# Franc-Z/CuClarabel

Measured on AMD Instinct MI355X. Metric: KKT factorize+solve/sec (fp64) per IPM iter, 100k-var SOCP, higher is better.
Workload: dtype f64

## Files before the change

### cuclarabel_amd/csrc/chain_kernels.hip

```cpp
#include "kernels.hpp"
#include "solve_common.hpp"
#include <cstdlib>

namespace hipkkt {

constexpr int kTinyFrontMax = 8;
constexpr int kChainPF = 4;

__device__ __forceinline__ void chain_add(int* w)
{
    (void)__hip_atomic_fetch_add(w, 1, __ATOMIC_RELAXED, __HIP_MEMORY_SCOPE_AGENT);
}
__device__ __forceinline__ void chain_set(int* w, int v)
{
    __hip_atomic_store(w, v, __ATOMIC_RELAXED, __HIP_MEMORY_SCOPE_AGENT);
}
__device__ __forceinline__ void drain_stores() { asm volatile("s_waitcnt vmcnt(0)" ::: "memory"); }

template <int BS, int PF, int NR>
__device__ __forceinline__ void chain_fwd_block(const SolveArgs& A, const ChainArgs& C, const RecSeg& R, int begin, int bx, long long t0)
{
    extern __shared__ __attribute__((aligned(16))) double smem[];
    __shared__ int sh_ok;
    const int tid = threadIdx.x, lane = tid & 63;
// ... 341 lines not shown
            if (tid < f) z[lds_ix<NR>(c, cst, tid)] = (tid < nc) ? zv[c] * dinv : -zv[c];
    }
#pragma unroll
    for (int c = 0; c < NR; ++c) {
        const double* xc = A.xp + c;
        for (int i = tid + BS; i < f; i += BS)
            z[lds_ix<NR>(c, cst, i)] = (i < nc) ? LD_AGENT_F64(xc + (int64_t)(c0 + i) * NR) * A.Dinv[c0 + i]
                                      : -LD_AGENT_F64(xc + (int64_t)(rec ? rec_idx(rec, i) : T.rows[rp + i - nc]) * NR);
    }
    __syncthreads();
    CH_STAMP(1, 3);
    auto apply = [&](const ItemRegs& R, int it) {
        if constexpr (NR == 2) {
            item_apply_cols<NR>(R, z, cst, nc, f, part, ncpad, it, ncb, lane);
        } else {
            const int rs = it / ncb, cb = it - rs * ncb;
            const int j = cb * 64 + lane, r0 = 8 * rs;
#pragma unroll
            for (int c = 0; c < NR; ++c) {
                double acc = 0.0;
#pragma unroll
                for (int q = 0; q < 8; ++q) acc = fma(R.m[q], (r0 + q < f) ? z[c * cst + r0 + q] : 0.0, acc);
                if (j < nc) part[c * cst + rs * ncpad + j] = acc;
            }
        }
    };
#pragma unroll
    for (int p = 0; p < PB; ++p)
        if (wv + p * NW < nitB) apply(rbk[p], wv + p * NW);
    for (int it0 = wv + PB * NW; it0 < nitB; it0 += 2 * NW) {
        ItemRegs rr[2];
#pragma unroll
        for (int u = 0; u < 2; ++u) {
            const int it = it0 + u * NW;
            const int rs = it / ncb, cb = it - rs * ncb;
            const int j = cb * 64 + lane, r0 = 8 * rs;
            const bool live = it < nitB && !(r0 + 7 < cb * 64);
#pragma unroll
            for (int q = 0; q < 8; ++q) rr[u].m[q] = (live && j < nc && r0 + q < f) ? Wt[j + (int64_t)(r0 + q) * nc] : 0.0;
        }
#pragma unroll
        for (int u = 0; u < 2; ++u)
            if (it0 + u * NW < nitB) apply(rr[u], it0 + u * NW);
    }
    __syncthreads();
    CH_STAMP(1, 4);
    for (int j = tid; j < nc; j += BS) {
        const int pi = j == tid ? ridx : (rec ? rec_idx(rec, j) : T.perm[c0 + j]);
        const double2 vp = lds_sum_pair<NR>(part, j, nrs, ncpad);
#pragma unroll
        for (int c = 0; c < NR; ++c) {
            const double v = lds_sum_col<NR>(vp, part, cst, c, j, nrs, ncpad);
            ST_AGENT_F64(A.xp + (int64_t)(c0 + j) * NR + c, v);
            A.out[c * A.ld_out + pi] = v;
        }
    }
    drain_stores();
    __syncthreads();
    CH_STAMP(1, 5);
    if (tid == 0) chain_set(C.done + s, C.epoch);
}
#undef CH_STAMP

template <int BS, int NR>
__device__ __forceinline__ void chain_bwd_wave(const SolveArgs& A, const ChainArgs& C, const RecSeg& R, int begin, int count, int bx, long long t0)
{
    const int lane = threadIdx.x & 63;
    const int wv = __builtin_amdgcn_readfirstlane((int)(threadIdx.x >> 6));
    const int item = bx * (BS / 64) + wv;
    if (item >= count) return;
    const TreeDev& T = A.T;
    int s, c0, nc, nb, par, idx = 0;
    int64_t f_off;
    if (const char* rec = rec_of(A, R, 1, item)) {
        const SolveHdr h = *reinterpret_cast<const SolveHdr*>(rec);
        idx = rec_idx(rec, lane);
        s = h.s; c0 = h.c0; nc = h.nc; nb = h.nb; par = h.par; f_off = h.mat_off;
    } else {
        const FrontDesc fd = T.desc[begin + item];
        s = fd.s; c0 = fd.c0; nc = fd.nc; nb = fd.nb; f_off = fd.front_off;
        par = T.sn_parent[s];
        idx = (lane < nc) ? T.perm[c0 + lane] : ((lane < nc + nb) ? T.rows[fd.rp + lane - nc] : 0);
    }
    const int f = nc + nb;
    const double* __restrict__ F = A.fronts + f_off;
    const double di = (lane < nc) ? A.Dinv[c0 + lane] : 0.0;
    const int ri = idx, pi = idx;
    double lv0[8];
#pragma unroll
    for (int q = 0; q < 8; ++q) {
        const int j = nc - 1 - q;
        lv0[q] = (j >= 0 && lane > j && lane < f) ? F[lane + (int64_t)j * f] : 0.0;
    }
    if (chain_parent_pending(T, C, par)) {
        int ok = 1;
        if (lane == 0 && !wait_flag(C.done + par, C.epoch, C.abort_word, t0, A.top_limit)) ok = 0;
        ok = __builtin_amdgcn_readfirstlane(ok);
        if (!ok) return;
        asm volatile("" ::: "memory");
    }
    double y[NR];
#pragma unroll
    for (int c = 0; c < NR; ++c) y[c] = (lane < f) ? LD_AGENT_F64(A.xp + (int64_t)(lane < nc ? c0 + lane : ri) * NR + c) : 0.0;
    if (lane < nc) {
#pragma unroll
        for (int c = 0; c < NR; ++c) y[c] *= di;
    }
    for (int j1 = nc; j1 > 0; j1 -= 8) {
        double lv[8];
#pragma unroll
        for (int q = 0; q < 8; ++q) {
            const int j = j1 - 1 - q;
            lv[q] = j1 == nc ? lv0[q] : ((j >= 0 && lane > j && lane < f) ? F[lane + (int64_t)j * f] : 0.0);
        }
#pragma unroll
        for (int q = 0; q < 8; ++q) {
            const int j = j1 - 1 - q;
            if (j >= 0) {
#pragma unroll
                for (int c = 0; c < NR; ++c) {
                    const double sum = wave_reduce_sum(lv[q] * y[c]);
                    if (lane == j) y[c] -= sum;
                }
            }
        }
    }
    if (lane < nc) {
#pragma unroll
        for (int c = 0; c < NR; ++c) {
            ST_AGENT_F64(A.xp + (int64_t)(c0 + lane) * NR + c, y[c]);
            A.out[c * A.ld_out + pi] = y[c];
        }
    }
    drain_stores();
    if (lane == 0) chain_set(C.done + s, C.epoch);
}

template <int BS, int NR>
__device__ __forceinline__ void chain_bwd_tiny(const SolveArgs& A, const ChainArgs& C, const RecSeg& R, int begin, int count, int bx, long long t0)
{
    const int sub = threadIdx.x & 7;
    const int item = bx * (BS >> 3) + (int)(threadIdx.x >> 3);
    const bool live = item < count;
    if (!__any(live)) return;
    const TreeDev& T = A.T;
    int s, c0, nc, nb, par, idx = 0;
    int64_t f_off;
    if (const char* rec = rec_of(A, R, 2, live ? item : count - 1)) {
        const SolveHdr* h = reinterpret_cast<const SolveHdr*>(rec);
        s = h->s; c0 = h->c0; nc = h->nc; nb = h->nb; par = h->par; f_off = h->mat_off;
        idx = rec_idx(rec, sub);
    } else {
        const FrontDesc fd = T.desc[begin + (live ? item : count - 1)];
        s = fd.s; c0 = fd.c0; nc = fd.nc; nb = fd.nb; f_off = fd.front_off;
        par = T.sn_parent[s];
        idx = (sub < nc) ? T.perm[c0 + sub] : ((sub < nc + nb) ? T.rows[fd.rp + sub - nc] : 0);
    }
    const int f = nc + nb;
    const double* __restrict__ F = A.fronts + f_off;
    const double di = (sub < nc) ? A.Dinv[c0 + sub] : 0.0;
    const int ri = idx, pi = idx;
    double lv[kTinyFrontMax];
#pragma unroll
    for (int j = 0; j < kTinyFrontMax; ++j) lv[j] = (j < nc && sub > j && sub < f) ? F[sub + j * f] : 0.0;
    {
        bool ok = true;
        if (live && sub == 0 && chain_parent_pending(T, C, par) && !wait_flag(C.done + par, C.epoch, C.abort_word, t0, A.top_limit)) ok = false;
        if (__any(!ok)) return;
        asm volatile("" ::: "memory");
    }
    double y[NR];
#pragma unroll
    for (int c = 0; c < NR; ++c) y[c] = (sub < f) ? LD_AGENT_F64(A.xp + (int64_t)(sub < nc ? c0 + sub : ri) * NR + c) : 0.0;
    if (sub < nc) {
#pragma unroll
        for (int c = 0; c < NR; ++c) y[c] *= di;
    }
#pragma unroll
    for (int j = kTinyFrontMax - 1; j >= 0; --j) {
#pragma unroll
        for (int c = 0; c < NR; ++c) {
            const double sum = group8_sum(lv[j] * y[c]);
            if (j < nc && sub == j) y[c] -= sum;
        }
    }
    if (live && sub < nc) {
#pragma unroll
        for (int c = 0; c < NR; ++c) {
            ST_AGENT_F64(A.xp + (int64_t)(c0 + sub) * NR + c, y[c]);
            A.out[c * A.ld_out + pi] = y[c];
        }
    }
    drain_stores();
    if (live && sub == 0) chain_set(C.done + s, C.epoch);
}

template <int BS, int NR, int PF>
__global__ __launch_bounds__(BS) void k_bwd_chain(SolveArgs A, ChainArgs C)
{
    const long long t0 = wall_clock64();
    const int k = chain_find_seg(C, blockIdx.x);
    const int begin = C.seg[k].begin, nblock = C.seg[k].nblock, nwave = C.seg[k].nwave, ntiny = C.seg[k].ntiny;
    const int b = (int)blockIdx.x - C.seg[k].wg0;
    const int nwb = (nwave + BS / 64 - 1) / (BS / 64);
    if (b < nblock) { chain_bwd_block<BS, PF, NR>(A, C, C.seg[k].rec, begin, b, t0); return; }
    if (b < nblock + nwb) chain_bwd_wave<BS, NR>(A, C, C.seg[k].rec, begin + nblock, nwave, b - nblock, t0);
    else chain_bwd_tiny<BS, NR>(A, C, C.seg[k].rec, begin + nblock + nwave, ntiny, b - nblock - nwb, t0);
}

#define HIPKKT_NR_SWITCH(nr, ...)                                                                 \
    do {                                                                                         \
        if ((nr) == 1) { constexpr int NR = 1; __VA_ARGS__; }                                    \
        else if ((nr) == 2) { constexpr int NR = 2; __VA_ARGS__; }                               \
        else { constexpr int NR = 4; __VA_ARGS__; }                                              \
    } while (0)

static void init_chain_lds()
{
    static PerDeviceOnce once;
    once.run([]() {
        hipError_t e = hipSuccess;
        auto set = [&](auto k, int bytes) { if (e == hipSuccess) e = set_max_lds(k, bytes); };
#define HIPKKT_SET_CHAIN(NRV) set(k_fwd_chain<kChainBS, NRV, kChainPF>, 150 * 1024); set(k_bwd_chain<kChainBS, NRV, kChainPF>, 150 * 1024);
        HIPKKT_SET_CHAIN(1) HIPKKT_SET_CHAIN(2) HIPKKT_SET_CHAIN(4)
#undef HIPKKT_SET_CHAIN
        return e;
    });
}

void launch_fwd_chain(const SolveArgs& a, const ChainArgs& c, int nwg, size_t lds, hipStream_t st, int nr)
{
    if (nwg <= 0) return;
    init_chain_lds();
    HIPKKT_NR_SWITCH(nr, hipLaunchKernelGGL((k_fwd_chain<kChainBS, NR, kChainPF>), dim3(nwg), dim3(kChainBS), lds * NR, st, a, c));
}
void launch_bwd_chain(const SolveArgs& a, const ChainArgs& c, int nwg, size_t lds, hipStream_t st, int nr)
{
    if (nwg <= 0) return;
    init_chain_lds();
    HIPKKT_NR_SWITCH(nr, hipLaunchKernelGGL((k_bwd_chain<kChainBS, NR, kChainPF>), dim3(nwg), dim3(kChainBS), lds * NR, st, a, c));
}

}
// ... 1 lines not shown
```

### cuclarabel_amd/csrc/hipkkt.hip

```cpp
#include "../../include/hipkkt.h"

#include <hip/hip_runtime.h>

#include <algorithm>
#include <cfloat>
#include <chrono>
#include <cmath>
#include <cstdio>
#include <cstdlib>
#include <cstring>
#include <array>
#include <map>
#include <memory>
#include <mutex>
#include <stdexcept>
#include <string>
#include <vector>

#include "kernels.hpp"
#include "kkt_assembly.hpp"
#include "symbolic.hpp"
#include "knobs.hpp"

namespace hipkkt {
// ... 86 lines not shown
    LDLEngine(int N, const int64_t* colptr, const int64_t* rowval, int base, const std::vector<int>& dsigns,
              const hipkkt_settings& st)
    {
        SymbolicOptions opt;
        opt.ordering = st.ordering;
        opt.amd_dense_scale = st.amd_dense_scale > 0 ? st.amd_dense_scale : 1.5;
        if (st.nd_leaf_size > 0) opt.nd_leaf_size = st.nd_leaf_size;
        opt.user_perm = st.user_perm;
        apply_knobs(opt);
        analyse(N, colptr, rowval, base, opt, S);
        panel_cap = opt.panel_cap;
        panel_max_slices = std::max(1, opt.panel_max_slices);
        dyn_eps = st.dynamic_regularization_eps;
        dyn_delta = st.dynamic_regularization_delta;
        build_schedule();
        upload(dsigns);
        if (knobs().verbose) {
            int nblock = 0, nsl_fronts = 0, ov_slices = 0;
            for (const Launch& L : launches) if (!L.small) { nblock += L.count; nsl_fronts += L.nsliced; }
            if (overlap_wanted()) for (size_t q = ov_first; q < launches.size(); ++q) ov_slices += launches[q].slice_count;
            std::fprintf(stderr, "[hipkkt] N %d, %d supernodes in %zu levels (%zu launches), %d block-class fronts, %d of them in "
                         "%zu row slices; persistent solve set: last %zu launches, %d fronts on %d workgroups, %d (front, slice) tasks; "
                         "factorisation overlap: last %zu launches (%d row slices in them)\n",
                         S.N, S.nsuper, S.levels.size(), launches.size(), nblock, nsl_fronts, slice_list.size(), top_launches,
                         top_count, top_ntask > 0 ? top_sgrid : top_grid, top_ntask, overlap_wanted() ? launches.size() - ov_first : (size_t)0,
                         ov_slices);
            {
                int ntall_all = 0;
                for (const Launch& L : launches) ntall_all += L.ntall;
                if (ntall_all) std::fprintf(stderr, "[hipkkt] %d fronts too tall for the block sweep kernels (k_fwd_tall / k_bwd_tall)\n", ntall_all);
            }
            if (knobs().verbose >= 2)
                for (size_t q = 0; q < launches.size(); ++q) {
                    const Launch& L = launches[q];
                    int fmin = 1 << 30, ncmin = 1 << 30;
                    double flops = 0;
                    for (int t = L.begin; t < L.begin + L.count; ++t) {
                        const int sn = sched[(size_t)t], nc = S.sn_start[sn + 1] - S.sn_start[sn], f = front_size(sn);
                        fmin = std::min(fmin, f); ncmin = std::min(ncmin, nc);
                        flops += (double)nc * (f - nc) * (f - nc) + (double)nc * nc * (f - nc) + (double)nc * nc * nc / 3;
                    }
                    std::fprintf(stderr, "[hipkkt] launch %zu level %d: %d fronts (%s), f %d..%d, nc %d..%d, %d sliced into %d, %d tiles (%d columns deep on average), %.3f GF\n",
                                 q, L.level, L.count, L.small ? "one wave" : "block", fmin, L.fmax, ncmin, L.ncmax, L.nsliced, L.slice_count,
                                 L.ntiles, L.tile_nc, flops * 1e-9);
                }
            if (overlap_wanted())
                for (size_t q = ov_first; q < launches.size(); ++q)
                    std::fprintf(stderr, "[hipkkt] overlap admission: launch %zu: %d panel workgroups, %d tiles behind a gate, %d CUs\n", q,
                                 ov_group_of[q] >= 0 ? ov_groups[(size_t)ov_group_of[q]].count : launches[q].count - launches[q].nsliced + launches[q].slice_count,
                                 launches[q].ntiles, n_cus);
        }
    }

    void factor(const double* d_Kval, const double* d_eps)
    {
        const bool want_stamps = knobs().stamps;
        const bool no_graph = !knobs().graph;
        if (want_stamps || no_graph || n_factor_calls++ == 0) {
            enqueue_factor(d_Kval, d_eps, stream, nullptr, want_stamps);
            return;
        }
        auto key = std::make_pair((const void*)d_Kval, (const void*)d_eps);
        auto it = factor_graphs.find(key);
        if (it == factor_graphs.end()) {
            ensure_capture_streams();
            HIP_CHECK(hipStreamBeginCapture(cap_stream, hipStreamCaptureModeThreadLocal));
            enqueue_factor(d_Kval, d_eps, cap_stream, cap_side, false);
            hipGraph_t g;
            HIP_CHECK(hipStreamEndCapture(cap_stream, &g));
            hipGraphExec_t ex;
            HIP_CHECK(hipGraphInstantiate(&ex, g, nullptr, nullptr, 0));
            HIP_CHECK(hipGraphDestroy(g));
            it = factor_graphs.emplace(key, ex).first;
        }
        HIP_CHECK(hipGraphLaunch(it->second, stream));
    }

    void solve(const double* d_b, double* d_x, bool allow_top = false, int nr = 1, int64_t ldb = 0, int64_t ldx = 0)
    {
        const bool no_graph = !knobs().graph;
        if (nr > 1) {
            if (!supports_nr(nr)) throw ArgError("solve: this structure takes one right-hand side per sweep");
            reserve_nr(nr);
        }
        if (no_graph || nr > 1 || n_solve_calls++ == 0) {
            const bool waits = allow_top && ((!top_disabled && top_launches > 0) || (!chain_disabled && chain_from < launches.size()));
            const bool tok = waits && claim_dev(kOpS);
            TokenRelease rel{this, tok};
            enqueue_solve(d_b, d_x, stream, tok, nr, ldb, ldx, tok);
            if (tok) { rel.on = false; dev_enqueued(true); }
            return;
        }
        auto key = std::make_pair((const void*)d_b, (const void*)d_x);
        auto it = solve_graphs.find(key);
        if (it == solve_graphs.end()) {
            ensure_capture_streams();
            HIP_CHECK(hipStreamBeginCapture(cap_stream, hipStreamCaptureModeThreadLocal));
            enqueue_solve(d_b, d_x, cap_stream, false, 1, 0, 0);
            hipGraph_t g;
            HIP_CHECK(hipStreamEndCapture(cap_stream, &g));
            hipGraphExec_t ex;
            HIP_CHECK(hipGraphInstantiate(&ex, g, nullptr, nullptr, 0));
            HIP_CHECK(hipGraphDestroy(g));
            it = solve_graphs.emplace(key, ex).first;
        }
        HIP_CHECK(hipGraphLaunch(it->second, stream));
    }
    bool supports_nr(int nr) const
    {
        if (nr == 1) return true;
        if (nr != 2 && nr != 4) return false;
        if (top_ntask > 0 && (nr != 2 || top_sgrid2 <= 0)) return false;
        const size_t below = top_ntask > 0 ? launches.size() - top_launches : launches.size();
        for (size_t q = 0; q < below; ++q)
            if (!launches[q].small && (launches[q].ntall > 0 || launches[q].lds_solve * (size_t)nr > kLdsCap)) return false;
        return true;
    }

    void solve_multi(const double* d_B, int64_t ldb, double* d_X, int64_t ldx, int nrhs)
    {
        if (nrhs <= 0) return;
        if (nrhs == 1) { solve(d_B, d_X); return; }
        const int KP = multi_prepare(nrhs);
        launch_permute_in(d_B, ldb, xp_m.p, KP, d_iperm.p, S.N, nrhs, stream);
        multi_sweeps(KP);
        launch_permute_out(d_X, ldx, xp_m.p, KP, d_iperm.p, S.N, nrhs, stream);
        HIP_CHECK(hipGetLastError());
    }
    void solve_multi_rm(const double* d_B, double* d_X, int KP, const double* d_add = nullptr)
    {
        if (KP <= 0 || (KP & 15)) throw ArgError("solve_multi_rm: KP must be a positive multiple of 16");
        multi_prepare(KP);
        multi_sweeps(KP, d_B, d_X, d_add);
        HIP_CHECK(hipGetLastError());
    }

private:
    int multi_prepare(int nrhs)
    {
        const int KP = (nrhs + 15) & ~15;
        if (KP / 8 > 65535) throw ArgError("solve_multi: too many right-hand sides per call");
        {
            int64_t widest = 0;
            for (const Launch& L : launches) if (!L.small) widest = std::max<int64_t>(widest, (L.count + 7) / 8);
            if (widest * (KP / 16) > 65535) throw ArgError("solve_multi: too many right-hand sides per call for this structure (split the call)");
        }
        wait_w(stream);
        if ((size_t)KP > multi_cap) {
            xp_m.alloc((size_t)S.N * KP);
            uvec_m.alloc(std::max<size_t>(S.rows.size(), 1) * KP);
            multi_cap = (size_t)KP;
        }
        if (!d_iperm.p) d_iperm.upload(S.iperm);
        return KP;
    }
    void multi_sweeps(int KP, const double* b_rm = nullptr, double* out_rm = nullptr, const double* add_rm = nullptr)
    {
        SolveArgs a;
        a.T = tree();
// ... 102 lines not shown
            if (cap_side && !new_main) beside.push_back(cap_side);
            if (cu_mask) ov_stream = stream_beside(ov_stream, beside, masked, &ov_concurrent);
            else ov_stream = stream_beside(ov_stream, beside, plain, &ov_concurrent);
            if (!ov_stream) {
                ov_disabled = true;
                std::fprintf(stderr, "[hipkkt] no stream for the Schur tiles: factorisation overlap off\n");
            } else if (!had) {
                HIP_CHECK(hipEventCreateWithFlags(&ev_ov_fork, hipEventDisableTiming));
                HIP_CHECK(hipEventCreateWithFlags(&ev_ov_join, hipEventDisableTiming));
            }
            if (ov_stream && !ov_concurrent && knobs().verbose)
                std::fprintf(stderr, "[hipkkt] the main and the tile stream share a hardware queue: no merged panel kernel for this handle\n");
        }
        ensure_capture_streams();
        if (new_main) {
            std::vector<hipStream_t> beside{st};
            if (ov_stream) beside.push_back(ov_stream);
            cap_side = stream_beside(cap_side, beside, plain, &side_concurrent);
            if (!side_concurrent && knobs().verbose)
                std::fprintf(stderr, "[hipkkt] no stream beside the main stream for the W formation: it will run in submission order\n");
        }
        sides_for = st;
    }

    void enqueue_factor(const double* d_Kval, const double* d_eps, hipStream_t st, hipStream_t side, bool want_stamps)
    {
        wait_w(st);
        if (ov_join_pending) {
            if (side) HIP_CHECK(hipEventSynchronize(ev_ov_join));
            else HIP_CHECK(hipStreamWaitEvent(st, ev_ov_join, 0));
            ov_join_pending = false;
        }
        ZeroList zl;
        zl.add(flags.p, 3);
        const bool want_ov = overlap_wanted();
        const bool use_ov = want_ov && !side && !want_stamps && !ov_disabled && ov_first < launches.size();
        const bool no_overlap = knobs().no_overlap;
        const bool side_w = !side && !no_overlap && !want_stamps && late_launches > 0 && late_launches < launches.size();
        const bool tok_x = use_ov && claim_dev(kOpX);
        const bool tok = tok_x || (side_w && claim_dev(kOpM));
        TokenRelease ov_release{this, tok};
        if (!side && !want_stamps) choose_side_streams(st, tok_x);
        const bool ov_on = tok_x && !ov_disabled && ov_stream != nullptr;
        auto group_of = [&](size_t q) -> const MergeGroup* {
            return (ov_concurrent && q < ov_group_of.size() && ov_group_of[q] >= 0) ? &ov_groups[(size_t)ov_group_of[q]] : nullptr;
        };
        const size_t merge_from = (ov_concurrent && !ov_groups.empty()) ? ov_groups.back().first : ~(size_t)0;
        if (ov_on) {
            zl.add(d_ov_prog.p, S.nsuper);
            zl.add(d_ov_done.p, S.nsuper);
            if (!slice_list.empty()) zl.add(d_ov_sprog.p, (int)slice_list.size());
            zl.add(d_ov_started.p, (int)launches.size());
        }
        launch_zero_ints_multi(zl, st);
        FactorArgs a;
        a.T = tree();
        a.Kval = d_Kval;
        a.eps = d_eps;
        a.fronts = fronts.p;
        a.upd = upd.p;
        a.Dinv = Dinv.p;
        a.flags = flags.p;
        a.dyn_eps = dyn_eps;
        a.dyn_delta = dyn_delta;
        a.ov_prog = d_ov_prog.p; a.ov_done = d_ov_done.p; a.ov_ntiles = d_ov_ntiles.p; a.ov = 0;
        a.ov_sprog = d_ov_sprog.p; a.ov_sbase = d_ov_sbase.p;
        a.ov_started = d_ov_started.p; a.ov_slot = 0;
        const long long ov_limit = knobs().ov_test_limit;
        a.ov_limit = ov_limit;
        a.stamps = nullptr;
        a.stamp_row = 0;
        if (want_stamps) {
            if (!stamps.p) { stamps.alloc(launches.size() * 16); }
            stamps.zero(st);
            a.stamps = (long long*)stamps.p;
        }
        int li = 0;
        bool forked = false;
#ifdef HIPKKT_EXPERIMENTS
        static const bool no_gate = std::getenv("HIPKKT_EXPERIMENT_NO_GATE") != nullptr;
#else
        constexpr bool no_gate = false;
#endif
#ifdef HIPKKT_EXPERIMENTS
        static const int skip_w_after = std::getenv("HIPKKT_EXPERIMENT_SKIP_WINV") ? std::atoi(std::getenv("HIPKKT_EXPERIMENT_SKIP_WINV")) : -1;
        const bool skip_w = skip_w_after >= 0 && n_skipw_calls++ >= skip_w_after;
#else
        const bool skip_w = false;
#endif
        auto form_w = [&](const int* list, int count, int ncmax, hipStream_t on, int max_blocks) {
            const size_t i0 = (size_t)(list - d_tinv_list.p);
            const int nsmall = i0 + (size_t)count < tinv_small_prefix.size() ? tinv_small_prefix[i0 + (size_t)count] - tinv_small_prefix[i0] : 0;
            if (!skip_w) launch_tinv(a.T, fronts.p, tinv.p, list, count, ncmax, on, max_blocks, nsmall);
        };
        const size_t nl = launches.size();
        const size_t first_top = (tok && side_w) ? nl - late_launches : nl;
        bool eager_fork = false;
        int w_done = 0;
        for (size_t q = 0; q < nl; ++q) {
            const Launch& L = launches[q];
            a.stamp_row = li++;
            const bool runs = ov_on && merge_from < nl;
            const size_t tail_fork = runs ? nl : (nl >= (size_t)std::max(0, knobs().winv_tail) ? nl - (size_t)std::max(0, knobs().winv_tail) : 0);
            const MergeGroup* gq = runs ? group_of(q) : nullptr;
            const bool run_forks = knobs().winv_run_forks;
            const bool run_first = gq && gq->first == q && (run_forks || q == merge_from);
            auto fork_at = [&](size_t want) {
// ... 67 lines not shown
            w_pending = true;
        } else {
            form_w(d_tinv_list.p, (int)tinv_list.size(), tinv_ncmax, st, 0);
        }
        if (ov_on) {
            HIP_CHECK(hipEventRecord(ev_ov_join, ov_stream));
            ov_join_pending = true;
        }
        if (tok) {
            ov_release.on = false;
            dev_enqueued(true);
        }
        HIP_CHECK(hipGetLastError());
        if (want_stamps) {
            std::vector<long long> h(launches.size() * 16);
            HIP_CHECK(hipMemcpyAsync(h.data(), stamps.p, h.size() * 8, hipMemcpyDeviceToHost, st));
            HIP_CHECK(hipStreamSynchronize(st));
            static int printed = 0;
            if (printed++ == 2) {
                for (size_t r = 0; r < launches.size(); ++r) {
                    const long long* q = &h[r * 16];
                    if (launches[r].small) continue;
                    std::fprintf(stderr, "[stamps2] launch %zu: wave 0's items %.1f us (first batch's loads %.1f us), then all waves %.1f us\n", r, (q[7] - q[6]) * 0.01, (q[15] - q[6]) * 0.01, (q[3] - q[7]) * 0.01);
                    std::fprintf(stderr, "[stamps] launch %zu fronts %d f=%lld nc=%lld kids=%lld | zero %.1f K %.1f kids %.1f factor %.1f "
                                 "(diag %.1f trsm %.1f trail %.1f) store %.1f us  clk %.0f MHz\n", r, launches[r].count, q[11], q[12], q[13],
                                 (q[1] - q[0]) * 0.01, (q[2] - q[1]) * 0.01, (q[3] - q[2]) * 0.01, (q[4] - q[3]) * 0.01,
                                 q[8] * 0.01, q[9] * 0.01, q[10] * 0.01, (q[5] - q[4]) * 0.01,
                                 (double)q[14] / ((q[5] - q[0]) * 0.01));
                }
            }
        }
    }

    void reserve_nr(int nr)
    {
        if ((size_t)nr <= nr_cap) return;
        wait_w(stream);
        HIP_CHECK(hipStreamSynchronize(stream));
        for (auto& kv : solve_graphs) (void)hipGraphExecDestroy(kv.second);
        solve_graphs.clear();
        xp.alloc((size_t)S.N * nr);
        uvec.alloc(std::max<size_t>(S.rows.size(), 1) * nr);
        nr_cap = (size_t)nr;
    }
    int top_grid_for(int nr)
    {
        if (nr == 1) return top_grid;
        if (top_ntask > 0) return nr == 2 ? top_sgrid2 : 0;
        int& g = top_grid_nr[nr == 2 ? 0 : 1];
        if (g < 0) g = std::min(top_grid, top_solve_capacity_nr(top_lds * (size_t)nr, nr));
        return g;
    }

    void enqueue_solve(const double* d_b, double* d_x, hipStream_t st, bool use_top, int nr, int64_t ldb, int64_t ldx, bool allow_chain = false)
    {
        SolveArgs a;
        a.T = tree();
        a.fronts = fronts.p;
        a.tinv = tinv.p;
        a.Dinv = Dinv.p;
        a.b = d_b;
        a.out = d_x;
        a.xp = xp.p;
        a.uvec = uvec.p;
        const long long top_limit = knobs().top_test_limit;
        a.top_limit = top_limit;
        const int stamp_call = knobs().top_stamps;
        a.top_stamps = nullptr;
        bool stamp_now = false;
        a.ld_b = ldb; a.ld_out = ldx; a.ld_xp = S.N; a.ld_uvec = (int64_t)std::max<size_t>(S.rows.size(), 1);
        a.tk_pos = d_tk_pos.p; a.tk_sl = d_tk_sl.p; a.tbase = d_tbase.p; a.xf = xf.p; a.add = nullptr;
        a.chain_cnt = nullptr;
        a.recs = d_recs.p ? reinterpret_cast<const char*>(d_recs.p) : nullptr;
        a.tall_ws = tall_ws.p;
        const bool no_top = knobs().no_top;
        if (nr > 1 && top_ntask > 0 && (no_top || !use_top || top_disabled || top_sgrid2 <= 0)) {
            for (int c = 0; c < nr; ++c) enqueue_solve(d_b + (int64_t)c * ldb, d_x + (int64_t)c * ldx, st, use_top, 1, 0, 0, allow_chain);
            return;
        }
        const size_t nl = launches.size();
        const bool chain_env = knobs().chain;
        const bool chain_top = knobs().chain_top;
        const bool chain_want = chain_env && allow_chain && !chain_disabled && chain_from < nl && chain_lds * (size_t)nr <= 150 * 1024;
        const bool keep_top = chain_want && (chain_top || top_ntask > 0);
        const int tgrid = (no_top || !use_top || top_disabled || (chain_want && !keep_top)) ? 0 : top_grid_for(nr);
        size_t ntl = tgrid > 0 ? top_launches : 0;
        int ncount = top_count;
        if (ntl > 0 && w_pending && late_launches > 0 && late_launches < ntl && !(nr > 1 && top_ntask > 0)) { ntl = late_launches; ncount = late_count; }
        const size_t first_w = nl - std::min(nl, late_launches);
        const bool chain_on = chain_want && chain_from + 2 <= nl - ntl;
        const size_t nper = chain_on ? chain_from : nl - ntl;
        const bool no_merge = knobs().no_level_merge;
        auto pair_at = [&](size_t q) {
            return !no_merge && q + 1 < nper && !launches[q].small && launches[q].ntall == 0 && launches[q + 1].small &&
                   launches[q].level == launches[q + 1].level;
        };
        auto pair_rec = [](const Launch& Lb, const Launch& Ls) {
            RecSeg r = Ls.rec;
            r.off[0] = Lb.rec.off[0]; r.stride[0] = Lb.rec.stride[0]; r.fmax[0] = Lb.rec.fmax[0];
            return r;
        };
        bool chain_stamp = false;
        ChainArgs ca;
        int ca_wgs = 0;
        size_t ca_lds = 0;
        auto chain_reset = [&]() {
            ca.nseg = 0; ca.lo = 1 << 30; ca.hi = 0; ca.cnt = d_chain.p; ca.done = d_chain.p + S.nsuper; ca.nchild = d_chain_nchild.p;
            ca.abort_word = top_flags.p + 2 * top_nflag; ca.epoch = chain_epoch;
            ca.lo0 = chain_on ? launches[nper].begin : 0;
            ca.nstamp = chain_on ? launches[nl - ntl - 1].begin + launches[nl - ntl - 1].count - ca.lo0 : 0;
            ca_wgs = 0; ca_lds = 0;
        };
        auto chain_flush = [&](bool fwd) {
            if (ca.nseg > 0) {
                a.top_stamps = chain_stamp ? (long long*)top_stamps.p : nullptr;
                if (fwd) launch_fwd_chain(a, ca, ca_wgs, ca_lds, st, nr);
                else launch_bwd_chain(a, ca, ca_wgs, ca_lds, st, nr);
                a.top_stamps = nullptr;
            }
            chain_reset();
        };
        auto chain_add = [&](const Launch& L, bool fwd) {
            const bool blocks = !L.small;
            if (ca.nseg == kChainMaxSeg) chain_flush(fwd);
            ChainSeg& sg = ca.seg[ca.nseg++];
            sg.begin = L.begin;
            sg.nblock = blocks ? L.count : 0;
            sg.nwave = blocks ? 0 : L.count - L.ntiny;
            sg.ntiny = blocks ? 0 : L.ntiny;
            sg.wg0 = ca_wgs;
// ... 1414 lines not shown
            pool.push_back(s.b);
        }
        spans.clear();
    }
    ~Profiler()
    {
        for (Span& s : spans) { (void)hipEventDestroy(s.a); (void)hipEventDestroy(s.b); }
        for (hipEvent_t e : pool) (void)hipEventDestroy(e);
    }
};

}

using namespace hipkkt;

struct hipkkt_ldl_s {
    int device = 0;
    hipkkt_settings st;
    hipStream_t stream = nullptr;
    int64_t N = 0, nnzK = 0;
    int base = 0;
    std::unique_ptr<LDLEngine> eng;
    DBuf<double> Kval, vals, b, x;
    DBuf<double> mB;
    size_t mcap = 0;
    DBuf<int> idx;
    ~hipkkt_ldl_s() { if (stream) (void)hipStreamDestroy(stream); }
};

struct hipkkt_kkt_s {
    int device = 0;
    hipkkt_settings st;
    hipStream_t stream = nullptr;
    bool own_stream = true;
    KKTAssembly K;
    std::unique_ptr<LDLEngine> eng;
    DBuf<double> Kval, Pval, Aval;
    DBuf<int> mapP, mapA, mapHs, mapDiag, mapU, mapV, mapD, soc_of_entry;
    DBuf<int64_t> fptr;
    DBuf<int> fcol, fmap;
    DBuf<int64_t> fpend;
    DBuf<double> fval;
    bool fval_dirty = true;
    DBuf<int> kpos;
    DBuf<int> long_rows;
    DBuf<int64_t> long_chunk_ptr, chunk_q;
    DBuf<double> long_partial;
    int nlong = 0, nchunks = 0;
    size_t long_partial_cols = 0;
    int lanes_per_row = 8;
    DBuf<double> b, x, e, dx, rx, rz, sbuf, zbuf, ybuf;
    double *cur_x = nullptr, *cur_dx = nullptr;
    DBuf<double> partial, scal;
    std::unique_ptr<PinnedScalars> pin;
    DBuf<int> c_kind, c_off, c_numel, c_sidx, c_soff, c_elem, c_soclist;
    DBuf<int64_t> c_boff;
    DBuf<double> w, eta, soc_u, soc_v, soc_eta2, Hs;
    DBuf<int> fail;
    int nsoc = 0, npsd = 0, psd_kmax = 1;
    DBuf<int> c_explist, c_powlist, c_nsidx;
    DBuf<double> c_param, ns_grad, ns_H;
    int nexp = 0, npow = 0, ns_strategy = HIPKKT_SCALING_PRIMAL_DUAL;
    double ns_mu = 0.0;
    DBuf<int> gp_cone, gp_dim1, gp_off, gp_small, gp_big, gp_mapP, gp_mapQR, gp_mapD;
    DBuf<double> gp_alpha, gp_grad, gp_d, gp_p, gp_qr;
    int ngp_small = 0, ngp_big = 0;
    double gp_mu = 0.0;
    DBuf<int> c_psdlist, c_psddim;
    DBuf<int64_t> c_psdaoff;
    DBuf<double> psdA, psdR, psdRinv;
    bool has_psd = false, psd_too_big = false, scaling_valid = false;
    double last_eps = 0;
    int64_t last_ir = 0;
    DBuf<double> irbuf;
    double *ir_state = nullptr, *ir_readback = nullptr, *ir_sticky = nullptr, *ir_norms = nullptr, *sys_out_dev = nullptr;
    int ir_stride = 0;
    int r_spec = 1;
    bool publish_ok = true;
    long long publish_seq = 0;
    int spec_low_calls = 0;
    bool deferred = false;
    DBuf<double> lam;
    DBuf<double> sq, snegq, sb, sx2, sz2, sworkx, sworkz, sconic, spa, spb, spc;
    DBuf<double> sys_partial, sys_dots, sys_cached, sys_in;
    bool sys_ready = false;
    bool sys_lazy = false;
    bool sys_const_pending = false;
    bool sys_update_unread = false;
    DBuf<double> hst;
    bool host_vars_valid = false;
    hipEvent_t ev_upload = nullptr;
    void host_upload_mark(hipStream_t st)
    {
        if (!ev_upload) HIP_CHECK(hipEventCreateWithFlags(&ev_upload, hipEventDisableTiming));
        HIP_CHECK(hipEventRecord(ev_upload, st));
    }
    void host_upload_wait() { if (ev_upload) HIP_CHECK(hipEventSynchronize(ev_upload)); }
    DBuf<double> mB, mX, mC, mE, mE2, mpartial, mnorms;
    DBuf<int> mmask;
    size_t mcap = 0;
    Profiler prof;
    ~hipkkt_kkt_s()
    {
        if (ev_upload) (void)hipEventDestroy(ev_upload);
        if (stream && own_stream) (void)hipStreamDestroy(stream);
    }
// ... 296 lines not shown
        if (!h || nrhs < 0 || (nrhs > 0 && (!d_X || !d_B || ldx < h->N || ldb < h->N)))
            throw ArgError("hipkkt_ldl_solve_multi_dev: bad argument");
        HIP_CHECK(hipSetDevice(h->device));
        h->eng->solve_multi(d_B, ldb, d_X, ldx, (int)nrhs);
        return HIPKKT_OK;
    });
}

int hipkkt_ldl_solve_multi(hipkkt_ldl_t h, int64_t nrhs, double* X, const double* B)
{
    return guarded([&]() {
        if (!h || nrhs < 0 || (nrhs > 0 && (!X || !B))) throw ArgError("hipkkt_ldl_solve_multi: bad argument");
        if (nrhs == 0) return HIPKKT_OK;
        HIP_CHECK(hipSetDevice(h->device));
        if ((size_t)nrhs > h->mcap) { h->mB.alloc((size_t)h->N * nrhs); h->mcap = (size_t)nrhs; }
        const size_t bytes = (size_t)h->N * nrhs * sizeof(double);
        HIP_CHECK(hipMemcpyAsync(h->mB.p, B, bytes, hipMemcpyHostToDevice, h->stream));
        h->eng->solve_multi(h->mB.p, h->N, h->mB.p, h->N, (int)nrhs);
        HIP_CHECK(hipMemcpyAsync(X, h->mB.p, bytes, hipMemcpyDeviceToHost, h->stream));
        HIP_CHECK(hipStreamSynchronize(h->stream));
        return HIPKKT_OK;
    });
}

int hipkkt_ldl_info(hipkkt_ldl_t h, hipkkt_info* info)
{
    return guarded([&]() {
        if (!h || !info) throw ArgError("hipkkt_ldl_info: bad argument");
        std::memset(info, 0, sizeof(*info));
        fill_info(h->eng->S, info);
        return HIPKKT_OK;
    });
}

int hipkkt_ldl_get_perm(hipkkt_ldl_t h, int64_t* perm)
{
    return guarded([&]() {
        if (!h || !perm) throw ArgError("hipkkt_ldl_get_perm: bad argument");
        for (int64_t i = 0; i < h->N; ++i) perm[i] = h->eng->S.perm[i];
        return HIPKKT_OK;
    });
}

int hipkkt_ldl_fallbacks(hipkkt_ldl_t h, int64_t out[2])
{
    return guarded([&]() {
        if (!h || !out) throw ArgError("hipkkt_ldl_fallbacks: bad argument");
        out[0] = h->eng->n_ov_fallbacks;
        out[1] = h->eng->n_top_fallbacks;
        return HIPKKT_OK;
    });
}

int hipkkt_kkt_create(hipkkt_kkt_t* out, int64_t n, int64_t m, const int64_t* Pcolptr, const int64_t* Prowval,
                      const double* Pnzval, const int64_t* Acolptr, const int64_t* Arowval, const double* Anzval,
                      int64_t ncones, const int32_t* kinds, const int64_t* dims, const hipkkt_settings* settings,
                      int base)
{
    return hipkkt_kkt_create_ex(out, n, m, Pcolptr, Prowval, Pnzval, Acolptr, Arowval, Anzval, ncones, kinds, dims, nullptr,
                                settings, base);
}

int hipkkt_kkt_create_ex(hipkkt_kkt_t* out, int64_t n, int64_t m, const int64_t* Pcolptr, const int64_t* Prowval,
                         const double* Pnzval, const int64_t* Acolptr, const int64_t* Arowval, const double* Anzval,
                         int64_t ncones, const int32_t* kinds, const int64_t* dims, const double* cone_params,
                         const hipkkt_settings* settings, int base)
{
    std::vector<int64_t> pptr;
    std::vector<double> pvals;
    if (ncones > 0 && kinds) {
        for (int64_t c = 0; c < ncones; ++c)
            if (kinds[c] == HIPKKT_CONE_GENPOW) {
                g_last_error = "a generalized power cone has one alpha per row of its first block: use hipkkt_kkt_create_ex2";
                return HIPKKT_ERR_ARG;
            }
        if (cone_params) {
            pptr.assign((size_t)ncones + 1, base);
            for (int64_t c = 0; c < ncones; ++c) {
                pptr[(size_t)c + 1] = pptr[(size_t)c];
                if (kinds[c] == HIPKKT_CONE_POW) { pvals.push_back(cone_params[c]); pptr[(size_t)c + 1] += 1; }
            }
        }
    }
    return hipkkt_kkt_create_ex2(out, n, m, Pcolptr, Prowval, Pnzval, Acolptr, Arowval, Anzval, ncones, kinds, dims,
                                 pptr.empty() ? nullptr : pptr.data(), pvals.data(), settings, base);
}

int hipkkt_kkt_create_ex2(hipkkt_kkt_t* out, int64_t n, int64_t m, const int64_t* Pcolptr, const int64_t* Prowval,
                          const double* Pnzval, const int64_t* Acolptr, const int64_t* Arowval, const double* Anzval,
                          int64_t ncones, const int32_t* kinds, const int64_t* dims, const int64_t* cone_param_ptr,
                          const double* cone_param_vals, const hipkkt_settings* settings, int base)
{
    return guarded([&]() {
        if (!out || !Pcolptr || !Acolptr || n < 0 || m < 0 || ncones < 0 || (ncones > 0 && (!kinds || !dims)))
            throw ArgError("hipkkt_kkt_create: bad argument");
        if (base != 0 && base != 1) throw ArgError("index_base must be 0 or 1");
        if (n + m == 0) throw ArgError("empty problem");
        std::unique_ptr<hipkkt_kkt_s> h(new hipkkt_kkt_s);
        if (settings) h->st = *settings; else hipkkt_default_settings(&h->st);
        try {
            assemble_kkt(n, m, Pcolptr, Prowval, Pnzval, Acolptr, Arowval, Anzval, ncones, kinds, dims, base, h->K, cone_param_ptr,
                         cone_param_vals);
        } catch (const std::runtime_error& e) {
            throw ArgError(e.what());
        }
        h->device = select_device(h->st);
        HIP_CHECK(hipStreamCreateWithFlags(&h->stream, hipStreamNonBlocking));
        KKTAssembly& K = h->K;
        hipkkt_settings st = h->st;
        if (st.ordering == HIPKKT_ORDER_USER && !st.user_perm) throw ArgError("ORDER_USER needs user_perm");
        std::vector<int64_t> rv(K.rowval.begin(), K.rowval.end());
        std::vector<int64_t> uperm;
        if (st.ordering == HIPKKT_ORDER_USER) {
            uperm.resize(K.N);
            for (int i = 0; i < K.N; ++i) uperm[i] = st.user_perm[i] - base;
            st.user_perm = uperm.data();
        }
        h->eng.reset(new LDLEngine(K.N, K.colptr.data(), rv.data(), 0, K.dsigns, st));
        h->eng->stream = h->stream;
        h->eng->set_device(h->device);
        h->st.user_perm = nullptr;

        h->Kval.upload(K.nzval);
        h->mapP.upload(K.mapP);
        h->mapA.upload(K.mapA);
        h->mapHs.upload(K.mapHs);
        h->mapDiag.upload(K.map_diag);
        h->mapU.upload(K.mapU);
        h->mapV.upload(K.mapV);
        h->mapD.upload(K.mapD);
        h->Pval.alloc(K.mapP.size());
        h->Aval.alloc(K.mapA.size());
        {
            const int N = K.N;
            std::vector<int64_t> ptr((size_t)N + 1, 0);
            for (int j = 0; j < N; ++j)
                for (int64_t q = K.colptr[j]; q < K.colptr[j + 1]; ++q) {
                    int i = K.rowval[q];
                    ptr[i + 1]++;
                    if (i != j) ptr[j + 1]++;
                }
            for (int i = 0; i < N; ++i) ptr[i + 1] += ptr[i];
            std::vector<int> col((size_t)ptr[N]), vmap((size_t)ptr[N]);
            std::vector<int64_t> nx(ptr.begin(), ptr.end() - 1);
            for (int j = 0; j < N; ++j) {
                for (int64_t q = K.colptr[j]; q < K.colptr[j + 1]; ++q) {
                    int i = K.rowval[q];
                    int64_t d = nx[j]++;
                    col[d] = i;
                    vmap[d] = (int)q;
                }
            }
            for (int j = 0; j < N; ++j)
                for (int64_t q = K.colptr[j]; q < K.colptr[j + 1]; ++q) {
                    int i = K.rowval[q];
                    if (i == j) continue;
                    int64_t d = nx[i]++;
                    col[d] = j;
                    vmap[d] = (int)q;
                }
            h->fptr.upload(ptr);
            h->fcol.upload(col);
            h->fmap.upload(vmap);
            {
                std::vector<int64_t> pend((size_t)std::max<int64_t>(K.n, 1), 0);
                for (int64_t i = 0; i < K.n; ++i)
                    pend[(size_t)i] = std::lower_bound(col.begin() + ptr[(size_t)i], col.begin() + ptr[(size_t)i + 1], (int)K.n) - col.begin();
                h->fpend.upload(pend);
            }
            h->fval.alloc(vmap.size());
            {
                std::vector<int> kp((size_t)2 * K.nnzK, -1);
                for (size_t q = 0; q < vmap.size(); ++q) {
                    const size_t e = (size_t)vmap[q];
                    if (kp[2 * e] < 0) kp[2 * e] = (int)q; else kp[2 * e + 1] = (int)q;
                }
                h->kpos.upload(kp);
            }
            {
                std::vector<int> lrows;
// ... 99 lines not shown
                for (double* q : {h->gp_grad.p, h->gp_d.p, h->gp_p.p, h->gp_qr.p}) HIP_CHECK(hipMemset(q, 0, gl * sizeof(double)));
            }
            {
                std::vector<int> plist, pdim(nc, 0);
                std::vector<int64_t> paoff(nc, 0);
                int64_t ao = 0;
                for (size_t c = 0; c < nc; ++c) {
                    const ConeInfo& ci = K.cones[c];
                    if (ci.kind != HIPKKT_CONE_PSD) continue;
                    plist.push_back((int)c);
                    pdim[c] = ci.dim;
                    paoff[c] = ao;
                    ao += (int64_t)ci.dim * ci.dim;
                    h->psd_kmax = std::max(h->psd_kmax, ci.dim);
                }
                h->npsd = (int)plist.size();
                h->c_psdlist.upload(plist); h->c_psddim.upload(pdim); h->c_psdaoff.upload(paoff);
                h->psdA.alloc((size_t)ao); h->psdR.alloc((size_t)ao); h->psdRinv.alloc((size_t)ao);
            }
            h->c_kind.upload(kind); h->c_off.upload(off); h->c_numel.upload(numel); h->c_boff.upload(boff);
            h->c_sidx.upload(sidx); h->c_soff.upload(soff); h->c_elem.upload(elem); h->c_soclist.upload(soclist);
            h->soc_of_entry.upload(soc_of);
            h->w.alloc((size_t)K.m); h->eta.alloc(nc); h->lam.alloc((size_t)K.m);
            h->soc_u.alloc((size_t)K.sparse_len); h->soc_v.alloc((size_t)K.sparse_len);
            h->soc_eta2.alloc((size_t)K.nsparse); h->Hs.alloc((size_t)K.nHs);
            h->fail.alloc(1);
            HIP_CHECK(hipMemset(h->fail.p, 0, sizeof(int)));
        }
        *out = h.release();
        return HIPKKT_OK;
    });
}

void hipkkt_kkt_destroy(hipkkt_kkt_t h)
{
    if (!h) return;
    (void)hipSetDevice(h->device);
    (void)hipStreamSynchronize(h->stream);
    delete h;
}

int hipkkt_kkt_info(hipkkt_kkt_t h, hipkkt_info* info)
{
    return guarded([&]() {
        if (!h || !info) throw ArgError("hipkkt_kkt_info: bad argument");
        std::memset(info, 0, sizeof(*info));
        fill_info(h->eng->S, info);
        info->n = h->K.n; info->m = h->K.m; info->p = h->K.p;
        info->nHs = h->K.nHs; info->nsparse_soc = h->K.nsparse; info->sparse_soc_len = h->K.sparse_len;
        return HIPKKT_OK;
    });
}

static int kkt_update_device(hipkkt_kkt_t h, bool deferred = false)
{
    KKTAssembly& K = h->K;
    int pu = h->prof.begin(0, h->stream);
    launch_update_values(h->Kval.p, h->mapHs.p, h->Hs.p, (int)K.nHs, h->mapU.p, h->mapV.p, h->mapD.p, h->soc_u.p, h->soc_v.p,
                         h->soc_eta2.p, h->soc_of_entry.p, K.sparse_len, K.nsparse, h->fval_dirty ? nullptr : h->fval.p,
                         h->kpos.p, h->stream);
    const double* eps_ptr = nullptr;
    if (h->st.static_regularization_enable) {
        launch_regularizer(h->Kval.p, h->mapDiag.p, K.N, h->st.static_regularization_constant,
                           h->st.static_regularization_proportional, h->partial.p, h->scal.p, h->stream);
        eps_ptr = h->scal.p;
    }
    h->prof.end(pu, h->stream);
    int pf = h->prof.begin(1, h->stream);
    h->eng->factor(h->Kval.p, eps_ptr);
    h->prof.end(pf, h->stream);
    launch_collect_status(h->scal.p + 8, h->scal.p, h->fail.p, h->eng->flags_ptr(), h->stream, deferred ? h->ir_sticky : nullptr);
    if (deferred) return HIPKKT_OK;
    HIP_CHECK(hipMemcpyAsync(h->pin->h + 8, h->scal.p + 8, 5 * sizeof(double), hipMemcpyDeviceToHost, h->stream));
    HIP_CHECK(hipStreamSynchronize(h->stream));
    if (h->pin->h[12] != 0.0) {
        h->eng->ov_gave_up();
        h->eng->factor(h->Kval.p, eps_ptr);
        launch_collect_status(h->scal.p + 8, h->scal.p, h->fail.p, h->eng->flags_ptr(), h->stream);
        HIP_CHECK(hipMemcpyAsync(h->pin->h + 8, h->scal.p + 8, 5 * sizeof(double), hipMemcpyDeviceToHost, h->stream));
        HIP_CHECK(hipStreamSynchronize(h->stream));
    }
    h->last_eps = h->st.static_regularization_enable ? h->pin->h[8] : 0.0;
    h->prof.acc.dynamic_regularizations += (int64_t)h->pin->h[10];
    if (h->pin->h[9] != 0.0) return HIPKKT_NUMERIC_FAILURE;
    return h->pin->h[11] != 0.0 ? HIPKKT_NUMERIC_FAILURE : HIPKKT_OK;
}

int hipkkt_kkt_update_cones(hipkkt_kkt_t h, const double* Hs, const double* soc_u, const double* soc_v,
                            const double* soc_eta2)
{
    return guarded([&]() {
        if (!h) throw ArgError("null handle");
        KKTAssembly& K = h->K;
        if ((K.nHs > 0 && !Hs) || (K.nsparse > 0 && (!soc_u || !soc_v || !soc_eta2)))
            throw ArgError("hipkkt_kkt_update_cones: missing cone data");
        if (K.ngenpow > 0)
            throw ArgError("hipkkt_kkt_update_cones: (Hs, u, v, eta^2) cannot carry p, q, r of a generalized power cone; such a "
                           "handle is scaled on the device (hipkkt_kkt_update_from_sz, hipkkt_kkt_system_update)");
        HIP_CHECK(hipSetDevice(h->device));
        if (K.nHs) HIP_CHECK(hipMemcpyAsync(h->Hs.p, Hs, (size_t)K.nHs * sizeof(double), hipMemcpyHostToDevice, h->stream));
        if (K.nsparse) {
            HIP_CHECK(hipMemcpyAsync(h->soc_u.p, soc_u, (size_t)K.sparse_len * sizeof(double), hipMemcpyHostToDevice, h->stream));
            HIP_CHECK(hipMemcpyAsync(h->soc_v.p, soc_v, (size_t)K.sparse_len * sizeof(double), hipMemcpyHostToDevice, h->stream));
            HIP_CHECK(hipMemcpyAsync(h->soc_eta2.p, soc_eta2, (size_t)K.nsparse * sizeof(double), hipMemcpyHostToDevice, h->stream));
        }
        launch_zero_ints(h->fail.p, 1, h->stream);
        h->scaling_valid = false;
        return kkt_update_device(h);
    });
}

static int kkt_update_from_sz_dev_impl(hipkkt_kkt_t h, const double* d_s, const double* d_z, bool deferred)
{
    return guarded([&]() {
        if (!h || (h->K.m > 0 && (!d_s || !d_z))) throw ArgError("hipkkt_kkt_update_from_sz: bad argument");
        if (h->psd_too_big)
            throw ArgError("update_from_sz: PSD cones with side > 48 are scaled by the caller; use hipkkt_kkt_update_cones");
        HIP_CHECK(hipSetDevice(h->device));
        launch_zero_ints(h->fail.p, 1, h->stream);
        int pu = h->prof.begin(0, h->stream);
        h->gp_mu = h->ns_mu;
        launch_cone_scaling(h->cone_dev(), h->cone_state(), d_s, d_z, h->K.m, h->stream);
        h->prof.end(pu, h->stream);
        h->scaling_valid = true;
        return kkt_update_device(h, deferred);
    });
}
int hipkkt_kkt_update_from_sz_dev(hipkkt_kkt_t h, const double* d_s, const double* d_z)
{
    return kkt_update_from_sz_dev_impl(h, d_s, d_z, h && h->deferred);
}

int hipkkt_kkt_update_from_sz(hipkkt_kkt_t h, const double* s, const double* z)
{
    return guarded([&]() {
        if (!h || (h->K.m > 0 && (!s || !z))) throw ArgError("hipkkt_kkt_update_from_sz: bad argument");
        HIP_CHECK(hipSetDevice(h->device));
        size_t bytes = (size_t)h->K.m * sizeof(double);
        if (bytes) {
            HIP_CHECK(hipMemcpyAsync(h->sbuf.p, s, bytes, hipMemcpyHostToDevice, h->stream));
            HIP_CHECK(hipMemcpyAsync(h->zbuf.p, z, bytes, hipMemcpyHostToDevice, h->stream));
        }
        return hipkkt_kkt_update_from_sz_dev(h, h->sbuf.p, h->zbuf.p);
    });
}

int hipkkt_kkt_update_P(hipkkt_kkt_t h, const double* Pnzval)
{
    return guarded([&]() {
        if (!h || (h->K.mapP.size() && !Pnzval)) throw ArgError("hipkkt_kkt_update_P: bad argument");
        HIP_CHECK(hipSetDevice(h->device));
        size_t k = h->K.mapP.size();
        if (!k) return HIPKKT_OK;
        HIP_CHECK(hipMemcpyAsync(h->Pval.p, Pnzval, k * sizeof(double), hipMemcpyHostToDevice, h->stream));
        launch_scatter(h->Kval.p, h->mapP.p, h->Pval.p, (int64_t)k, 1.0, h->stream);
        h->fval_dirty = true;
        HIP_CHECK(hipStreamSynchronize(h->stream));
        return HIPKKT_OK;
    });
}

int hipkkt_kkt_update_A(hipkkt_kkt_t h, const double* Anzval)
{
    return guarded([&]() {
        if (!h || (h->K.mapA.size() && !Anzval)) throw ArgError("hipkkt_kkt_update_A: bad argument");
        HIP_CHECK(hipSetDevice(h->device));
        size_t k = h->K.mapA.size();
        if (!k) return HIPKKT_OK;
        HIP_CHECK(hipMemcpyAsync(h->Aval.p, Anzval, k * sizeof(double), hipMemcpyHostToDevice, h->stream));
        launch_scatter(h->Kval.p, h->mapA.p, h->Aval.p, (int64_t)k, 1.0, h->stream);
        h->fval_dirty = true;
        HIP_CHECK(hipStreamSynchronize(h->stream));
        return HIPKKT_OK;
    });
}

int hipkkt_kkt_setrhs_dev(hipkkt_kkt_t h, const double* d_rx, const double* d_rz)
{
    return guarded([&]() {
        if (!h || (h->K.n && !d_rx) || (h->K.m && !d_rz)) throw ArgError("hipkkt_kkt_setrhs: bad argument");
        HIP_CHECK(hipSetDevice(h->device));
        launch_pack_rhs(h->b.p, d_rx, d_rz, h->K.n, h->K.m, h->K.p, h->stream);
        return HIPKKT_OK;
    });
}

int hipkkt_kkt_setrhs(hipkkt_kkt_t h, const double* rx, const double* rz)
{
    return guarded([&]() {
        if (!h || (h->K.n && !rx) || (h->K.m && !rz)) throw ArgError("hipkkt_kkt_setrhs: bad argument");
        HIP_CHECK(hipSetDevice(h->device));
        if (h->K.n) HIP_CHECK(hipMemcpyAsync(h->rx.p, rx, (size_t)h->K.n * sizeof(double), hipMemcpyHostToDevice, h->stream));
        if (h->K.m) HIP_CHECK(hipMemcpyAsync(h->rz.p, rz, (size_t)h->K.m * sizeof(double), hipMemcpyHostToDevice, h->stream));
        launch_pack_rhs(h->b.p, h->rx.p, h->rz.p, h->K.n, h->K.m, h->K.p, h->stream);
        HIP_CHECK(hipStreamSynchronize(h->stream));
        return HIPKKT_OK;
    });
}

static SpmvDev kkt_spmv(hipkkt_kkt_t h)
{
    if (h->fval_dirty) {
        launch_gather_values(h->fval.p, h->Kval.p, h->fmap.p, (int64_t)h->fmap.n, h->stream);
        h->fval_dirty = false;
    }
    SpmvDev A;
    A.ptr = h->fptr.p; A.col = h->fcol.p; A.vmap = h->fmap.p; A.val = h->fval.p; A.N = h->K.N;
    A.pend = h->fpend.p;
    A.lanes_per_row = h->lanes_per_row;
    A.nlong = h->nlong; A.nchunks = h->nchunks; A.long_rows = h->long_rows.p; A.long_chunk_ptr = h->long_chunk_ptr.p;
    A.chunk_q = h->chunk_q.p; A.long_partial = h->long_partial.p;
    return A;
}

static bool kkt_partials_mode(hipkkt_kkt_t h, int nr) { return residual_partials_ok(kkt_spmv(h), nr); }
static double* kkt_partials(hipkkt_kkt_t h, bool candidate) { return h->partial.p + (candidate ? h->partial.n / 2 : 0); }
static void kkt_enqueue_refine_error(hipkkt_kkt_t h, const double* xi, double* norm_out, double* normb_out, int nr, bool candidate)
{
    const SpmvDev A = kkt_spmv(h);
    const bool unfinished = kkt_partials_mode(h, nr);
    int pr = h->prof.begin(3, h->stream);
    launch_residual(A, h->Kval.p, h->b.p, xi, h->e.p, kkt_partials(h, candidate), unfinished ? nullptr : norm_out, h->stream, nr,
                    nr > 1 ? (int64_t)h->K.N : 0, h->eng->top_abort_word(), h->scal.p + 3, normb_out);
    h->prof.end(pr, h->stream);
}
static void kkt_trisolve(hipkkt_kkt_t h, const double* rhs, double* out, bool allow_top = true, int nr = 1)
{
    int ps = h->prof.begin(2, h->stream);
    h->eng->solve(rhs, out, allow_top, nr, h->K.N, h->K.N);
    h->prof.end(ps, h->stream);
}

struct IrNorms { double *norme0, *normb, *cand; };
static IrNorms kkt_ir_norms(hipkkt_kkt_t h, int nr)
{
    if (nr == 1) return IrNorms{h->scal.p + 1, h->scal.p + 2, h->scal.p + 4};
    return IrNorms{h->ir_norms, h->ir_norms + kMaxNR, h->ir_norms + 2 * kMaxNR};
}
static void kkt_launch_ir(hipkkt_kkt_t h, int r, bool first, bool readback, bool fold, int nr)
{
    const hipkkt_settings& st = h->st;
    const IrNorms nm = kkt_ir_norms(h, nr);
    const double* abortw = h->eng->top_abort_word() ? h->scal.p + 3 : nullptr;
    IrPartials Q;
    const bool unfinished = kkt_partials_mode(h, nr);
    if (unfinished) {
        Q.np = residual_grid(kkt_spmv(h)) + 1;
        Q.e0 = kkt_partials(h, false);
        Q.b0 = Q.e0 + (size_t)nr * Q.np;
        Q.cand = r > 0 ? kkt_partials(h, true) : nullptr;
        Q.flag_in = h->eng->top_abort_word();
    }
    launch_ir_round(h->ir_state, h->ir_stride, r, first, nm.norme0, nm.normb, nm.cand, abortw, h->x.p, h->dx.p, h->K.N, nr,
                    st.iterative_refinement_abstol, st.iterative_refinement_reltol, st.iterative_refinement_stop_ratio,
                    std::max(st.iterative_refinement_max_iter, 0), readback ? h->ir_readback : nullptr,
                    (fold && (nr == 1 || unfinished)) ? h->ir_sticky : nullptr, h->stream, Q);
    if (fold && nr > 1 && !unfinished) launch_ir_fold(h->ir_state, h->ir_stride, r, nr, abortw, h->ir_sticky, h->stream);
}
static void kkt_enqueue_round(hipkkt_kkt_t h, int r, bool first, bool readback, bool fold, int nr)
{
    kkt_trisolve(h, h->e.p, h->dx.p, true, nr);
    launch_axpby_sum(h->dx.p, h->dx.p, h->x.p, (int64_t)h->K.N * nr, h->stream);
    kkt_enqueue_refine_error(h, h->dx.p, kkt_ir_norms(h, nr).cand, nullptr, nr, true);
    kkt_launch_ir(h, r, first, readback, fold, nr);
}
static int kkt_solve_core(hipkkt_kkt_t h, bool may_defer = false, int nr = 1, int64_t* ir_out = nullptr, bool force_defer = false)
{
    const hipkkt_settings& st = h->st;
    const bool deferred = force_defer || (may_defer && h->deferred);
    h->cur_x = h->x.p;
    h->cur_dx = h->dx.p;
    h->last_ir = 0;
    if (ir_out) for (int c = 0; c < nr; ++c) ir_out[c] = deferred ? -1 : 0;
    if (!st.iterative_refinement_enable) {
        kkt_trisolve(h, h->b.p, h->x.p, false, nr);
        int bad = 0;
        launch_zero_ints(h->fail.p, 1, h->stream);
        launch_check_finite(h->x.p, h->K.N * nr, h->fail.p, h->stream);
        if (deferred) { launch_fold_flag(h->ir_sticky, h->fail.p, h->stream); return HIPKKT_OK; }
        HIP_CHECK(hipMemcpyAsync(&bad, h->fail.p, sizeof(int), hipMemcpyDeviceToHost, h->stream));
        HIP_CHECK(hipStreamSynchronize(h->stream));
        return bad ? HIPKKT_NUMERIC_FAILURE : HIPKKT_OK;
    }
    const int max_iter = std::max(st.iterative_refinement_max_iter, 0);
    int R = std::min(max_iter, std::max(h->r_spec, deferred ? 1 : 0));
    const IrNorms nm = kkt_ir_norms(h, nr);
    kkt_trisolve(h, h->b.p, h->x.p, true, nr);
    kkt_enqueue_refine_error(h, h->x.p, nm.norme0, nm.normb, nr, false);
    if (R == 0) kkt_launch_ir(h, 0, true, !deferred, deferred, nr);
    for (int r = 1; r <= R; ++r) kkt_enqueue_round(h, r, r == 1, r == R && !deferred, r == R && deferred, nr);
    if (deferred) { h->last_ir = -1; return HIPKKT_OK; }
    int64_t total = 0;
    for (;;) {
        HIP_CHECK(hipMemcpyAsync(h->pin->h + 16, h->ir_readback, 5 * (size_t)nr * sizeof(double), hipMemcpyDeviceToHost, h->stream));
        HIP_CHECK(hipStreamSynchronize(h->stream));
        bool any_active = false, any_bad = false, aborted = false;
        total = 0;
        for (int c = 0; c < nr; ++c) {
            const double* rb = h->pin->h + 16 + 5 * c;
            any_active = any_active || rb[0] != 0.0;
            any_bad = any_bad || rb[2] != 0.0;
            aborted = aborted || rb[4] != 0.0;
            total += (int64_t)rb[1];
            if (ir_out) ir_out[c] = (int64_t)rb[1];
        }
        if (aborted && h->eng->top_abort_word() != nullptr) {
            h->eng->top_gave_up();
            return kkt_solve_core(h, false, nr, ir_out);
        }
        h->last_ir = total;
        if (any_bad) { h->prof.acc.ir_iterations += total; return HIPKKT_NUMERIC_FAILURE; }
        if (!any_active || R >= max_iter) break;
        ++R;
        kkt_enqueue_round(h, R, false, true, false, nr);
    }
// ... 485 lines not shown
    if (rc != HIPKKT_OK) return rc;
    if (enqueue_only) h->sys_update_unread = true;
    return guarded([&]() { return sys_after_update(h); });
}

int hipkkt_kkt_system_solve_initial_point(hipkkt_kkt_t h, double* d_x, double* d_s, double* d_z)
{
    return guarded([&]() {
        if (!h || !h->sys_ready) throw ArgError("hipkkt_kkt_system_*: call hipkkt_kkt_system_init first");
        if ((h->K.n && !d_x) || (h->K.m && (!d_s || !d_z))) throw ArgError("hipkkt_kkt_system_solve_initial_point: bad argument");
        HIP_CHECK(hipSetDevice(h->device));
        const int n = h->K.n, m = h->K.m;
        int rc = sys_flush_startup(h);
        if (rc != HIPKKT_OK) return rc;
        if (h->mapP.n == 0) {
            if (n) HIP_CHECK(hipMemsetAsync(h->sworkx.p, 0, (size_t)n * sizeof(double), h->stream));
            rc = sys_solve_into(h, h->sworkx.p, h->sb.p, d_x, h->sworkz.p);
            if (rc != HIPKKT_OK) return rc;
            launch_neg_copy(d_s, h->sworkz.p, m, h->stream);
            if (m) HIP_CHECK(hipMemsetAsync(h->sworkz.p, 0, (size_t)m * sizeof(double), h->stream));
            rc = sys_solve_into(h, h->snegq.p, h->sworkz.p, nullptr, d_z);
            if (rc != HIPKKT_OK) return rc;
        } else {
            rc = sys_solve_into(h, h->snegq.p, h->sb.p, d_x, d_z);
            if (rc != HIPKKT_OK) return rc;
            launch_neg_copy(d_s, d_z, m, h->stream);
        }
        HIP_CHECK(hipStreamSynchronize(h->stream));
        return HIPKKT_OK;
    });
}

static void sys_finish_step(hipkkt_kkt_t h, const double* x1, const double* z1, double* d_lhs_x, double* d_lhs_s, double* d_lhs_z,
                            double* lhs_tau_kappa, double rhs_tau, double rhs_kappa, const double* d_var_x, double var_tau,
                            double var_kappa, bool with_const = false, const double* addend = nullptr, const Publish& pub = Publish{})
{
    const int n = h->K.n, m = h->K.m;
    hipStream_t st = h->stream;
    const double* x2 = with_const ? h->x.p : h->sx2.p;
    const double* z2 = with_const ? h->x.p + n : h->sz2.p;
    launch_P_spmv2(sys_spmv(h), h->Kval.p, x1, d_var_x, x2, var_tau, h->spa.p, h->spb.p, h->sworkx.p,
                   with_const ? h->spc.p : nullptr, n, st);
    DotPairs P{};
    P.npairs = with_const ? 7 : 4;
    if (with_const) {
        P.a[4] = h->sq.p; P.b[4] = x2; P.len[4] = n;
        P.a[5] = h->sb.p; P.b[5] = z2; P.len[5] = m;
        P.a[6] = x2; P.b[6] = h->spc.p; P.len[6] = n;
    }
    P.a[0] = h->sq.p; P.b[0] = x1; P.len[0] = n;
    P.a[1] = h->sb.p; P.b[1] = z1; P.len[1] = m;
    P.a[2] = d_var_x; P.b[2] = h->spa.p; P.len[2] = n;
    P.a[3] = h->sworkx.p; P.b[3] = h->spb.p; P.len[3] = n;
    launch_dots_sys_step(P, h->sys_partial.p, h->sys_cached.p, rhs_tau, rhs_kappa, var_tau, var_kappa, h->sys_out_dev, d_lhs_x, d_lhs_z,
                         x1, z1, x2, z2, n, m, st, with_const ? h->sx2.p : nullptr, with_const ? h->sz2.p : nullptr);
    launch_mul_Hs(h->cone_dev(), h->cone_state(), d_lhs_s, d_lhs_z, m, st, addend ? addend : h->sconic.p, pub);
    if (!lhs_tau_kappa) return;
    HIP_CHECK(hipMemcpyAsync(h->pin->h + 48, h->sys_out_dev, 2 * sizeof(double), hipMemcpyDeviceToHost, st));
    HIP_CHECK(hipStreamSynchronize(st));
    lhs_tau_kappa[0] = h->pin->h[48];
    lhs_tau_kappa[1] = h->pin->h[49];
}
static int sys_flush_update_status(hipkkt_kkt_t h)
{
    if (!h->sys_update_unread) return HIPKKT_OK;
    h->sys_update_unread = false;
    HIP_CHECK(hipMemcpyAsync(h->pin->h + 40, h->ir_sticky, 8 * sizeof(double), hipMemcpyDeviceToHost, h->stream));
    launch_zero_ints((int*)h->ir_sticky, 16, h->stream);
    HIP_CHECK(hipStreamSynchronize(h->stream));
    bool gave_up = false;
    int rc = kkt_eval_sticky(h, h->pin->h + 40, &gave_up);
    if (rc == HIPKKT_REFINEMENT_INCOMPLETE) rc = gave_up ? kkt_update_device(h) : HIPKKT_OK;
    return rc;
}
static int sys_flush_startup(hipkkt_kkt_t h)
{
    const int rc = sys_flush_update_status(h);
    return rc == HIPKKT_NUMERIC_FAILURE ? HIPKKT_OK : rc;
}
static void sys_cache_constant_terms(hipkkt_kkt_t h)
{
    launch_P_spmv(sys_spmv(h), h->Kval.p, h->sx2.p, h->spa.p, h->K.n, h->stream);
    DotPairs P{};
    P.npairs = 3;
    P.a[0] = h->sq.p; P.b[0] = h->sx2.p; P.len[0] = h->K.n;
    P.a[1] = h->sb.p; P.b[1] = h->sz2.p; P.len[1] = h->K.m;
    P.a[2] = h->sx2.p; P.b[2] = h->spa.p; P.len[2] = h->K.n;
    launch_dots(P, h->sys_partial.p, h->sys_cached.p, h->stream);
}

static int sys_solve_step(hipkkt_kkt_t h, double* d_lhs_x, double* d_lhs_s, double* d_lhs_z, double* lhs_tau_kappa,
                          const double* d_rhs_x, const double* d_rhs_s, const double* d_rhs_z, double rhs_tau,
                          double rhs_kappa, const double* d_var_x, const double* d_var_s, const double* d_var_z,
                          double var_tau, double var_kappa, int steptype)
{
    if (!h->sys_ready) throw ArgError("hipkkt_kkt_system_*: call hipkkt_kkt_system_init first");
    const int n = h->K.n, m = h->K.m;
    const bool affine = steptype == 0;
    if ((n && (!d_lhs_x || !d_rhs_x || !d_var_x)) || (m && (!d_lhs_s || !d_lhs_z || !d_rhs_z || !d_var_s || !d_var_z)) ||
        (m && !affine && !d_rhs_s) || !lhs_tau_kappa || (steptype != 0 && steptype != 1))
        throw ArgError("hipkkt_kkt_system_solve: bad argument");
    if (!h->scaling_valid) throw ArgError("hipkkt_kkt_system_solve: needs the cone scaling of hipkkt_kkt_system_update");
    if (h->deferred) throw ArgError("hipkkt_kkt_system_*: level C reads its scalars back (deferred status is for level B)");
    HIP_CHECK(hipSetDevice(h->device));
    hipStream_t st = h->stream;
    const bool pair = h->sys_const_pending && affine && h->eng->supports_nr(2);
    if (h->sys_const_pending && !pair) {
        h->sys_const_pending = false;
        int rc = sys_flush_update_status(h);
        if (rc == HIPKKT_OK) rc = sys_constant_rhs(h);
        if (rc != HIPKKT_OK) return rc;
    }
    h->sys_const_pending = false;
    const size_t N = (size_t)h->K.N;
    auto run = [&](bool defer) -> int {
        if (!affine && !launch_sys_offset(h->cone_dev(), h->cone_state(), h->sconic.p, h->sworkz.p, d_rhs_s, d_var_z, d_rhs_z,
                                          m, false, st))
            throw ArgError("hipkkt_kkt_system_solve: unsupported cone kind");
        if (pair) {
            launch_pack_rhs_affine(h->b.p, h->snegq.p, h->sb.p, d_rhs_x, d_var_s, d_rhs_z, n, m, h->K.p, 2, st);
            int rc = kkt_solve_core(h, false, 2, nullptr, defer);
            if (rc != HIPKKT_OK) return rc;
        } else {
            if (affine) launch_pack_rhs_affine(h->b.p, nullptr, nullptr, d_rhs_x, d_var_s, d_rhs_z, n, m, h->K.p, 1, st);
            else launch_pack_rhs(h->b.p, d_rhs_x, h->sworkz.p, n, m, h->K.p, st);
            int rc = kkt_solve_core(h, false, 1, nullptr, defer);
            if (rc != HIPKKT_OK) return rc;
        }
        const double* x1 = h->x.p + (pair ? N : 0);
        sys_finish_step(h, x1, x1 + n, d_lhs_x, d_lhs_s, d_lhs_z, defer ? nullptr : lhs_tau_kappa, rhs_tau, rhs_kappa, d_var_x, var_tau, var_kappa,
                        pair, affine ? d_var_s : nullptr,
                        (defer && h->publish_ok) ? Publish{h->pin->h + 40, h->ir_sticky, 10, 8, (double)++h->publish_seq} : Publish{});
        return HIPKKT_OK;
    };
    if (h->sys_lazy && h->st.iterative_refinement_enable) {
        const bool update_unread = h->sys_update_unread;
        h->sys_update_unread = false;
        int rc = run(true);
        if (rc != HIPKKT_OK) return rc;
        if (h->publish_ok) {
            HIP_CHECK(hipStreamSynchronize(st));
            if (h->pin->h[50] != (double)h->publish_seq || knobs().test_publish_fail) {
                h->publish_ok = false;
                if (knobs().verbose) std::fprintf(stderr, "[hipkkt] status record not published to host memory: copying it from now on\n");
                if (update_unread) {
                    rc = kkt_update_device(h);
                    if (rc != HIPKKT_OK) return rc;
                }
                return run(false);
            }
        } else {
            HIP_CHECK(hipMemcpyAsync(h->pin->h + 40, h->ir_sticky, 10 * sizeof(double), hipMemcpyDeviceToHost, st));
            launch_zero_ints((int*)h->ir_sticky, 16, st);
            HIP_CHECK(hipStreamSynchronize(st));
        }
        bool gave_up = false;
        rc = kkt_eval_sticky(h, h->pin->h + 40, &gave_up, true);
        h->last_ir = (int64_t)h->pin->h[43];
        if (rc == HIPKKT_OK) {
            lhs_tau_kappa[0] = h->pin->h[48];
            lhs_tau_kappa[1] = h->pin->h[49];
            return HIPKKT_OK;
        }
        if (rc != HIPKKT_REFINEMENT_INCOMPLETE) return rc;
        if (update_unread && gave_up) {
            rc = kkt_update_device(h);
            if (rc != HIPKKT_OK) return rc;
        }
    } else {
        int rc = sys_flush_update_status(h);
        if (rc != HIPKKT_OK) return rc;
    }
    return run(false);
}

int hipkkt_kkt_system_solve(hipkkt_kkt_t h, double* d_lhs_x, double* d_lhs_s, double* d_lhs_z, double* lhs_tau_kappa,
                            const double* d_rhs_x, const double* d_rhs_s, const double* d_rhs_z, double rhs_tau,
                            double rhs_kappa, const double* d_var_x, const double* d_var_s, const double* d_var_z,
// ... 566 lines not shown
```

### cuclarabel_amd/csrc/kernels.hip

```cpp
#include "kernels.hpp"
#include "knobs.hpp"
#include <algorithm>

#include <cmath>

namespace hipkkt {

static inline int grid_for(int64_t n, int bs, int cap = 4096)
{
    int64_t g = (n + bs - 1) / bs;
    if (g < 1) g = 1;
    if (g > cap) g = cap;
    return (int)g;
}

__global__ void k_scatter(double* __restrict__ K, const int* __restrict__ idx, const double* __restrict__ v,
                          int64_t n, double scale)
{
    for (int64_t i = blockIdx.x * (int64_t)blockDim.x + threadIdx.x; i < n; i += (int64_t)gridDim.x * blockDim.x)
        K[idx[i]] = v[i] * scale;
}
void launch_scatter(double* K, const int* idx, const double* v, int64_t n, double scale, hipStream_t st)
{
    if (n <= 0) return;
    hipLaunchKernelGGL(k_scatter, dim3(grid_for(n, 256)), dim3(256), 0, st, K, idx, v, n, scale);
}
__device__ __forceinline__ void put_k(double* __restrict__ K, double* __restrict__ fval, const int* __restrict__ kpos, int e, double v)
{
    K[e] = v;
    if (fval) {
        const int p0 = kpos[2 * e], p1 = kpos[2 * e + 1];
        if (p0 >= 0) fval[p0] = v;
        if (p1 >= 0) fval[p1] = v;
    }
}
__global__ void k_update_values(double* __restrict__ K, const int* __restrict__ mapHs, const double* __restrict__ Hs, int nHs,
                                const int* __restrict__ mapU, const int* __restrict__ mapV, const int* __restrict__ mapD,
                                const double* __restrict__ u, const double* __restrict__ v, const double* __restrict__ eta2,
                                const int* __restrict__ soc_of_entry, int sparse_len, int nsparse,
                                double* __restrict__ fval, const int* __restrict__ kpos)
{
    const int total = nHs + sparse_len + nsparse;
    for (int i = blockIdx.x * blockDim.x + threadIdx.x; i < total; i += gridDim.x * blockDim.x) {
        if (i < nHs) {
            put_k(K, fval, kpos, mapHs[i], -Hs[i]);
        } else if (i < nHs + sparse_len) {
            const int j = i - nHs;
            const double e2 = eta2[soc_of_entry[j]];
            put_k(K, fval, kpos, mapU[j], u[j] * (-e2));
            put_k(K, fval, kpos, mapV[j], v[j] * (-e2));
        } else {
            const int j = i - nHs - sparse_len;
            put_k(K, fval, kpos, mapD[2 * j], -eta2[j]);
            put_k(K, fval, kpos, mapD[2 * j + 1], eta2[j]);
        }
    }
}
void launch_update_values(double* K, const int* mapHs, const double* Hs, int nHs, const int* mapU, const int* mapV,
                          const int* mapD, const double* u, const double* v, const double* eta2, const int* soc_of_entry,
                          int sparse_len, int nsparse, double* fval, const int* kpos, hipStream_t st)
{
    const int total = nHs + sparse_len + nsparse;
    if (total <= 0) return;
    hipLaunchKernelGGL(k_update_values, dim3(grid_for(total, 256)), dim3(256), 0, st, K, mapHs, Hs, nHs, mapU, mapV, mapD, u, v,
                       eta2, soc_of_entry, sparse_len, nsparse, fval, kpos);
}
__global__ void k_scale(double* __restrict__ K, const int* __restrict__ idx, double scale, int64_t n)
{
    for (int64_t i = blockIdx.x * (int64_t)blockDim.x + threadIdx.x; i < n; i += (int64_t)gridDim.x * blockDim.x)
        K[idx[i]] *= scale;
}
void launch_scale(double* K, const int* idx, double scale, int64_t n, hipStream_t st)
{
    if (n <= 0) return;
    hipLaunchKernelGGL(k_scale, dim3(grid_for(n, 256)), dim3(256), 0, st, K, idx, scale, n);
}

__global__ void k_soc_columns(double* __restrict__ K, const int* __restrict__ mapU, const int* __restrict__ mapV,
                              const int* __restrict__ mapD, const double* __restrict__ u,
                              const double* __restrict__ v, const double* __restrict__ eta2,
                              const int* __restrict__ soc_of_entry, int sparse_len, int nsparse)
{
    const int i = blockIdx.x * blockDim.x + threadIdx.x;
    if (i < sparse_len) {
        const double e2 = eta2[soc_of_entry[i]];
        K[mapU[i]] = u[i] * (-e2);
        K[mapV[i]] = v[i] * (-e2);
    }
    if (i < nsparse) {
        K[mapD[2 * i]] = -eta2[i];
        K[mapD[2 * i + 1]] = eta2[i];
    }
}
void launch_soc_columns(double* K, const int* mapU, const int* mapV, const int* mapD, const double* u,
                        const double* v, const double* eta2, const int* soc_of_entry, int sparse_len,
                        int nsparse, hipStream_t st)
{
    int n = sparse_len > nsparse ? sparse_len : nsparse;
    if (n <= 0) return;
    hipLaunchKernelGGL(k_soc_columns, dim3((n + 255) / 256), dim3(256), 0, st, K, mapU, mapV, mapD, u, v, eta2,
                       soc_of_entry, sparse_len, nsparse);
}

__device__ inline double block_max_256(double v, double* sh)
{
#pragma unroll
    for (int o = 32; o > 0; o >>= 1) v = fmax(v, __shfl_down(v, o, 64));
    const int lane = threadIdx.x & 63, wave = threadIdx.x >> 6;
    if (lane == 0) sh[wave] = v;
    __syncthreads();
    if (threadIdx.x == 0) {
        for (int w = 1; w < (int)(blockDim.x >> 6); ++w) v = fmax(v, sh[w]);
    }
    return v;
}

constexpr int kRedBlocks = 256;

__global__ void k_diag_absmax(const double* __restrict__ K, const int* __restrict__ diag, int N,
                              double* __restrict__ partial)
{
    __shared__ double sh[4];
    double v = 0.0;
    for (int i = blockIdx.x * blockDim.x + threadIdx.x; i < N; i += gridDim.x * blockDim.x)
        v = fmax(v, fabs(K[diag[i]]));
    v = block_max_256(v, sh);
    if (threadIdx.x == 0) partial[blockIdx.x] = v;
}
__global__ void k_finish_regularizer(const double* __restrict__ partial, int nparts, double c0, double c1,
                                     double* __restrict__ eps_out)
{
    __shared__ double sh[4];
    double v = 0.0;
    for (int i = threadIdx.x; i < nparts; i += blockDim.x) v = fmax(v, partial[i]);
    v = block_max_256(v, sh);
    if (threadIdx.x == 0) eps_out[0] = c0 + c1 * v;
}
void launch_regularizer(const double* K, const int* diag, int N, double c0, double c1, double* partial,
                        double* eps_out, hipStream_t st)
{
    int g = grid_for(N, 256, kRedBlocks);
    hipLaunchKernelGGL(k_diag_absmax, dim3(g), dim3(256), 0, st, K, diag, N, partial);
    hipLaunchKernelGGL(k_finish_regularizer, dim3(1), dim3(256), 0, st, partial, g, c0, c1, eps_out);
}

template <int G, int NC>
__global__ __launch_bounds__(256) void k_residual(SpmvDev A, const double* __restrict__ K,
                                                  const double* __restrict__ b, const double* __restrict__ x,
                                                  double* __restrict__ e, double* __restrict__ partial, int64_t ld,
                                                  double* __restrict__ bpartial)
{
    __shared__ double sh[4];
    const int col0 = blockIdx.y * NC;
    b += col0 * ld;
    x += col0 * ld;
    e += col0 * ld;
    partial += col0 * (gridDim.x + 1);
    const int sub = threadIdx.x % G;
    const int rows_per_block = 256 / G;
    if (bpartial) bpartial += col0 * gridDim.x;
    double vmax[NC], bmax[NC];
    bool bad[NC];
#pragma unroll
    for (int c = 0; c < NC; ++c) { vmax[c] = 0.0; bmax[c] = 0.0; bad[c] = false; }
    for (int row = blockIdx.x * rows_per_block + threadIdx.x / G; row < A.N; row += gridDim.x * rows_per_block) {
        const int64_t q0 = A.ptr[row], q1 = A.ptr[row + 1];
        if (q1 - q0 > kLongRow) continue;
// ... 196 lines not shown
    const int N = n + m + p;
    const bool aff = ncol == 1 || blockIdx.y == 1;
    b += (int64_t)blockIdx.y * N;
    for (int i = blockIdx.x * blockDim.x + threadIdx.x; i < N; i += gridDim.x * blockDim.x) {
        double v = 0.0;
        if (i < n) v = aff ? rhs_x[i] : negq[i];
        else if (i < n + m) v = aff ? s[i - n] - rhs_z[i - n] : bb[i - n];
        b[i] = v;
    }
}
void launch_pack_rhs_affine(double* b, const double* negq, const double* bb, const double* rhs_x, const double* s,
                            const double* rhs_z, int n, int m, int p, int ncol, hipStream_t st)
{
    hipLaunchKernelGGL(k_pack_rhs_affine, dim3(grid_for(n + m + p, 256), ncol), dim3(256), 0, st, b, negq, bb, rhs_x, s, rhs_z,
                       n, m, p, ncol);
}
__global__ void k_accept_columns(double* __restrict__ x, const double* __restrict__ cand, double* __restrict__ e,
                                 const double* __restrict__ e2, const int* __restrict__ mask, int N)
{
    if (!mask[blockIdx.y]) return;
    const int64_t o = (int64_t)blockIdx.y * N;
    for (int i = blockIdx.x * blockDim.x + threadIdx.x; i < N; i += gridDim.x * blockDim.x) {
        x[o + i] = cand[o + i];
        e[o + i] = e2[o + i];
    }
}
void launch_accept_columns(double* x, const double* cand, double* e, const double* e2, const int* mask, int N,
                           int nrhs, hipStream_t st)
{
    if (N <= 0 || nrhs <= 0) return;
    hipLaunchKernelGGL(k_accept_columns, dim3(grid_for(N, 256, 1024), nrhs), dim3(256), 0, st, x, cand, e, e2, mask, N);
}
__global__ void k_unpack_lhs(double* __restrict__ lhsx, double* __restrict__ lhsz, const double* __restrict__ x, int n, int m)
{
    for (int i = blockIdx.x * blockDim.x + threadIdx.x; i < n + m; i += gridDim.x * blockDim.x) {
        if (i < n) { if (lhsx) lhsx[i] = x[i]; }
        else if (lhsz) lhsz[i - n] = x[i];
    }
}
void launch_unpack_lhs(double* lhsx, double* lhsz, const double* x, int n, int m, hipStream_t st)
{
    if (n + m <= 0 || (!lhsx && !lhsz)) return;
    hipLaunchKernelGGL(k_unpack_lhs, dim3(grid_for(n + m, 256)), dim3(256), 0, st, lhsx, lhsz, x, n, m);
}
__global__ void k_zero_ints(int* __restrict__ p, int n)
{
    for (int i = blockIdx.x * blockDim.x + threadIdx.x; i < n; i += gridDim.x * blockDim.x) p[i] = 0;
}
__global__ void k_zero_ints_multi(ZeroList Z)
{
    int* __restrict__ p = Z.p[blockIdx.y];
    const int n = Z.n[blockIdx.y];
    for (int i = blockIdx.x * blockDim.x + threadIdx.x; i < n; i += gridDim.x * blockDim.x) p[i] = 0;
}
void launch_zero_ints_multi(const ZeroList& Z, hipStream_t st)
{
    if (Z.count <= 0) return;
    int nmax = 1;
    for (int k = 0; k < Z.count; ++k) nmax = Z.n[k] > nmax ? Z.n[k] : nmax;
    hipLaunchKernelGGL(k_zero_ints_multi, dim3(grid_for(nmax, 256, 256), Z.count), dim3(256), 0, st, Z);
}
__global__ void k_collect_status(double* __restrict__ dst, const double* __restrict__ eps, const int* __restrict__ conefail,
                                 const int* __restrict__ flags, double* __restrict__ sticky)
{
    if (threadIdx.x == 0) {
        const double e = eps ? eps[0] : 0.0, cf = conefail ? (double)conefail[0] : 0.0;
        const double f0 = (double)flags[0], f1 = (double)flags[1], f2 = (double)flags[2];
        dst[0] = e;
        dst[1] = cf;
        dst[2] = f0;
        dst[3] = f1;
        dst[4] = f2;
        if (sticky) {
            if (cf != 0.0 || f1 != 0.0) sticky[0] = 1.0;
            if (f2 != 0.0) sticky[7] = 1.0;
            sticky[4] += f0;
            sticky[5] = e;
        }
    }
}
void launch_collect_status(double* dst, const double* eps, const int* conefail, const int* flags, hipStream_t st, double* sticky)
{
    hipLaunchKernelGGL(k_collect_status, dim3(1), dim3(64), 0, st, dst, eps, conefail, flags, sticky);
}
__device__ inline void ir_initial(double norme0, double normb, double abstol, double reltol, int max_iter,
                                  double& active, double& rounds, double& bad, double& norme)
{
    norme = norme0;
    bad = isfinite(norme) ? 0.0 : 1.0;
    rounds = 0.0;
    active = (bad == 0.0 && max_iter > 0 && !(norme <= abstol + reltol * normb)) ? 1.0 : 0.0;
}
__device__ inline void block_max3_of(const double* __restrict__ p0, int n0, const double* __restrict__ p1, int n1,
                                     const double* __restrict__ p2, int n2, double (&out)[3], double (*sh)[4])
{
    double v[3] = {0.0, 0.0, 0.0};
    constexpr int kTrips = (kNormParts + 1 + 255) / 256;
    double t[3][kTrips];
#pragma unroll
    for (int k = 0; k < kTrips; ++k) {
        const int i = (int)threadIdx.x + 256 * k;
        t[0][k] = (p0 && i < n0) ? p0[i] : 0.0;
        t[1][k] = (p1 && i < n1) ? p1[i] : 0.0;
        t[2][k] = (p2 && i < n2) ? p2[i] : 0.0;
    }
#pragma unroll
// ... 763 lines not shown
{
    extern __shared__ __attribute__((aligned(16))) double smem[];
    const int tid = threadIdx.x;
    const int c = C.psd_list[blockIdx.x];
    const int k = C.psd_dim[c], off = C.off[c], kk = k * k, t = k * (k + 1) / 2;
    double* X = smem;
    double* Am = smem + kk;
    double* Tm = smem + 2 * kk;
    const double is2 = 0.70710678118654752440;
    const double* A = S.psdA + C.psd_aoff[c];
    for (int idx = tid; idx < kk; idx += 256) Am[idx] = A[idx];
    for (int idx = tid; idx < t; idx += 256) {
        int r, cl;
        svec_index(idx, r, cl);
        const double v = x[off + idx];
        if (r == cl) X[r + cl * k] = v;
        else X[r + cl * k] = X[cl + r * k] = v * is2;
    }
    __syncthreads();
    for (int idx = tid; idx < kk; idx += 256) {
        const int r = idx % k, cl = idx / k;
        double acc = 0.0;
        for (int q = 0; q < k; ++q) acc = fma(X[r + q * k], Am[q + cl * k], acc);
        Tm[idx] = acc;
    }
    __syncthreads();
    for (int idx = tid; idx < t; idx += 256) {
        int r, cl;
        svec_index(idx, r, cl);
        double a1 = 0.0, a2 = 0.0;
        for (int q = 0; q < k; ++q) { a1 = fma(Am[r + q * k], Tm[q + cl * k], a1); a2 = fma(Am[cl + q * k], Tm[q + r * k], a2); }
        const double v = (r == cl) ? a1 : (a1 + a2) * is2;
        y[off + idx] = addend ? -(v + addend[off + idx]) : v;
    }
}

void launch_cone_scaling(const ConeDev& C, const ConeState& S, const double* s, const double* z, int m,
                         hipStream_t st)
{
    const int ge = m > 0 ? grid_for(m, 256) : 0, gs = (C.nsoc + 3) / 4;
    const int gx = (C.nexp + 255) / 256, gp = (C.npow + 255) / 256;
    const int gg = (C.ngp_small + 3) / 4 + C.ngp_big;
    if (gx + gp + gg > 0)
        hipLaunchKernelGGL(k_cone_scaling_ns, dim3(ge + gs + gx + gp + gg), dim3(256), 0, st, C, S, s, z, m, ge, gs, gx, gp);
    else if (ge + gs > 0) hipLaunchKernelGGL(k_cone_scaling, dim3(ge + gs), dim3(256), 0, st, C, S, s, z, m, ge);
    if (C.npsd > 0) {
        static PerDeviceOnce once;
        once.run([]() { return set_max_lds(k_cone_psd, 150 * 1024); });
        const size_t lds = (size_t)6 * C.psd_kmax * C.psd_kmax * sizeof(double);
        hipLaunchKernelGGL(k_cone_psd, dim3(C.npsd), dim3(256), lds, st, C, S, s, z);
    }
}

__device__ inline void mul_Hs_elementwise_body(const ConeDev& C, const ConeState& S, double* __restrict__ y,
                                               const double* __restrict__ x, int m, const double* __restrict__ addend, int bx, int nb)
{
    for (int i = bx * 256 + threadIdx.x; i < m; i += nb * 256) {
        const int kind = C.kind[C.elem_cone[i]];
        double v;
        if (kind == 0) v = 0.0;
        else if (kind == 1) v = S.w[i] * (S.w[i] * x[i]);
        else if (kind == 4 || kind == 5) {
            const int c = C.elem_cone[i], off = C.off[c], r = i - off;
            const double* Hs = S.Hs + C.boff[c];
            auto at = [&](int a, int b) { return a <= b ? Hs[b * (b + 1) / 2 + a] : Hs[a * (a + 1) / 2 + b]; };
            v = at(r, 0) * x[off] + at(r, 1) * x[off + 1] + at(r, 2) * x[off + 2];
        }
        else continue;
        y[i] = addend ? -(v + addend[i]) : v;
    }
}
__device__ inline void mul_Hs_soc_body(const ConeDev& C, const ConeState& S, double* __restrict__ y,
                                       const double* __restrict__ x, const double* __restrict__ addend, int ci, int lane)
{
    const int c = C.soc_list[ci];
    const int off = C.off[c], n = C.numel[c];
    const double* w = S.w + off;
    double dot = 0.0;
    for (int i = lane; i < n; i += 64) dot += w[i] * x[off + i];
    dot = 2.0 * wave_sum(dot);
    const double e2 = S.eta[c] * S.eta[c];
    for (int i = lane; i < n; i += 64) {
        const double xi = x[off + i];
        const double v = ((i == 0 ? -xi : xi) + dot * w[i]) * e2;
        y[off + i] = addend ? -(v + addend[off + i]) : v;
    }
}
__device__ inline void publish_record(const Publish& P)
{
    for (int i = 0; i < P.n; ++i) P.dst[i] = P.rec[i];
    P.dst[P.n] = P.seq;
    for (int i = 0; i < P.nzero; ++i) P.rec[i] = 0.0;
}
__global__ void k_publish(Publish P) { if (blockIdx.x == 0 && threadIdx.x == 0) publish_record(P); }
void launch_publish(const Publish& p, hipStream_t st)
{
    if (p.dst) hipLaunchKernelGGL(k_publish, dim3(1), dim3(64), 0, st, p);
}
__global__ __launch_bounds__(256) void k_mul_Hs(ConeDev C, ConeState S, double* __restrict__ y, const double* __restrict__ x,
                                                int m, const double* __restrict__ addend, int ge, Publish P)
{
    if (P.dst && blockIdx.x == gridDim.x - 1 && threadIdx.x == 255) publish_record(P);
    if ((int)blockIdx.x < ge) { mul_Hs_elementwise_body(C, S, y, x, m, addend, blockIdx.x, ge); return; }
    const int ci = ((int)blockIdx.x - ge) * 4 + (int)(threadIdx.x >> 6);
    if (ci < C.nsoc) mul_Hs_soc_body(C, S, y, x, addend, ci, threadIdx.x & 63);
}
__global__ __launch_bounds__(256) void k_mul_Hs_gp(ConeDev C, ConeState S, double* __restrict__ y, const double* __restrict__ x,
                                                   int m, const double* __restrict__ addend, int ge, int gs, Publish P)
{
    __shared__ double sh[12];
    if (P.dst && blockIdx.x == gridDim.x - 1 && threadIdx.x == 255) publish_record(P);
    const int bx = (int)blockIdx.x;
    if (bx < ge) { mul_Hs_elementwise_body(C, S, y, x, m, addend, bx, ge); return; }
    if (bx < ge + gs) {
        const int ci = (bx - ge) * 4 + (int)(threadIdx.x >> 6);
        if (ci < C.nsoc) mul_Hs_soc_body(C, S, y, x, addend, ci, threadIdx.x & 63);
        return;
    }
    const int gq = (C.ngp_small + 3) / 4, b0 = bx - ge - gs;
    if (b0 < gq) {
        const int i = b0 * 4 + (int)(threadIdx.x >> 6);
        if (i < C.ngp_small) mul_Hs_genpow_body<64>(C, S, y, x, addend, C.gp_small[i], threadIdx.x & 63, nullptr);
        return;
    }
    mul_Hs_genpow_body<256>(C, S, y, x, addend, C.gp_big[b0 - gq], threadIdx.x, sh);
}
__global__ __launch_bounds__(256) void k_psd_A_from_R(ConeDev C, ConeState S)
{
    const int c = C.psd_list[blockIdx.x];
    const int k = C.psd_dim[c];
    const double* R = S.psdR + C.psd_aoff[c];
    double* A = S.psdA + C.psd_aoff[c];
    for (int idx = threadIdx.x; idx < k * k; idx += 256) {
        const int r = idx % k, cl = idx / k;
        double acc = 0.0;
        for (int q = 0; q < k; ++q) acc = fma(R[r + q * k], R[cl + q * k], acc);
        A[idx] = acc;
    }
}
void launch_psd_A_from_R(const ConeDev& C, const ConeState& S, hipStream_t st)
{
    if (C.npsd > 0) hipLaunchKernelGGL(k_psd_A_from_R, dim3(C.npsd), dim3(256), 0, st, C, S);
}

__global__ void k_hs_from_w_elementwise(ConeDev C, ConeState S, int m)
{
    for (int i = blockIdx.x * blockDim.x + threadIdx.x; i < m; i += gridDim.x * blockDim.x) {
        const int c = C.elem_cone[i];
        const int kind = C.kind[c];
        if (kind == 0) S.Hs[C.boff[c] + (i - C.off[c])] = 0.0;
        else if (kind == 1) { const double w = S.w[i]; S.Hs[C.boff[c] + (i - C.off[c])] = w * w; }
    }
}
__global__ __launch_bounds__(64) void k_soc_from_w(ConeDev C, ConeState S)
{
    const int c = C.soc_list[blockIdx.x];
    const int off = C.off[c], n = C.numel[c];
    const int lane = threadIdx.x;
    const double* w = S.w + off;
    double w1sqn = 0.0;
    for (int i = 1 + lane; i < n; i += 64) { const double wi = w[i]; w1sqn += wi * wi; }
    w1sqn = wave_sum(w1sqn);
    const double w0n = w[0];
    const double eta = S.eta[c];
    const double eta2 = eta * eta;
    double* Hs = S.Hs + C.boff[c];
    const int sidx = C.sidx[c];
    if (sidx >= 0) {
        const double alpha = 2.0 * w0n;
// ... 34 lines not shown
    __syncthreads();
    double* Hs = S.Hs + C.boff[c];
    const double s2 = 1.41421356237309504880;
    const int nh = t * (t + 1) / 2;
    for (int e = tid; e < nh; e += 256) {
        int row, col;
        svec_index(e, row, col);
        int i, j, kq, l;
        svec_index(row, i, j);
        svec_index(col, kq, l);
        double v;
        const bool ij = (i == j), kl = (kq == l);
        if (!ij && !kl) v = Am[i + kq * k] * Am[j + l * k] + Am[i + l * k] * Am[j + kq * k];
        else if (ij && !kl) v = s2 * Am[j + l * k] * Am[j + kq * k];
        else if (!ij && kl) v = s2 * Am[i + l * k] * Am[j + kq * k];
        else v = Am[j + l * k] * Am[j + l * k];
        Hs[e] = v;
    }
}
void launch_cone_from_scaling(const ConeDev& C, const ConeState& S, int m, hipStream_t st)
{
    if (m > 0) hipLaunchKernelGGL(k_hs_from_w_elementwise, dim3(grid_for(m, 256)), dim3(256), 0, st, C, S, m);
    if (C.nsoc > 0) hipLaunchKernelGGL(k_soc_from_w, dim3(C.nsoc), dim3(64), 0, st, C, S);
    if (C.npsd > 0) {
        hipLaunchKernelGGL(k_psd_A_from_R, dim3(C.npsd), dim3(256), 0, st, C, S);
        const size_t lds = (size_t)C.psd_kmax * C.psd_kmax * sizeof(double);
        hipLaunchKernelGGL(k_psd_hs_from_A, dim3(C.npsd), dim3(256), lds, st, C, S);
    }
}
void launch_mul_Hs(const ConeDev& C, const ConeState& S, double* y, const double* x, int m, hipStream_t st, const double* addend,
                   const Publish& pub)
{
    const int ge = m > 0 ? grid_for(m, 256) : 0, gs = (C.nsoc + 3) / 4;
    const bool ride = ge + gs > 0 && C.npsd == 0;
    const int gg = (C.ngp_small + 3) / 4 + C.ngp_big;
    if (gg > 0)
        hipLaunchKernelGGL(k_mul_Hs_gp, dim3(ge + gs + gg), dim3(256), 0, st, C, S, y, x, m, addend, ge, gs, ride ? pub : Publish{});
    else if (ge + gs > 0) hipLaunchKernelGGL(k_mul_Hs, dim3(ge + gs), dim3(256), 0, st, C, S, y, x, m, addend, ge, ride ? pub : Publish{});
    if (C.npsd > 0) {
        const size_t lds = (size_t)3 * C.psd_kmax * C.psd_kmax * sizeof(double);
        hipLaunchKernelGGL(k_mul_Hs_psd, dim3(C.npsd), dim3(256), lds, st, C, S, y, x, addend);
    }
    if (!ride) launch_publish(pub, st);
}

}


namespace hipkkt {

__device__ inline void sys_offset_elementwise_body(const ConeDev& C, const ConeState& S, double* __restrict__ konst,
                                                   double* __restrict__ workz, const double* __restrict__ ds,
                                                   const double* __restrict__ z, const double* __restrict__ rhs_z, int m,
                                                   int affine, int bx, int nb)
{
    for (int i = bx * 256 + threadIdx.x; i < m; i += nb * 256) {
        double o;
        if (affine) {
            o = ds[i];
        } else {
            const int kind = C.kind[C.elem_cone[i]];
            if (kind == 0) o = 0.0;
            else if (kind == 1) o = ds[i] / z[i];
            else if (kind >= 4) o = ds[i];
            else continue;
        }
        konst[i] = o;
        workz[i] = o - rhs_z[i];
    }
}

__device__ inline void sys_offset_soc_body(const ConeDev& C, const ConeState& S, double* __restrict__ konst,
                                           double* __restrict__ workz, const double* __restrict__ ds,
                                           const double* __restrict__ z, const double* __restrict__ rhs_z, int ci, int lane)
{
    const int c = C.soc_list[ci];
    const int off = C.off[c], n = C.numel[c];
    const double* dsc = ds + off;
    const double* zc = z + off;
    const double* w = S.w + off;
    const double* lam = S.lam + off;
    double zz = 0.0, l1d1 = 0.0, w1d1 = 0.0;
    for (int i = 1 + lane; i < n; i += 64) {
        zz += zc[i] * zc[i];
        l1d1 += lam[i] * dsc[i];
        w1d1 += w[i] * dsc[i];
    }
    zz = sqrt(wave_sum(zz));
    l1d1 = wave_sum(l1d1);
    w1d1 = wave_sum(w1d1);
    const double z0 = zc[0];
    const double resz = (z0 - zz) * (z0 + zz);
    const double eta = S.eta[c];
    const double cc = (lam[0] * dsc[0] - l1d1) / resz;
    const double linv = 1.0 / lam[0];
    const double wfac = w1d1 / (1.0 + w[0]);
    for (int i = lane; i < n; i += 64) {
        double o;
        if (i == 0) o = z0 * cc + eta * w1d1;
        else o = -zc[i] * cc + eta * (dsc[i] + wfac * w[i]);
        o *= linv;
        konst[off + i] = o;
        workz[off + i] = o - rhs_z[off + i];
    }
}

__global__ __launch_bounds__(256) void k_sys_offset_psd(ConeDev C, ConeState S, double* __restrict__ konst,
                                                       double* __restrict__ workz, const double* __restrict__ ds,
                                                       const double* __restrict__ rhs_z)
{
    extern __shared__ __attribute__((aligned(16))) double smem[];
    const int tid = threadIdx.x;
    const int c = C.psd_list[blockIdx.x];
    const int k = C.psd_dim[c], off = C.off[c], kk = k * k, t = k * (k + 1) / 2;
    double* X = smem;
    double* Rm = smem + kk;
    double* Tm = smem + 2 * kk;
    const double is2 = 0.70710678118654752440;
    const double* R = S.psdR + C.psd_aoff[c];
    const double* lam = S.lam + off;
    for (int idx = tid; idx < kk; idx += 256) Rm[idx] = R[idx];
    for (int idx = tid; idx < t; idx += 256) {
        int r, cl;
        svec_index(idx, r, cl);
        const double v = ds[off + idx] * (r == cl ? 1.0 : is2) * 2.0 / (lam[r] + lam[cl]);
        X[r + cl * k] = v;
        X[cl + r * k] = v;
    }
    __syncthreads();
    for (int idx = tid; idx < kk; idx += 256) {
        const int r = idx % k, cl = idx / k;
        double acc = 0.0;
        for (int q = 0; q < k; ++q) acc = fma(X[r + q * k], Rm[cl + q * k], acc);
        Tm[idx] = acc;
    }
    __syncthreads();
    for (int idx = tid; idx < t; idx += 256) {
        int r, cl;
        svec_index(idx, r, cl);
        double a1 = 0.0, a2 = 0.0;
        for (int q = 0; q < k; ++q) { a1 = fma(Rm[r + q * k], Tm[q + cl * k], a1); a2 = fma(Rm[cl + q * k], Tm[q + r * k], a2); }
        const double o = (r == cl) ? a1 : (a1 + a2) * is2;
        konst[off + idx] = o;
        workz[off + idx] = o - rhs_z[off + idx];
    }
}

__global__ __launch_bounds__(256) void k_sys_offset(ConeDev C, ConeState S, double* __restrict__ konst, double* __restrict__ workz,
                                                    const double* __restrict__ ds, const double* __restrict__ z,
                                                    const double* __restrict__ rhs_z, int m, int affine, int ge)
{
    if ((int)blockIdx.x < ge) { sys_offset_elementwise_body(C, S, konst, workz, ds, z, rhs_z, m, affine, blockIdx.x, ge); return; }
    const int ci = ((int)blockIdx.x - ge) * 4 + (int)(threadIdx.x >> 6);
    if (ci < C.nsoc) sys_offset_soc_body(C, S, konst, workz, ds, z, rhs_z, ci, threadIdx.x & 63);
}
bool launch_sys_offset(const ConeDev& C, const ConeState& S, double* konst, double* workz, const double* ds,
                       const double* z, const double* rhs_z, int m, bool affine, hipStream_t st)
{
    if (m <= 0) return true;
    if (!affine && C.npsd > 0) {
        static PerDeviceOnce once;
        once.run([]() { return set_max_lds(k_sys_offset_psd, 150 * 1024); });
        const size_t lds = (size_t)3 * C.psd_kmax * C.psd_kmax * sizeof(double);
        hipLaunchKernelGGL(k_sys_offset_psd, dim3(C.npsd), dim3(256), lds, st, C, S, konst, workz, ds, rhs_z);
    }
    const int ge = grid_for(m, 256), gs = affine ? 0 : (C.nsoc + 3) / 4;
    hipLaunchKernelGGL(k_sys_offset, dim3(ge + gs), dim3(256), 0, st, C, S, konst, workz, ds, z, rhs_z, m, affine ? 1 : 0, ge);
    return true;
}

__global__ __launch_bounds__(256) void k_P_spmv(SpmvDev A, const double* __restrict__ K, const double* __restrict__ x,
                                                double* __restrict__ y, int n)
{
    const int sub = threadIdx.x & 7;
    for (int row = blockIdx.x * 32 + (threadIdx.x >> 3); row < n; row += gridDim.x * 32) {
        double acc = 0.0;
        const int64_t qend = A.pend ? A.pend[row] : A.ptr[row + 1];
        for (int64_t q = A.ptr[row] + sub; q < qend; q += 8) {
            const int c = A.col[q];
            if (c < n) acc = fma(A.val ? A.val[q] : K[A.vmap[q]], x[c], acc);
        }
#pragma unroll
        for (int o = 4; o > 0; o >>= 1) acc += __shfl_down(acc, o, 8);
        if (sub == 0) y[row] = acc;
    }
}
void launch_P_spmv(const SpmvDev& A, const double* Kval, const double* x, double* y, int n, hipStream_t st)
{
    if (n <= 0) return;
    int g = (n + 31) / 32;
    if (g > 2048) g = 2048;
    hipLaunchKernelGGL(k_P_spmv, dim3(g), dim3(256), 0, st, A, Kval, x, y, n);
}

__global__ __launch_bounds__(256) void k_P_spmv2(SpmvDev A, const double* __restrict__ K, const double* __restrict__ x1,
                                                 const double* __restrict__ x, const double* __restrict__ x2, double tau,
                                                 double* __restrict__ pa, double* __restrict__ pb,
                                                 double* __restrict__ xm_out, double* __restrict__ pc, int n)
{
    const int sub = threadIdx.x & 7;
    for (int row = blockIdx.x * 32 + (threadIdx.x >> 3); row < n; row += gridDim.x * 32) {
        double a1 = 0.0, a2 = 0.0, a3 = 0.0;
        const int64_t qend = A.pend ? A.pend[row] : A.ptr[row + 1];
        for (int64_t q = A.ptr[row] + sub; q < qend; q += 8) {
            const int c = A.col[q];
            if (c < n) {
                const double v = A.val ? A.val[q] : K[A.vmap[q]];
                const double x2c = x2[c];
                a1 = fma(v, x1[c], a1);
                a2 = fma(v, x[c] / tau - x2c, a2);
                a3 = fma(v, x2c, a3);
            }
        }
#pragma unroll
        for (int o = 4; o > 0; o >>= 1) { a1 += __shfl_down(a1, o, 8); a2 += __shfl_down(a2, o, 8); a3 += __shfl_down(a3, o, 8); }
        if (sub == 0) {
            pa[row] = a1;
            pb[row] = a2;
            if (pc) pc[row] = a3;
            xm_out[row] = x[row] / tau - x2[row];
// ... 100 lines not shown
                                                          const double* __restrict__ z1, const double* __restrict__ x2,
                                                          const double* __restrict__ z2, const double* __restrict__ partial,
                                                          double* __restrict__ cached, double rhs_tau, double rhs_kappa, double tau,
                                                          double kappa, double* __restrict__ out, int npairs, int n, int m,
                                                          double* __restrict__ keep_x2, double* __restrict__ keep_z2)
{
    __shared__ double d[8];
    __shared__ double sh_dtau;
    const int p = threadIdx.x;
    if (p < npairs) {
        double acc = 0.0;
        for (int i = 0; i < kDotBlocks; ++i) acc += partial[p * kDotBlocks + i];
        d[p] = acc;
    }
    __syncthreads();
    if (p == 0) {
        const double c0 = npairs == 7 ? d[4] : cached[0], c1 = npairs == 7 ? d[5] : cached[1], c2 = npairs == 7 ? d[6] : cached[2];
        const double tau_num = rhs_tau - rhs_kappa / tau + d[0] + d[1] + 2.0 * (d[2] / tau);
        double tau_den = kappa / tau - c0 - c1;
        tau_den += d[3] - c2;
        const double dtau = tau_num / tau_den;
        sh_dtau = dtau;
        if (blockIdx.x == 0) {
            if (npairs == 7) { cached[0] = c0; cached[1] = c1; cached[2] = c2; }
            out[0] = dtau;
            out[1] = -(rhs_kappa + kappa * dtau) / tau;
            out[2] = tau_num;
            out[3] = tau_den;
        }
    }
    __syncthreads();
    const double dtau = sh_dtau;
    for (int i = blockIdx.x * blockDim.x + threadIdx.x; i < n + m; i += gridDim.x * blockDim.x) {
        if (i < n) {
            const double v = x2[i];
            dx[i] = x1[i] + dtau * v;
            if (keep_x2) keep_x2[i] = v;
        } else {
            const double v = z2[i - n];
            dz[i - n] = z1[i - n] + dtau * v;
            if (keep_z2) keep_z2[i - n] = v;
        }
    }
}
void launch_dots_sys_step(const DotPairs& P, double* partial, double* cached, double rhs_tau, double rhs_kappa, double tau,
                          double kappa, double* out, double* dx, double* dz, const double* x1, const double* z1, const double* x2,
                          const double* z2, int n, int m, hipStream_t st, double* keep_x2, double* keep_z2)
{
    hipLaunchKernelGGL(k_dots, dim3(kDotBlocks, P.npairs), dim3(256), 0, st, P, partial);
    hipLaunchKernelGGL(k_sys_step_scalars, dim3(grid_for(std::max(n + m, 1), 256)), dim3(256), 0, st, dx, dz, x1, z1, x2, z2,
                       (const double*)partial, cached, rhs_tau, rhs_kappa, tau, kappa, out, P.npairs, n, m, keep_x2, keep_z2);
}

__global__ void k_neg_sum(double* __restrict__ y, const double* __restrict__ a, const double* __restrict__ b, int n)
{
    for (int i = blockIdx.x * blockDim.x + threadIdx.x; i < n; i += gridDim.x * blockDim.x) y[i] = -(a[i] + b[i]);
}
void launch_neg_sum(double* y, const double* a, const double* b, int n, hipStream_t st)
{
    if (n <= 0) return;
    hipLaunchKernelGGL(k_neg_sum, dim3(grid_for(n, 256)), dim3(256), 0, st, y, a, b, n);
}
__global__ void k_neg_copy(double* __restrict__ y, const double* __restrict__ a, int n)
{
    for (int i = blockIdx.x * blockDim.x + threadIdx.x; i < n; i += gridDim.x * blockDim.x) y[i] = -a[i];
}
void launch_neg_copy(double* y, const double* a, int n, hipStream_t st)
{
    if (n <= 0) return;
    hipLaunchKernelGGL(k_neg_copy, dim3(grid_for(n, 256)), dim3(256), 0, st, y, a, n);
}

}


namespace hipkkt {

__device__ inline void atomic_max_nonneg(double* addr, double v)
{
    atomicMax(reinterpret_cast<unsigned long long*>(addr), (unsigned long long)__double_as_longlong(v));
}

__global__ void k_equil_norms(EquilDev E)
{
    const int64_t tot = E.nnzP + E.nnzA;
    for (int64_t j = blockIdx.x * (int64_t)blockDim.x + threadIdx.x; j < tot; j += (int64_t)gridDim.x * blockDim.x) {
        if (j < E.nnzP) {
            const double v = fabs(E.Pval[j]);
            atomic_max_nonneg(E.dwork + E.Pcol[j], v);
            atomic_max_nonneg(E.dwork + E.Prow[j], v);
        } else {
            const int64_t k = j - E.nnzP;
            const double v = fabs(E.Aval[k]);
            atomic_max_nonneg(E.dwork + E.Acol[k], v);
            atomic_max_nonneg(E.ework + E.Arow[k], v);
        }
    }
}
__global__ void k_equil_scalings(EquilDev E, double smin, double smax)
{
    for (int i = blockIdx.x * blockDim.x + threadIdx.x; i < E.n + E.m; i += gridDim.x * blockDim.x) {
        double* w = i < E.n ? E.dwork + i : E.ework + (i - E.n);
        double* cum = i < E.n ? E.d + i : E.e + (i - E.n);
        double v = *w;
        if (v == 0.0) v = 1.0;
        v = 1.0 / sqrt(v);
// ... 303 lines not shown
```

### cuclarabel_amd/csrc/kernels.hpp

```cpp
#pragma once
#include <hip/hip_runtime.h>
#include <cstdint>
#include <mutex>
#include <stdexcept>
#include <string>

namespace hipkkt {

struct HipError : std::runtime_error { using std::runtime_error::runtime_error; };

class PerDeviceOnce {
    std::mutex mu_;
    uint64_t done_[4] = {0, 0, 0, 0};
public:
    template <class F>
    void run(F&& fn)
    {
        int dev = 0;
        if (hipGetDevice(&dev) != hipSuccess || dev < 0 || dev >= 256) throw HipError("hipGetDevice failed");
        std::lock_guard<std::mutex> lk(mu_);
        if (done_[dev >> 6] >> (dev & 63) & 1) return;
        const hipError_t e = fn();
        if (e != hipSuccess) {
            (void)hipGetLastError();
// ... 186 lines not shown
void launch_pull_leaves_multi(const SolveArgs& a, int nrows, int KP, hipStream_t st);
void launch_bwd_multi(const SolveArgs& a, int begin, int count, bool small, int ncmax, int KP, hipStream_t st, bool leaves = false);

struct ChainSeg {
    int begin;
    int nblock, nwave, ntiny;
    int wg0;
    int leaf;
    RecSeg rec;
};
constexpr int kChainMaxSeg = 20;
struct ChainArgs {
    int nseg;
    int lo, hi;
    int* cnt;
    const int* nchild;
    int* done;
    int* abort_word;
    int epoch;
    int lo0, nstamp;
    ChainSeg seg[kChainMaxSeg];
};
void launch_fwd_chain(const SolveArgs& a, const ChainArgs& c, int nwg, size_t lds, hipStream_t st, int nr);
void launch_bwd_chain(const SolveArgs& a, const ChainArgs& c, int nwg, size_t lds, hipStream_t st, int nr);
constexpr int kChainBS = 512;
inline int chain_seg_wgs(const ChainSeg& s) { return s.nblock + (s.nwave + kChainBS / 64 - 1) / (kChainBS / 64) + (s.ntiny + kChainBS / 8 - 1) / (kChainBS / 8); }

void launch_scatter(double* Kval, const int* idx, const double* vals, int64_t n, double scale, hipStream_t st);
void launch_scale(double* Kval, const int* idx, double scale, int64_t n, hipStream_t st);
void launch_soc_columns(double* Kval, const int* mapU, const int* mapV, const int* mapD,
                        const double* u, const double* v, const double* eta2, const int* soc_of_entry,
                        int sparse_len, int nsparse, hipStream_t st);
void launch_regularizer(const double* Kval, const int* diag, int N, double c0, double c1,
                        double* partial, double* eps_out, hipStream_t st);

struct SpmvDev {
    const int64_t* ptr;
    const int* col;
    const int* vmap;
    const double* val;
    const int64_t* pend;
    int N;
    int lanes_per_row;
    int nlong, nchunks;
    const int* long_rows;
    const int64_t* long_chunk_ptr;
    const int64_t* chunk_q;
    double* long_partial;
};
constexpr int kLongRow = 4096;
constexpr int kLongChunk = 2048;
constexpr int kNormParts = 2048;
constexpr int kMaxNormbCols = 4;
void launch_update_values(double* K, const int* mapHs, const double* Hs, int nHs, const int* mapU, const int* mapV,
                          const int* mapD, const double* u, const double* v, const double* eta2, const int* soc_of_entry,
                          int sparse_len, int nsparse, double* fval, const int* kpos, hipStream_t st);
void launch_residual(const SpmvDev& A, const double* Kval, const double* b, const double* x, double* e,
                     double* partial, double* norm_out, hipStream_t st, int nrhs = 1, int64_t ld = 0,
                     const int* flag_in = nullptr, double* flag_out = nullptr, double* normb_out = nullptr);
void launch_norm_inf(const double* v, int n, double* partial, double* out, hipStream_t st, int nrhs = 1,
                     int64_t ld = 0);
void launch_axpby_sum(double* y, const double* a, const double* b, int64_t n, hipStream_t st);
void launch_gather_values(double* val, const double* Kval, const int* vmap, int64_t nnz, hipStream_t st);
void launch_pack_rhs(double* b, const double* rx, const double* rz, int n, int m, int p, hipStream_t st,
                     int nrhs = 1);
void launch_pack_rhs_rm(double* B, const double* rx, const double* rz, int n, int m, int p, int nrhs, int KP, hipStream_t st);
void launch_unpack_lhs_rm(double* lhsx, double* lhsz, const double* X, int n, int m, int nrhs, int KP, hipStream_t st);
void launch_residual_rm(const SpmvDev& A, const double* B, const double* X, double* E, double* partial, double* norm_out,
                        double* normb_out, int KP, hipStream_t st);
void launch_accept_columns_rm(double* X, const double* cand, double* E, const double* E2, const int* mask, int N, int KP,
                              hipStream_t st);
void launch_accept_columns(double* x, const double* cand, double* e, const double* e2, const int* mask, int N,
                           int nrhs, hipStream_t st);
void launch_check_finite(const double* v, int n, int* flag, hipStream_t st);
void launch_unpack_lhs(double* lhsx, double* lhsz, const double* x, int n, int m, hipStream_t st);
struct IrPartials { const double* e0 = nullptr; const double* b0 = nullptr; const double* cand = nullptr; int np = 0; const int* flag_in = nullptr; };
void launch_ir_round(double* state, int state_stride, int r, bool first, double* norme0, double* normb,
                     const double* cand, const double* abort_word, double* x, const double* dx, int n, int nr, double abstol,
                     double reltol, double stop_ratio, int max_iter, double* readback, double* sticky, hipStream_t st,
                     const IrPartials& Q = IrPartials{});
int residual_grid(const SpmvDev& A);
inline bool residual_partials_ok(const SpmvDev& A, int nrhs) { return A.nlong == 0 && nrhs <= kMaxNormbCols; }
void launch_ir_fold(const double* state, int state_stride, int r, int nr, const double* abort_word, double* sticky, hipStream_t st);
void launch_fold_update_status(double* sticky, const double* st4, hipStream_t st);
void launch_fold_flag(double* sticky, const int* flag, hipStream_t st);
void launch_zero_ints(int* p, int n, hipStream_t st);
struct ZeroList {
    int* p[8];
    int n[8];
    int count = 0;
    void add(int* ptr, int len) { if (ptr && len > 0 && count < 8) { p[count] = ptr; n[count] = len; ++count; } }
};
void launch_zero_ints_multi(const ZeroList& Z, hipStream_t st);
void launch_collect_status(double* dst, const double* eps, const int* conefail, const int* flags, hipStream_t st, double* sticky = nullptr);

struct ConeDev {
    int ncones;
    const int* kind;
    const int* off;
    const int* numel;
    const int64_t* boff;
    const int* sidx;
    const int* soff;
    const int* elem_cone;
    const int* soc_list;
    int nsoc;
    const int* psd_list;
    const int* psd_dim;
    const int64_t* psd_aoff;
    int npsd;
    int psd_kmax;
    const int* exp_list = nullptr;
    const int* pow_list = nullptr;
    const int* ns_index = nullptr;
    const double* param = nullptr;
    int nexp = 0, npow = 0;
    int ns_strategy = 0;
    double ns_mu = 0.0;
    const int* gp_cone = nullptr;
    const int* gp_dim1 = nullptr;
    const int* gp_off = nullptr;
    const double* gp_alpha = nullptr;
    const int* gp_small = nullptr;
    const int* gp_big = nullptr;
    const int* gp_mapP = nullptr;
    const int* gp_mapQR = nullptr;
    const int* gp_mapD = nullptr;
    int ngp_small = 0, ngp_big = 0;
    double gp_mu = 0.0;
};
constexpr int kGenPowWaveMax = 512;
struct ConeState {
    double* w;
    double* lam;
    double* eta;
    double* u;
    double* v;
    double* eta2;
    double* Hs;
    double* psdA;
    double* psdR;
    double* psdRinv;
    int* fail;
    double* ns_grad = nullptr;
    double* ns_H = nullptr;
    double* gp_grad = nullptr;
    double* gp_d = nullptr;
    double* gp_p = nullptr;
    double* gp_qr = nullptr;
    double* Kval = nullptr;
    double* fval = nullptr;
    const int* kpos = nullptr;
};
constexpr int kPsdMaxDim = 48;
void launch_cone_scaling(const ConeDev& C, const ConeState& S, const double* s, const double* z, int m,
                         hipStream_t st);
struct Publish { double* dst = nullptr; double* rec = nullptr; int n = 0, nzero = 0; double seq = 0.0; };
void launch_publish(const Publish& p, hipStream_t st);
void launch_mul_Hs(const ConeDev& C, const ConeState& S, double* y, const double* x, int m, hipStream_t st, const double* addend = nullptr,
                   const Publish& pub = Publish{});
void launch_psd_A_from_R(const ConeDev& C, const ConeState& S, hipStream_t st);
void launch_cone_from_scaling(const ConeDev& C, const ConeState& S, int m, hipStream_t st);

bool launch_sys_offset(const ConeDev& C, const ConeState& S, double* konst, double* workz, const double* ds,
                       const double* z, const double* rhs_z, int m, bool affine, hipStream_t st);
void launch_P_spmv(const SpmvDev& A, const double* Kval, const double* x, double* y, int n, hipStream_t st);
void launch_sys_axpby(double* out, const double* a, const double* alpha_div, const double* b, const double* beta,
                      double beta_host, int n, hipStream_t st);
struct DotPairs { const double* a[8]; const double* b[8]; int len[8]; int npairs; };
void launch_dots(const DotPairs& P, double* partial, double* out, hipStream_t st);
void launch_sys_scalars(const double* dots, const double* cached, const double* scal_in, double* out, hipStream_t st);
void launch_neg_sum(double* y, const double* a, const double* b, int n, hipStream_t st);
void launch_P_spmv2(const SpmvDev& A, const double* Kval, const double* x1, const double* x, const double* x2, double tau,
                    double* pa, double* pb, double* xm_out, double* pc, int n, hipStream_t st);
void launch_pack_rhs_affine(double* b, const double* negq, const double* bb, const double* rhs_x, const double* s,
                            const double* rhs_z, int n, int m, int p, int ncol, hipStream_t st);
void launch_sys_step(double* dx, double* dz, const double* x1, const double* z1, const double* x2, const double* z2,
                     const double* scal, int n, int m, hipStream_t st);
void launch_dots_sys_step(const DotPairs& P, double* partial, double* cached, double rhs_tau, double rhs_kappa, double tau,
                          double kappa, double* out, double* dx, double* dz, const double* x1, const double* z1, const double* x2,
                          const double* z2, int n, int m, hipStream_t st, double* keep_x2 = nullptr, double* keep_z2 = nullptr);
void launch_neg_copy(double* y, const double* a, int n, hipStream_t st);


struct EquilDev {
    int n, m;
    int64_t nnzP, nnzA;
    const int* Prow; const int* Pcol;
    const int* Arow; const int* Acol;
    double* Pval; double* Aval; double* q; double* b;
    double* d; double* e;
    double* dwork; double* ework;
    double* scal;
    double* partial;
};
void launch_equil_round(const EquilDev& E, double scale_min, double scale_max, hipStream_t st);
void launch_equil_rectify(const EquilDev& E, const int* cone_kind, const int* cone_off, const int* cone_numel,
                          const int* elem_cone, int ncones, hipStream_t st);
void launch_lrscale(double* values, const int* row, const int* col, int64_t nnz, const double* L, const double* R,
                    double cscale, hipStream_t st);

}
```

### cuclarabel_amd/csrc/knobs.hpp

```cpp
#pragma once
#include <cstdlib>

namespace hipkkt {

#define HIPKKT_KNOBS(KNOB, FLAG_SET, FLAG_ON)                                                                                         \
                                                                                                                 \
    KNOB(int, verbose, "HIPKKT_VERBOSE", 0)                  \
    FLAG_SET(stamps, "HIPKKT_STAMPS")                                    \
    KNOB(int, top_stamps, "HIPKKT_TOP_STAMPS", 0)            \
    KNOB(int, top_stamps_nr, "HIPKKT_TOP_STAMPS_NR", 1)                                       \
    FLAG_SET(dump_levels, "HIPKKT_DUMP_LEVELS")                                \
    FLAG_SET(dump_subtrees, "HIPKKT_DUMP_SUBTREES")                        \
                                                                                      \
    KNOB(double, nd_sep_ratio, "HIPKKT_ND_SEP_RATIO", 0.10)  \
    KNOB(int, nd_sep_min, "HIPKKT_ND_SEP_MIN", 5000)                                           \
    KNOB(long long, panel_cap, "HIPKKT_PANEL_CAP", -1)       \
    KNOB(int, panel_max_cols, "HIPKKT_PANEL_MAX_COLS", -1)                                                  \
    KNOB(int, panel_slice_below, "HIPKKT_PANEL_SLICE_BELOW", -1)  \
    FLAG_SET(postorder_layout, "HIPKKT_POSTORDER_LAYOUT")                       \
    FLAG_ON(upd_pingpong, "HIPKKT_UPD_PINGPONG")                                        \
    KNOB(int, bundle_kids, "HIPKKT_BUNDLE_KIDS", 200)        \
    KNOB(int, bundle_kids_panel, "HIPKKT_BUNDLE_KIDS_PANEL", 400)   \
    FLAG_ON(bundle_cost, "HIPKKT_BUNDLE_COST")               \
                                                                                                  \
    KNOB(int, merge_small, "HIPKKT_MERGE_SMALL", 128)        \
    KNOB(int, slice_rows, "HIPKKT_SLICE_ROWS", 128)            \
    FLAG_ON(slice_fit, "HIPKKT_SLICE_FIT")                                    \
    KNOB(int, bs128_count, "HIPKKT_BS128_COUNT", 1024)                                 \
    KNOB(int, bs128_f, "HIPKKT_BS128_F", 128)                         \
    KNOB(int, solve_tall_rows, "HIPKKT_SOLVE_TALL_ROWS", 0)  \
    KNOB(int, tall_block_rows, "HIPKKT_TALL_BLOCK_ROWS", 256)  \
    FLAG_ON(dense_child, "HIPKKT_DENSE_CHILD")               \
    KNOB(int, tile_xcd, "HIPKKT_TILE_XCD", 150)              \
    FLAG_ON(pull_leaves, "HIPKKT_PULL_LEAVES")                   \
    FLAG_ON(packed, "HIPKKT_PACKED")                            \
    KNOB(long long, packed_max_mb, "HIPKKT_PACKED_MAX_MB", 4096)                       \
                                                                                                               \
    FLAG_SET(graph, "HIPKKT_GRAPH")                               \
    FLAG_SET(no_overlap, "HIPKKT_NO_OVERLAP")                                                         \
    KNOB(int, winv_tail, "HIPKKT_WINV_TAIL", 4)                \
    KNOB(int, winv_early, "HIPKKT_WINV_EARLY", 1)                                                   \
    KNOB(int, winv_blocks, "HIPKKT_WINV_BLOCKS", 0)                           \
    FLAG_ON(winv_split, "HIPKKT_WINV_SPLIT")                 \
    FLAG_ON(winv_run_forks, "HIPKKT_WINV_RUN_FORKS")                        \
    FLAG_ON(factor_overlap, "HIPKKT_FACTOR_OVERLAP")                 \
    FLAG_SET(ov_cu_mask, "HIPKKT_OV_CU_MASK")                                        \
    KNOB(long long, ov_test_limit, "HIPKKT_OV_TEST_LIMIT", 5000000)   \
    KNOB(int, ov_max_fronts, "HIPKKT_OV_MAX_FRONTS", 0)      \
    KNOB(int, ov_max_tiles, "HIPKKT_OV_MAX_TILES", 1600)     \
    KNOB(int, ov_merge, "HIPKKT_OV_MERGE", 100)                   \
    KNOB(int, ov_merge_wide, "HIPKKT_OV_MERGE_WIDE", 24)                     \
    KNOB(int, ov_merge_groups, "HIPKKT_OV_MERGE_GROUPS", 8)                                \
    KNOB(int, schur_pipe_tiles, "HIPKKT_SCHUR_PIPE_TILES", 1600)                     \
    KNOB(int, schur_pipe_nc, "HIPKKT_SCHUR_PIPE_NC", 64)            \
                                                                                                                      \
    FLAG_SET(no_top, "HIPKKT_NO_TOP")                                                            \
    KNOB(int, top_tall, "HIPKKT_TOP_TALL", -1)                                        \
    KNOB(int, top_cap, "HIPKKT_TOP_CAP", 1 << 30)                                        \
    KNOB(double, top_mult, "HIPKKT_TOP_MULT", 1.5)                            \
    KNOB(long long, top_test_limit, "HIPKKT_TOP_TEST_LIMIT", 5000000)  \
    FLAG_SET(no_level_merge, "HIPKKT_NO_LEVEL_MERGE")               \
    KNOB(int, solve_slice_kb, "HIPKKT_SOLVE_SLICE_KB", 80)                                  \
    KNOB(int, solve_slice_max, "HIPKKT_SOLVE_SLICE_MAX", 64)                                     \
    KNOB(long long, solve_slice_from, "HIPKKT_SOLVE_SLICE_FROM", -1)  \
    FLAG_ON(chain, "HIPKKT_CHAIN")                                                           \
    FLAG_ON(chain_top, "HIPKKT_CHAIN_TOP")                   \
    KNOB(int, chain_max, "HIPKKT_CHAIN_MAX", 640)                                             \
    FLAG_SET(test_publish_fail, "HIPKKT_TEST_PUBLISH_FAIL")  \
    KNOB(int, multi_vec, "HIPKKT_MULTI_VEC", 4)                                    \
    KNOB(int, multi_ct, "HIPKKT_MULTI_CT", 0)

struct Knobs {
#define HIPKKT_K_FIELD(type, field, name, dflt) type field = dflt;
#define HIPKKT_K_FLAG(field, name) bool field = false;
#define HIPKKT_K_FLAGON(field, name) bool field = true;
    HIPKKT_KNOBS(HIPKKT_K_FIELD, HIPKKT_K_FLAG, HIPKKT_K_FLAGON)
#undef HIPKKT_K_FIELD
#undef HIPKKT_K_FLAG
#undef HIPKKT_K_FLAGON
    static void get(int& v, const char* e) { v = std::atoi(e); }
    static void get(long long& v, const char* e) { v = std::atoll(e); }
    static void get(double& v, const char* e) { v = std::atof(e); }
    Knobs()
    {
#define HIPKKT_K_READ(type, field, name, dflt) if (const char* e_ = std::getenv(name)) get(field, e_);
#define HIPKKT_K_READF(field, name) field = std::getenv(name) != nullptr;
#define HIPKKT_K_READON(field, name) if (const char* e_ = std::getenv(name)) field = std::atoi(e_) != 0;
        HIPKKT_KNOBS(HIPKKT_K_READ, HIPKKT_K_READF, HIPKKT_K_READON)
#undef HIPKKT_K_READ
// ... 13 lines not shown
```

### cuclarabel_amd/csrc/solve_common.hpp

```cpp
#pragma once
#include "kernels.hpp"

namespace hipkkt {

__device__ inline double readlane_f64(double v, int lane)
{
    const int lo = __builtin_amdgcn_readlane(__double2loint(v), lane);
    const int hi = __builtin_amdgcn_readlane(__double2hiint(v), lane);
    return __hiloint2double(hi, lo);
}

template <int CTRL, int ROW_MASK>
__device__ __forceinline__ double dpp_add_step(double v)
{
    const int lo = __builtin_amdgcn_update_dpp(0, __double2loint(v), CTRL, ROW_MASK, 0xf, false);
    const int hi = __builtin_amdgcn_update_dpp(0, __double2hiint(v), CTRL, ROW_MASK, 0xf, false);
    return v + __hiloint2double(hi, lo);
}
__device__ inline double group8_sum(double v)
{
    v = dpp_add_step<0xB1, 0xf>(v);
    v = dpp_add_step<0x4E, 0xf>(v);
    v = dpp_add_step<0x141, 0xf>(v);
    return v;
}
__device__ inline double wave_reduce_sum(double v)
{
    v = dpp_add_step<0x111, 0xf>(v);
    v = dpp_add_step<0x112, 0xf>(v);
    v = dpp_add_step<0x114, 0xf>(v);
    v = dpp_add_step<0x118, 0xf>(v);
    v = dpp_add_step<0x142, 0xa>(v);
    v = dpp_add_step<0x143, 0xc>(v);
    return readlane_f64(v, 63);
}

template <int NR>
__device__ inline void ldv(const double* __restrict__ base, int64_t i, double (&out)[NR])
{
    if constexpr (NR == 1) out[0] = base[i];
    else if constexpr (NR == 2) {
        const double2 t = *reinterpret_cast<const double2*>(base + 2 * i);
        out[0] = t.x; out[1] = t.y;
    } else {
        static_assert(NR == 4, "1, 2 or 4 right-hand sides");
        const double4 t = *reinterpret_cast<const double4*>(base + 4 * i);
        out[0] = t.x; out[1] = t.y; out[2] = t.z; out[3] = t.w;
    }
}
template <int NR>
__device__ inline void stv(double* __restrict__ base, int64_t i, const double (&v)[NR])
{
    if constexpr (NR == 1) base[i] = v[0];
    else if constexpr (NR == 2) *reinterpret_cast<double2*>(base + 2 * i) = make_double2(v[0], v[1]);
    else *reinterpret_cast<double4*>(base + 4 * i) = make_double4(v[0], v[1], v[2], v[3]);
}

constexpr int kItemsInFlight = 2;
__device__ inline double lds_sum_strided(const double* p, int n, int stride)
{
    double v = 0.0;
    int k = 0;
    for (; k + 8 <= n; k += 8) {
        double t[8];
#pragma unroll
        for (int q = 0; q < 8; ++q) t[q] = p[(k + q) * stride];
#pragma unroll
        for (int q = 0; q < 8; ++q) v += t[q];
    }
    double t[8];
#pragma unroll
    for (int q = 0; q < 8; ++q) t[q] = (k + q < n) ? p[(k + q) * stride] : 0.0;
#pragma unroll
    for (int q = 0; q < 8; ++q) if (k + q < n) v += t[q];
    return v;
}

struct ItemRegs { double m[8]; };
__device__ inline void item_apply(const ItemRegs& R, const double* v, int Rn, int Kn, double* part, int ldp, int it,
                                  int nrb, int lane)
{
    const int ks = it / nrb, rb = it - ks * nrb;
    const int r = rb * 64 + lane, k0 = 8 * ks;
    double acc = 0.0;
#pragma unroll
    for (int q = 0; q < 8; ++q) acc = fma(R.m[q], (k0 + q < Kn) ? v[k0 + q] : 0.0, acc);
    if (r < Rn) part[ks * ldp + r] = acc;
// ... 166 lines not shown
```

### cuclarabel_amd/csrc/solve_kernels.hip

```cpp
#include "kernels.hpp"
#include "knobs.hpp"
#include "solve_common.hpp"
#include <algorithm>
#include <cstdlib>

namespace hipkkt {


struct FrontLoc { int c0, nc, nb; int64_t rp, mat; };
__device__ __forceinline__ FrontLoc front_loc(const SolveHdr& h) { return FrontLoc{h.c0, h.nc, h.nb, h.rp, h.mat_off}; }

template <int NR>
__device__ __forceinline__ void fwd_wave_body(const SolveArgs& A, const RecSeg& R, int begin, int count, int bx, bool leaf = false)
{
    const int lane = threadIdx.x & 63;
    const int wv = __builtin_amdgcn_readfirstlane((int)(threadIdx.x >> 6));
    const int item = bx * (int)(blockDim.x >> 6) + wv;
    if (item >= count) return;
    const TreeDev& T = A.T;
    FrontLoc L;
    int pi = 0;
    RowGather G;
    G.cnt = 0;
    if (const char* rec = rec_of(A, R, 1, item)) {
// ... 45 lines not shown
    const int lane = threadIdx.x & 63;
    const int wv = __builtin_amdgcn_readfirstlane((int)(threadIdx.x >> 6));
    const int item = bx * (int)(blockDim.x >> 6) + wv;
    if (item >= count) return;
    const TreeDev& T = A.T;
    FrontLoc L;
    int idx = 0;
    if (const char* rec = rec_of(A, R, 1, item)) {
        const SolveHdr h = *reinterpret_cast<const SolveHdr*>(rec);
        idx = rec_idx(rec, lane);
        L = front_loc(h);
    } else {
        const FrontDesc fd = T.desc[begin + item];
        L = FrontLoc{fd.c0, fd.nc, fd.nb, fd.rp, fd.front_off};
        idx = (lane < L.nc) ? T.perm[L.c0 + lane] : ((lane < L.nc + L.nb) ? T.rows[L.rp + lane - L.nc] : 0);
    }
    const int c0 = L.c0, nc = L.nc, nb = L.nb;
    const int f = nc + nb;
    const double* __restrict__ F = A.fronts + L.mat;

    double y[NR];
    {
        const double di = (lane < nc) ? A.Dinv[c0 + lane] : 0.0;
#pragma unroll
        for (int c = 0; c < NR; ++c) y[c] = 0.0;
        if (lane < f) ldv<NR>(A.xp, lane < nc ? c0 + lane : idx, y);
        if (lane < nc) {
#pragma unroll
            for (int c = 0; c < NR; ++c) y[c] *= di;
        }
    }
    for (int j1 = nc; j1 > 0; j1 -= 8) {
        double lv[8];
#pragma unroll
        for (int q = 0; q < 8; ++q) {
            const int j = j1 - 1 - q;
            lv[q] = (j >= 0 && lane > j && lane < f) ? F[lane + (int64_t)j * f] : 0.0;
        }
#pragma unroll
        for (int q = 0; q < 8; ++q) {
            const int j = j1 - 1 - q;
            if (j >= 0) {
#pragma unroll
                for (int c = 0; c < NR; ++c) {
                    const double sum = wave_reduce_sum(lv[q] * y[c]);
                    if (lane == j) y[c] -= sum;
                }
            }
        }
    }
    if (lane < nc) {
        stv<NR>(A.xp, c0 + lane, y);
#pragma unroll
        for (int c = 0; c < NR; ++c) A.out[c * A.ld_out + idx] = y[c];
    }
}

constexpr int kTinyFront = 8;
template <int NR>
__device__ __forceinline__ void fwd_tiny_body(const SolveArgs& A, const RecSeg& R, int begin, int count, int bx, bool leaf = false)
{
    const int sub = threadIdx.x & 7;
    const int item = bx * (int)(blockDim.x >> 3) + (threadIdx.x >> 3);
    const bool live = item < count;
    const TreeDev& T = A.T;
    FrontLoc L;
    int pi = 0;
    RowGather G;
    G.cnt = 0;
    if (const char* rec = rec_of(A, R, 2, live ? item : count - 1)) {
        const SolveHdr* h = reinterpret_cast<const SolveHdr*>(rec);
        L = FrontLoc{h->c0, h->nc, h->nb, h->rp, h->mat_off};
        pi = rec_idx(rec, sub);
        if (!leaf) G = rec_gather(rec, R.fmax[2], sub);
    } else {
        const FrontDesc fd = T.desc[begin + (live ? item : count - 1)];
        L = FrontLoc{fd.c0, fd.nc, fd.nb, fd.rp, fd.front_off};
        pi = (sub < L.nc) ? T.perm[L.c0 + sub] : 0;
        if (!leaf && sub < L.nc + L.nb) G = row_gather_lists(T, (int64_t)L.c0 + L.rp + sub);
    }
    const int c0 = L.c0, nc = L.nc, nb = L.nb;
    const int64_t rp = L.rp;
    const int f = nc + nb;
    const double* __restrict__ F = A.fronts + L.mat;
    double y[NR];
#pragma unroll
    for (int c = 0; c < NR; ++c) y[c] = (sub < nc) ? A.b[c * A.ld_b + pi] : 0.0;
    if (!leaf && sub < f) gather_add<NR, false>(A, G, y);
    double lv[kTinyFront];
#pragma unroll
    for (int k = 0; k < kTinyFront; ++k) lv[k] = (k < nc && sub > k && sub < f) ? F[sub + k * f] : 0.0;
#pragma unroll
    for (int k = 0; k < kTinyFront; ++k) {
#pragma unroll
        for (int c = 0; c < NR; ++c) {
            const double yk = __shfl(y[c], k, 8);
            if (k < nc) y[c] = fma(-lv[k], yk, y[c]);
        }
    }
    if (live) {
        if (sub < nc) stv<NR>(A.xp, c0 + sub, y);
        else if (sub < f) stv<NR>(A.uvec, rp + sub - nc, y);
    }
}
template <int NR>
__device__ __forceinline__ void bwd_tiny_body(const SolveArgs& A, const RecSeg& R, int begin, int count, int bx)
{
    const int sub = threadIdx.x & 7;
    const int item = bx * (int)(blockDim.x >> 3) + (threadIdx.x >> 3);
    const bool live = item < count;
    const TreeDev& T = A.T;
    FrontLoc L;
    int idx = 0;
    if (const char* rec = rec_of(A, R, 2, live ? item : count - 1)) {
        const SolveHdr* h = reinterpret_cast<const SolveHdr*>(rec);
        L = FrontLoc{h->c0, h->nc, h->nb, h->rp, h->mat_off};
        idx = rec_idx(rec, sub);
    } else {
        const FrontDesc fd = T.desc[begin + (live ? item : count - 1)];
        L = FrontLoc{fd.c0, fd.nc, fd.nb, fd.rp, fd.front_off};
        idx = (sub < L.nc) ? T.perm[L.c0 + sub] : ((sub < L.nc + L.nb) ? T.rows[L.rp + sub - L.nc] : 0);
    }
    const int c0 = L.c0, nc = L.nc, nb = L.nb;
    const int f = nc + nb;
    const double* __restrict__ F = A.fronts + L.mat;
    double y[NR];
    {
        const double di = (sub < nc) ? A.Dinv[c0 + sub] : 0.0;
#pragma unroll
        for (int c = 0; c < NR; ++c) y[c] = 0.0;
        if (sub < f) ldv<NR>(A.xp, sub < nc ? c0 + sub : idx, y);
        if (sub < nc) {
#pragma unroll
            for (int c = 0; c < NR; ++c) y[c] *= di;
        }
    }
    double lv[kTinyFront];
#pragma unroll
    for (int j = 0; j < kTinyFront; ++j) lv[j] = (j < nc && sub > j && sub < f) ? F[sub + j * f] : 0.0;
#pragma unroll
    for (int j = kTinyFront - 1; j >= 0; --j) {
#pragma unroll
        for (int c = 0; c < NR; ++c) {
            const double sum = group8_sum(lv[j] * y[c]);
            if (j < nc && sub == j) y[c] -= sum;
        }
    }
    if (live && sub < nc) {
        stv<NR>(A.xp, c0 + sub, y);
#pragma unroll
        for (int c = 0; c < NR; ++c) A.out[c * A.ld_out + idx] = y[c];
    }
}
template <int NR>
__global__ __launch_bounds__(256) void k_fwd_small(SolveArgs A, RecSeg R, int begin, int nwave, int ntiny, int leaf)
{
    const int nwb = (nwave + 3) >> 2;
    if ((int)blockIdx.x < nwb) fwd_wave_body<NR>(A, R, begin, nwave, blockIdx.x, leaf != 0);
    else fwd_tiny_body<NR>(A, R, begin + nwave, ntiny, blockIdx.x - nwb, leaf != 0);
}
template <int NR>
__global__ __launch_bounds__(256) void k_bwd_small(SolveArgs A, RecSeg R, int begin, int nwave, int ntiny)
{
    const int nwb = (nwave + 3) >> 2;
    if ((int)blockIdx.x < nwb) bwd_wave_body<NR>(A, R, begin, nwave, blockIdx.x);
    else bwd_tiny_body<NR>(A, R, begin + nwave, ntiny, blockIdx.x - nwb);
}


template <int BS, int NR>
__device__ __forceinline__ void fwd_block_body(const SolveArgs& A, const RecSeg& R, int begin, int bx)
{
    extern __shared__ __attribute__((aligned(16))) double smem[];
    const int tid = threadIdx.x, lane = tid & 63;
    const int wv = __builtin_amdgcn_readfirstlane(tid >> 6);
    constexpr int NW = BS / 64;
    const TreeDev& T = A.T;
    const char* rec = rec_of(A, R, 0, bx);
    FrontLoc L;
    int pi = 0;
    RowGather G;
    G.cnt = 0;
    if (rec) {
        const SolveHdr h = *reinterpret_cast<const SolveHdr*>(rec);
        if (tid < R.fmax[0]) { pi = rec_idx(rec, tid); G = rec_gather(rec, R.fmax[0], tid); }
        L = front_loc(h);
    } else {
        const FrontDesc fd = T.desc[begin + bx];
        L = FrontLoc{fd.c0, fd.nc, fd.nb, fd.rp, fd.w_off};
        if (tid < L.nc + L.nb) {
            pi = (tid < L.nc) ? T.perm[L.c0 + tid] : 0;
            G = row_gather_lists(T, (int64_t)L.c0 + L.rp + tid);
        }
    }
    const int c0 = L.c0, nc = L.nc, nb = L.nb;
    const int64_t rp = L.rp;
    const int f = nc + nb;
    const double* __restrict__ W = A.tinv + L.mat;
    const int fpad = (f + 3) & ~3;
    const int nks = (nc + 7) >> 3, nrb = (f + 63) >> 6;
    const int cst = (1 + nks) * fpad;
    double* y = smem;
    double* part = lds_part<NR>(smem, fpad);

// ... 109 lines not shown

template <int BS, int NR>
__device__ __forceinline__ void bwd_block_body(const SolveArgs& A, const RecSeg& R, int begin, int bx)
{
    extern __shared__ __attribute__((aligned(16))) double smem[];
    const int tid = threadIdx.x, lane = tid & 63;
    const int wv = __builtin_amdgcn_readfirstlane(tid >> 6);
    constexpr int NW = BS / 64;
    const TreeDev& T = A.T;
    const char* rec = rec_of(A, R, 0, bx);
    FrontLoc L;
    int idx = 0;
    if (rec) {
        const SolveHdr h = *reinterpret_cast<const SolveHdr*>(rec);
        if (tid < R.fmax[0]) idx = rec_idx(rec, tid);
        L = front_loc(h);
    } else {
        const FrontDesc fd = T.desc[begin + bx];
        L = FrontLoc{fd.c0, fd.nc, fd.nb, fd.rp, fd.w_off};
        if (tid < L.nc + L.nb) idx = (tid < L.nc) ? T.perm[L.c0 + tid] : T.rows[L.rp + tid - L.nc];
    }
    const int c0 = L.c0, nc = L.nc, nb = L.nb;
    const int64_t rp = L.rp;
    const int f = nc + nb;
    const double* __restrict__ Wt = A.tinv + L.mat + (int64_t)f * nc;
    const int fpad = (f + 3) & ~3, ncpad = (nc + 3) & ~3;
    const int nrs = (f + 7) >> 3;
    const int cst = fpad + nrs * ncpad;
    double* z = smem;
    double* part = lds_part<NR>(smem, fpad);

    BwdBatch first;
    bwd_load_items(first, Wt, nc, f, wv, NW, lane);
    for (int i = tid; i < f; i += BS) {
        const double di = (i < nc) ? A.Dinv[c0 + i] : 0.0;
        int ri = idx;
        if (i != tid && i >= nc) ri = rec ? rec_idx(rec, i) : T.rows[rp + i - nc];
        double w[NR];
        ldv<NR>(A.xp, i < nc ? c0 + i : ri, w);
#pragma unroll
        for (int c = 0; c < NR; ++c) z[lds_ix<NR>(c, cst, i)] = (i < nc) ? w[c] * di : -w[c];
    }
    __syncthreads();
    bwd_items<NR>(first, Wt, nc, f, z, part, ncpad, cst, wv, NW, lane);
    __syncthreads();
    for (int j = tid; j < nc; j += BS) {
        const int pi = j == tid ? idx : (rec ? rec_idx(rec, j) : T.perm[c0 + j]);
        double w[NR];
        const double2 vp = lds_sum_pair<NR>(part, j, nrs, ncpad);
#pragma unroll
        for (int c = 0; c < NR; ++c) {
            const double v = lds_sum_col<NR>(vp, part, cst, c, j, nrs, ncpad);
            w[c] = v;
            A.out[c * A.ld_out + pi] = v;
        }
        stv<NR>(A.xp, c0 + j, w);
    }
}
template <int BS, int NR>
__global__ __launch_bounds__(BS) void k_bwd_block(SolveArgs A, RecSeg R, int begin)
{
    bwd_block_body<BS, NR>(A, R, begin, blockIdx.x);
}
template <int BS, int NR>
__global__ __launch_bounds__(BS) void k_fwd_level(SolveArgs A, RecSeg R, int begin, int nblock, int nwave, int ntiny)
{
    const int bx = blockIdx.x, nwb = (nwave + BS / 64 - 1) / (BS / 64);
    if (bx < nblock) fwd_block_body<BS, NR>(A, R, begin, bx);
    else if (bx < nblock + nwb) fwd_wave_body<NR>(A, R, begin + nblock, nwave, bx - nblock);
    else fwd_tiny_body<NR>(A, R, begin + nblock + nwave, ntiny, bx - nblock - nwb);
}
template <int BS, int NR>
__global__ __launch_bounds__(BS) void k_bwd_level(SolveArgs A, RecSeg R, int begin, int nblock, int nwave, int ntiny)
{
    const int bx = blockIdx.x, nwb = (nwave + BS / 64 - 1) / (BS / 64);
    if (bx < nblock) bwd_block_body<BS, NR>(A, R, begin, bx);
    else if (bx < nblock + nwb) bwd_wave_body<NR>(A, R, begin + nblock, nwave, bx - nblock);
    else bwd_tiny_body<NR>(A, R, begin + nblock + nwave, ntiny, bx - nblock - nwb);
}


template <int BS, int kTopPF, int kTopPB, int NR>
__global__ __launch_bounds__(BS, BS == 1024 ? 4 : 2) void k_top_solve(SolveArgs A, int begin, int* flags, int epoch, int ntop, int nflag)
{
    extern __shared__ __attribute__((aligned(16))) double smem[];
    __shared__ int sh_ok;
    const int tid = threadIdx.x, lane = tid & 63;
    const int wv = __builtin_amdgcn_readfirstlane(tid >> 6);
    constexpr int NW = BS / 64;
    const TreeDev& T = A.T;
    const int me = blockIdx.x, G = gridDim.x;
    int* flag_f = flags;
    int* flag_b = flags + nflag;
    int* abort_word = flags + 2 * nflag;
    const long long t0 = wall_clock64();
    const long long limit = A.top_limit;

#define TOP_STAMP(dir, slot) do { if (A.top_stamps && tid == 0) A.top_stamps[((int64_t)(dir) * ntop + pos) * 8 + (slot)] = wall_clock64(); } while (0)
    int pos = me;
    for (; pos < ntop; pos += G) {
        TOP_STAMP(0, 0);
        const FrontDesc fd = T.desc[begin + pos];
        const int s = fd.s, c0 = fd.c0, nc = fd.nc, nb = fd.nb;
        const int64_t rp = fd.rp;
        const int f = nc + nb;
        const double* __restrict__ W = A.tinv + fd.w_off;
        const int fpad = (f + 3) & ~3;
// ... 193 lines not shown
            const int it = wv + p * NW;
            if constexpr (NR == 2) {
                if (it < nitB) item_apply_cols<NR>(rbk[p], z, cst, nc, f, part, ncpad, it, ncb, lane);
            } else if (it < nitB) {
                const int rs = it / ncb, cb = it - rs * ncb;
                const int j = cb * 64 + lane, r0 = 8 * rs;
#pragma unroll
                for (int c = 0; c < NR; ++c) {
                    double acc = 0.0;
#pragma unroll
                    for (int q = 0; q < 8; ++q) acc = fma(rbk[p].m[q], (r0 + q < f) ? z[c * cst + r0 + q] : 0.0, acc);
                    if (j < nc) part[c * cst + rs * ncpad + j] = acc;
                }
            }
        }
        for (int it0 = wv + kTopPB * NW; it0 < nitB; it0 += 3 * NW) {
            double m[3][8];
#pragma unroll
            for (int u = 0; u < 3; ++u) {
                const int it = it0 + u * NW;
                const int rs = it / ncb, cb = it - rs * ncb;
                const int j = cb * 64 + lane, r0 = 8 * rs;
                const bool live = it < nitB && !(r0 + 7 < cb * 64);
#pragma unroll
                for (int q = 0; q < 8; ++q) m[u][q] = (live && j < nc && r0 + q < f) ? Wt[j + (int64_t)(r0 + q) * nc] : 0.0;
            }
#pragma unroll
            for (int u = 0; u < 3; ++u) {
                const int it = it0 + u * NW;
                if constexpr (NR == 2) {
                    if (it < nitB) item_apply2(m[u], z, nc, f, part, ncpad, it, ncb, lane);
                } else if (it < nitB) {
                    const int rs = it / ncb, cb = it - rs * ncb;
                    const int j = cb * 64 + lane, r0 = 8 * rs;
#pragma unroll
                    for (int c = 0; c < NR; ++c) {
                        double acc = 0.0;
#pragma unroll
                        for (int q = 0; q < 8; ++q) acc = fma(m[u][q], (r0 + q < f) ? z[c * cst + r0 + q] : 0.0, acc);
                        if (j < nc) part[c * cst + rs * ncpad + j] = acc;
                    }
                }
            }
        }
        __syncthreads();
        TOP_STAMP(1, 4);
        for (int j = tid; j < nc; j += BS) {
            const int pi = j == tid ? ridx : T.perm[c0 + j];
            const double2 vp = lds_sum_pair<NR>(part, j, nrs, ncpad);
#pragma unroll
            for (int c = 0; c < NR; ++c) {
                const double v = lds_sum_col<NR>(vp, part, cst, c, j, nrs, ncpad);
                ST_AGENT_F64(A.xp + (int64_t)(c0 + j) * NR + c, v);
                A.out[c * A.ld_out + pi] = v;
            }
        }
        asm volatile("s_waitcnt vmcnt(0)" ::: "memory");
        __syncthreads();
        TOP_STAMP(1, 5);
        if (tid == 0) __hip_atomic_store(flag_b + pos, epoch, __ATOMIC_RELAXED, __HIP_MEMORY_SCOPE_AGENT);
    }
}
#undef TOP_STAMP

constexpr int kBdColsSolveMax = 160;
constexpr int kSlPF = 2;
constexpr int kSlGP = 4;
__device__ inline bool wait_children_tasks(const TreeDev& T, const int* __restrict__ tbase, int s, int begin, int pos0, int* flag,
                                           int epoch, int* abort_word, long long t0, long long limit, int lane)
{
    bool ok = true;
    const int ce1 = T.child_ptr[s + 1];
    for (int e0 = T.child_ptr[s]; e0 < ce1; e0 += 64) {
        int a = 0, b = 0;
        if (e0 + lane < ce1) {
            const int cp = T.spos[T.child_idx[e0 + lane]] - begin;
            if (cp >= pos0) { a = tbase[cp]; b = tbase[cp + 1]; }
        }
        if (b > a) ok = wait_flag(flag + a, epoch, abort_word, t0, limit) && ok;
        unsigned long long more = __ballot(b - a > 1);
        while (more) {
            const int c = __ffsll((long long)more) - 1;
            more &= more - 1;
            const int ca = __builtin_amdgcn_readlane(a, c), cb = __builtin_amdgcn_readlane(b, c);
            for (int q = ca + 1 + lane; q < cb; q += 64) ok = wait_flag(flag + q, epoch, abort_word, t0, limit) && ok;
        }
    }
    return ok;
}
__device__ inline bool wait_parent_tasks(const TreeDev& T, const int* __restrict__ tbase, int s, int begin, int* flag, int epoch,
                                         int* abort_word, long long t0, long long limit, int lane)
{
    bool ok = true;
    const int par = T.sn_parent[s];
    if (par >= 0) {
        const int pp = T.spos[par] - begin;
        for (int q = tbase[pp] + lane; q < tbase[pp + 1]; q += 64) ok = wait_flag(flag + q, epoch, abort_word, t0, limit) && ok;
    }
    return ok;
}

template <int GPB, int NR>
__device__ inline void gather_rest_nr(const TreeDev& T, const double* uvec, int64_t g, int64_t g1, double (&v)[NR])
{
    for (; g < g1; g += GPB) {
        int src[GPB];
        double u[NR][GPB];
// ... 402 lines not shown
            for (int p = 0; p < 4; ++p) {
                const int it = wv + p * NW;
                if constexpr (NR == 2) {
                    if (it < nitB) item_apply_cols<NR>(rbk[p], z, cst, nc, f, part, ncpad, it, ncb, lane);
                } else if (it < nitB) {
                    const int rs = it / ncb, cb = it - rs * ncb;
                    const int j = cb * 64 + lane, r0 = 8 * rs;
    #pragma unroll
                    for (int c = 0; c < NR; ++c) {
                        double acc = 0.0;
    #pragma unroll
                        for (int q = 0; q < 8; ++q) acc = fma(rbk[p].m[q], (r0 + q < f) ? z[c * cst + r0 + q] : 0.0, acc);
                        if (j < nc) part[c * cst + rs * ncpad + j] = acc;
                    }
                }
            }
            for (int it0 = wv + 4 * NW; it0 < nitB; it0 += 3 * NW) {
                double m[3][8];
    #pragma unroll
                for (int u = 0; u < 3; ++u) {
                    const int it = it0 + u * NW;
                    const int rs = it / ncb, cb = it - rs * ncb;
                    const int j = cb * 64 + lane, r0 = 8 * rs;
                    const bool live = it < nitB && !(r0 + 7 < cb * 64);
    #pragma unroll
                    for (int q = 0; q < 8; ++q) m[u][q] = (live && j < nc && r0 + q < f) ? Wt[j + (int64_t)(r0 + q) * nc] : 0.0;
                }
    #pragma unroll
                for (int u = 0; u < 3; ++u) {
                    const int it = it0 + u * NW;
                    if constexpr (NR == 2) {
                        if (it < nitB) item_apply2(m[u], z, nc, f, part, ncpad, it, ncb, lane);
                    } else if (it < nitB) {
                        const int rs = it / ncb, cb = it - rs * ncb;
                        const int j = cb * 64 + lane, r0 = 8 * rs;
    #pragma unroll
                        for (int c = 0; c < NR; ++c) {
                            double acc = 0.0;
    #pragma unroll
                            for (int q = 0; q < 8; ++q) acc = fma(m[u][q], (r0 + q < f) ? z[c * cst + r0 + q] : 0.0, acc);
                            if (j < nc) part[c * cst + rs * ncpad + j] = acc;
                        }
                    }
                }
            }
            __syncthreads();
            for (int j = tid; j < nc; j += BS) {
                const int pi = T.perm[c0 + j];
                const double2 vp = lds_sum_pair<NR>(part, j, nrs, ncpad);
    #pragma unroll
                for (int c = 0; c < NR; ++c) {
                    const double v = lds_sum_col<NR>(vp, part, cst, c, j, nrs, ncpad);
                    ST_AGENT_F64(A.xp + (int64_t)(c0 + j) * NR + c, v);
                    A.out[c * A.ld_out + pi] = v;
                }
            }
            asm volatile("s_waitcnt vmcnt(0)" ::: "memory");
            __syncthreads();
            SL_STAMP(1, 5);
            if (tid == 0) __hip_atomic_store(flag_b + tk, epoch, __ATOMIC_RELAXED, __HIP_MEMORY_SCOPE_AGENT);

            continue;
        }
        const FrontDesc fd = T.desc[begin + pos];
        const int s = fd.s, c0 = fd.c0, nc = fd.nc, nb = fd.nb;
        const int64_t rp = fd.rp;
        const int f = nc + nb;
        const double* __restrict__ W = A.tinv + fd.w_off;
        const int csz = (nc + R - 1) / R;
        const int j0 = sl * csz, ncl = max(0, min(csz, nc - j0));
        const int fpad = (f + 3) & ~3;
        const int cst = fpad + NW * 16;
        double* z = smem;
        double* part = smem + fpad;
        const int nrb = (f + 63) >> 6;
        constexpr int CW = 8;
        double pm[CW];
        {
            const int r = wv * 64 + lane;
#pragma unroll
            for (int c = 0; c < CW; ++c) pm[c] = (c < ncl && r < f) ? W[r + (int64_t)(j0 + c) * f] : 0.0;
        }
        int ridx[2] = {-1, -1};
        double dinv[2] = {0.0, 0.0};
#pragma unroll
        for (int x = 0; x < 2; ++x) {
            const int i = tid + x * BS;
            if (i < nc) dinv[x] = A.Dinv[c0 + i];
            else if (i < f) ridx[x] = T.rows[rp + i - nc];
        }
        if (tid == 0) sh_ok = 1;
        __syncthreads();
        if (wv == 0) {
            if (!wait_parent_tasks(T, A.tbase, s, begin, flag_b, epoch, abort_word, t0, limit, lane)) sh_ok = 0;
        }
        __syncthreads();
        if (!sh_ok) return;
        SL_STAMP(1, 2);
        {
            double zv[2][NR];
#pragma unroll
            for (int x = 0; x < 2; ++x) {
                const int i = tid + x * BS;
#pragma unroll
                for (int c = 0; c < NR; ++c)
                    zv[x][c] = (i < nc) ? LD_AGENT_F64(A.xf + (int64_t)(c0 + i) * NR + c)
                                        : (i < f ? LD_AGENT_F64(A.xp + (int64_t)ridx[x] * NR + c) : 0.0);
// ... 4 lines not shown
#pragma unroll
                for (int c = 0; c < NR; ++c)
                    if (i < f) z[c * cst + i] = (i < nc) ? zv[x][c] * dinv[x] : -zv[x][c];
            }
        }
#pragma unroll
        for (int c = 0; c < NR; ++c)
            for (int i = tid + 2 * BS; i < f; i += BS)
                z[c * cst + i] = (i < nc) ? LD_AGENT_F64(A.xf + (int64_t)(c0 + i) * NR + c) * A.Dinv[c0 + i]
                                          : -LD_AGENT_F64(A.xp + (int64_t)T.rows[rp + i - nc] * NR + c);
        __syncthreads();
        for (int cc = 0; cc < ncl; cc += CW) {
            const int ncc = min(CW, ncl - cc);
            double acc[NR][CW];
#pragma unroll
            for (int b = 0; b < NR; ++b)
#pragma unroll
                for (int c = 0; c < CW; ++c) acc[b][c] = 0.0;
            int x = 0;
            for (int rb = wv; rb < nrb; rb += NW, ++x) {
                const int r = rb * 64 + lane;
                double zl[NR];
#pragma unroll
                for (int b = 0; b < NR; ++b) zl[b] = r < f ? z[b * cst + r] : 0.0;
                if (cc == 0 && x == 0) {
#pragma unroll
                    for (int b = 0; b < NR; ++b)
#pragma unroll
                        for (int c = 0; c < CW; ++c) acc[b][c] = fma(pm[c], zl[b], acc[b][c]);
                } else {
                    double m[CW];
#pragma unroll
                    for (int c = 0; c < CW; ++c) m[c] = (c < ncc && r < f) ? W[r + (int64_t)(j0 + cc + c) * f] : 0.0;
#pragma unroll
                    for (int b = 0; b < NR; ++b)
#pragma unroll
                        for (int c = 0; c < CW; ++c) acc[b][c] = fma(m[c], zl[b], acc[b][c]);
                }
            }
#pragma unroll
            for (int b = 0; b < NR; ++b)
#pragma unroll
                for (int c = 0; c < CW; ++c) {
                    const double sum = wave_reduce_sum(acc[b][c]);
                    if (lane == 0) part[b * cst + wv * 16 + c] = sum;
                }
            __syncthreads();
            if (tid < ncc * NR) {
                const int b = tid / ncc, jj = tid - b * ncc;
                double v = 0.0;
                for (int w = 0; w < NW; ++w) v += part[b * cst + w * 16 + jj];
                const int j = j0 + cc + jj;
                ST_AGENT_F64(A.xp + (int64_t)(c0 + j) * NR + b, v);
                A.out[b * A.ld_out + T.perm[c0 + j]] = v;
            }
            __syncthreads();
        }
        asm volatile("s_waitcnt vmcnt(0)" ::: "memory");
        __syncthreads();
        SL_STAMP(1, 5);
            if (tid == 0) __hip_atomic_store(flag_b + tk, epoch, __ATOMIC_RELAXED, __HIP_MEMORY_SCOPE_AGENT);
    }
}
#undef SL_STAMP

constexpr int kWinvThreads = 512;
constexpr int kWinvSmallThreads = 128, kWinvSmallNc = 32;
template <int NT>
__device__ inline void winv_one(const TreeDev& T, const double* __restrict__ fronts, double* __restrict__ wst, int s,
                                double* smem)
{
    typedef double d4_t __attribute__((ext_vector_type(4)));
    constexpr int NWV = NT / 64;
    const int tid = threadIdx.x;
    const int lane = tid & 63, wvi = tid >> 6;
    const int ml = lane & 15, mk = lane >> 4;
    const int c0 = T.sn_start[s];
    const int nc = T.sn_start[s + 1] - c0;
    const int nb = (int)(T.rowptr[s + 1] - T.rowptr[s]);
    const int f = nc + nb;
    const double* __restrict__ F = fronts + T.front_off[s];
    double* __restrict__ W = wst + T.tinv_off[s];
    const int ld = nc | 1;
    const int nblk = (nc + 15) >> 4;
    double* Ls = smem;
#define WK(i, c) Ls[(c) * ld + (i)]
    for (int idx = tid; idx < nc * nc; idx += NT) {
        const int k = idx / nc, i = idx - k * nc;
        if (i > k) Ls[i * ld + k] = F[i + (int64_t)k * f];
    }
    __syncthreads();
    {
        for (int item = tid; item < nblk * 16; item += NT) {
            const int b = item >> 4, j = item & 15;
            const int o = 16 * b, w = min(16, nc - o);
            if (j >= w) continue;
            double t[16];
#pragma unroll
            for (int i = 0; i < 16; ++i) t[i] = 0.0;
#pragma unroll
            for (int i = 1; i < 16; ++i) {
                if (i > j && i < w) {
                    double acc = Ls[(o + i) * ld + o + j];
#pragma unroll
                    for (int k = 1; k < 16; ++k)
                        if (k > j && k < i) acc = fma(Ls[(o + i) * ld + o + k], t[k], acc);
                    t[i] = -acc;
// ... 189 lines not shown
            A.xp[c0 + i] = acc;
        }
        return;
    }
    for (int r = r0 + tid; r < r1; r += 1024) {
        const int64_t lc = (int64_t)c0 + rp + r;
        double v = 0.0;
        for (int64_t g = T.gl_ptr[lc]; g < T.gl_ptr[lc + 1]; ++g) v += A.uvec[T.gl_src[g]];
        double acc = 0.0;
        for (int k = 0; k < nc; ++k) acc = fma(W[r + (int64_t)k * f], ytop[k], acc);
        A.uvec[rp + r - nc] = v - acc;
    }
}
__global__ __launch_bounds__(1024) void k_bwd_tall(SolveArgs A, int begin, int BR, int N)
{
    extern __shared__ __attribute__((aligned(16))) double zloc[];
    __shared__ int sh_last;
    const int tid = threadIdx.x, lane = tid & 63, wv = tid >> 6;
    const TreeDev& T = A.T;
    const FrontDesc fd = T.desc[begin + blockIdx.y];
    const int c0 = fd.c0, nc = fd.nc, nb = fd.nb;
    const int64_t rp = fd.rp;
    const int f = nc + nb;
    const int r0 = (int)blockIdx.x * BR, r1 = min(f, r0 + BR);
    if (r0 >= f) return;
    const double* __restrict__ W = A.tinv + fd.w_off;
    for (int r = r0 + tid; r < r1; r += 1024)
        zloc[r - r0] = (r < nc) ? A.xp[c0 + r] * A.Dinv[c0 + r] : -A.xp[T.rows[rp + r - nc]];
    __syncthreads();
    double* front_part = A.tall_ws + N + (int64_t)blockIdx.y * gridDim.x * kBdColsSolveMax;
    double* part = front_part + (int64_t)blockIdx.x * kBdColsSolveMax;
    for (int j = wv; j < nc; j += 16) {
        double acc = 0.0;
        const double* __restrict__ Wj = W + (int64_t)j * f;
        for (int r = max(r0, j) + lane; r < r1; r += 64) acc = fma(Wj[r], zloc[r - r0], acc);
        acc = wave_reduce_sum(acc);
        if (lane == 0) ST_AGENT_F64(part + j, acc);
    }
    asm volatile("s_waitcnt vmcnt(0)" ::: "memory");
    __syncthreads();
    const int nb_used = (f + BR - 1) / BR;
    int* ticket = reinterpret_cast<int*>(A.tall_ws) + fd.s;
    if (tid == 0) {
        const int t = __hip_atomic_fetch_add(ticket, 1, __ATOMIC_RELAXED, __HIP_MEMORY_SCOPE_AGENT);
        sh_last = (t == nb_used - 1);
        if (sh_last) __hip_atomic_store(ticket, 0, __ATOMIC_RELAXED, __HIP_MEMORY_SCOPE_AGENT);
    }
    __syncthreads();
    if (!sh_last) return;
    for (int j = tid; j < nc; j += 1024) {
        double v = 0.0;
        for (int bx = j / BR; bx < nb_used; ++bx) v += LD_AGENT_F64(front_part + (int64_t)bx * kBdColsSolveMax + j);
        A.xp[c0 + j] = v;
        A.out[T.perm[c0 + j]] = v;
    }
}
static int tall_block_rows()
{
    const int br = knobs().tall_block_rows;
    return br < 64 ? 64 : (br > 4096 ? 4096 : (br & ~63));
}
size_t tall_ws_doubles(int N, int ntall, int fmax)
{
    const int BR = tall_block_rows();
    return (size_t)N + (size_t)ntall * (size_t)((fmax + BR - 1) / BR) * kBdColsSolveMax;
}
void launch_fwd_tall(const SolveArgs& a, int begin, int count, int fmax, hipStream_t st)
{
    if (count <= 0) return;
    const int BR = tall_block_rows();
    hipLaunchKernelGGL(k_fwd_tall, dim3(1 + (fmax + BR - 1) / BR, count), dim3(1024), 0, st, a, begin, BR);
}
void launch_bwd_tall(const SolveArgs& a, int begin, int count, int fmax, int N, hipStream_t st)
{
    if (count <= 0) return;
    const int BR = tall_block_rows();
    const int nblk = (fmax + BR - 1) / BR;
    hipLaunchKernelGGL(k_bwd_tall, dim3(nblk, count), dim3(1024), (size_t)BR * sizeof(double), st, a, begin, BR, N);
}

size_t solve_lds_bytes(int fmax, int ncmax)
{
    const size_t fpad = (size_t)((fmax + 3) & ~3), ncpad = (size_t)((ncmax + 3) & ~3);
    const size_t nks = (size_t)((ncmax + 7) >> 3), nrs = (size_t)((fmax + 7) >> 3);
    const size_t fwd = fpad + nks * fpad, bwd = fpad + nrs * ncpad;
    return (fwd > bwd ? fwd : bwd) * sizeof(double);
}

void launch_fwd(const SolveArgs& a, const RecSeg& rs, int begin, int count, int bs, size_t lds, hipStream_t st, int nr)
{
    if (count <= 0) return;
    init_solve_lds();
    if (bs == 128) HIPKKT_NR_SWITCH(nr, hipLaunchKernelGGL((k_fwd_block<128, NR>), dim3(count), dim3(128), lds * NR, st, a, rs, begin));
    else HIPKKT_NR_SWITCH(nr, hipLaunchKernelGGL((k_fwd_block<kSolveBS, NR>), dim3(count), dim3(kSolveBS), lds * NR, st, a, rs, begin));
}
void launch_fwd_level(const SolveArgs& a, const RecSeg& rs, int begin, int nblock, int nwave, int ntiny, int bs, size_t lds, hipStream_t st, int nr)
{
    init_solve_lds();
    if (bs == 128) {
        const int grid = nblock + (nwave + 1) / 2 + (ntiny + 15) / 16;
        HIPKKT_NR_SWITCH(nr, hipLaunchKernelGGL((k_fwd_level<128, NR>), dim3(grid), dim3(128), lds * NR, st, a, rs, begin, nblock, nwave, ntiny));
    } else {
        const int grid = nblock + (nwave + kSolveBS / 64 - 1) / (kSolveBS / 64) + (ntiny + kSolveBS / 8 - 1) / (kSolveBS / 8);
        HIPKKT_NR_SWITCH(nr, hipLaunchKernelGGL((k_fwd_level<kSolveBS, NR>), dim3(grid), dim3(kSolveBS), lds * NR, st, a, rs, begin, nblock, nwave, ntiny));
    }
}
void launch_bwd_level(const SolveArgs& a, const RecSeg& rs, int begin, int nblock, int nwave, int ntiny, int bs, size_t lds, hipStream_t st, int nr)
// ... 709 lines not shown
```

Before: 315.1.

## Fold small elementwise kernels into neighbors behind HIPKKT_FOLD knob

```diff
diff --git a/cuclarabel_amd/csrc/chain_kernels.hip b/cuclarabel_amd/csrc/chain_kernels.hip
--- a/cuclarabel_amd/csrc/chain_kernels.hip
+++ b/cuclarabel_amd/csrc/chain_kernels.hip
@@ -417,7 +417,7 @@
         for (int c = 0; c < NR; ++c) {
             const double v = lds_sum_col<NR>(vp, part, cst, c, j, nrs, ncpad);
             ST_AGENT_F64(A.xp + (int64_t)(c0 + j) * NR + c, v);
-            A.out[c * A.ld_out + pi] = v;
+            st_out(A, c * A.ld_out + pi, v);
         }
     }
     drain_stores();
@@ -494,7 +494,7 @@
 #pragma unroll
         for (int c = 0; c < NR; ++c) {
             ST_AGENT_F64(A.xp + (int64_t)(c0 + lane) * NR + c, y[c]);
-            A.out[c * A.ld_out + pi] = y[c];
+            st_out(A, c * A.ld_out + pi, y[c]);
         }
     }
     drain_stores();
@@ -553,7 +553,7 @@
 #pragma unroll
         for (int c = 0; c < NR; ++c) {
             ST_AGENT_F64(A.xp + (int64_t)(c0 + sub) * NR + c, y[c]);
-            A.out[c * A.ld_out + pi] = y[c];
+            st_out(A, c * A.ld_out + pi, y[c]);
         }
     }
     drain_stores();
diff --git a/cuclarabel_amd/csrc/hipkkt.hip b/cuclarabel_amd/csrc/hipkkt.hip
--- a/cuclarabel_amd/csrc/hipkkt.hip
+++ b/cuclarabel_amd/csrc/hipkkt.hip
@@ -162,6 +162,7 @@
         }
     }
 
+    const RegFinish* reg_finish = nullptr;
     void factor(const double* d_Kval, const double* d_eps)
     {
         const bool want_stamps = knobs().stamps;
@@ -186,7 +187,8 @@
         HIP_CHECK(hipGraphLaunch(it->second, stream));
     }
 
-    void solve(const double* d_b, double* d_x, bool allow_top = false, int nr = 1, int64_t ldb = 0, int64_t ldx = 0)
+    bool solve(const double* d_b, double* d_x, bool allow_top = false, int nr = 1, int64_t ldb = 0, int64_t ldx = 0,
+               const double* d_add = nullptr)
     {
         const bool no_graph = !knobs().graph;
         if (nr > 1) {
@@ -197,9 +199,9 @@
             const bool waits = allow_top && ((!top_disabled && top_launches > 0) || (!chain_disabled && chain_from < launches.size()));
             const bool tok = waits && claim_dev(kOpS);
             TokenRelease rel{this, tok};
-            enqueue_solve(d_b, d_x, stream, tok, nr, ldb, ldx, tok);
+            enqueue_solve(d_b, d_x, stream, tok, nr, ldb, ldx, tok, d_add);
             if (tok) { rel.on = false; dev_enqueued(true); }
-            return;
+            return true;
         }
         auto key = std::make_pair((const void*)d_b, (const void*)d_x);
         auto it = solve_graphs.find(key);
@@ -215,6 +217,7 @@
             it = solve_graphs.emplace(key, ex).first;
         }
         HIP_CHECK(hipGraphLaunch(it->second, stream));
+        return d_add == nullptr;
     }
     bool supports_nr(int nr) const
     {
@@ -423,7 +426,8 @@
             if (!slice_list.empty()) zl.add(d_ov_sprog.p, (int)slice_list.size());
             zl.add(d_ov_started.p, (int)launches.size());
         }
-        launch_zero_ints_multi(zl, st);
+        if (reg_finish && !side) launch_zero_ints_reg(zl, *reg_finish, st);
+        else launch_zero_ints_multi(zl, st);
         FactorArgs a;
         a.T = tree();
         a.Kval = d_Kval;
@@ -597,7 +601,8 @@
         return g;
     }
 
-    void enqueue_solve(const double* d_b, double* d_x, hipStream_t st, bool use_top, int nr, int64_t ldb, int64_t ldx, bool allow_chain = false)
+    void enqueue_solve(const double* d_b, double* d_x, hipStream_t st, bool use_top, int nr, int64_t ldb, int64_t ldx, bool allow_chain = false,
+                       const double* d_add = nullptr)
     {
         SolveArgs a;
         a.T = tree();
@@ -614,13 +619,14 @@
         a.top_stamps = nullptr;
         bool stamp_now = false;
         a.ld_b = ldb; a.ld_out = ldx; a.ld_xp = S.N; a.ld_uvec = (int64_t)std::max<size_t>(S.rows.size(), 1);
-        a.tk_pos = d_tk_pos.p; a.tk_sl = d_tk_sl.p; a.tbase = d_tbase.p; a.xf = xf.p; a.add = nullptr;
+        a.tk_pos = d_tk_pos.p; a.tk_sl = d_tk_sl.p; a.tbase = d_tbase.p; a.xf = xf.p; a.add = d_add;
         a.chain_cnt = nullptr;
         a.recs = d_recs.p ? reinterpret_cast<const char*>(d_recs.p) : nullptr;
         a.tall_ws = tall_ws.p;
         const bool no_top = knobs().no_top;
         if (nr > 1 && top_ntask > 0 && (no_top || !use_top || top_disabled || top_sgrid2 <= 0)) {
-            for (int c = 0; c < nr; ++c) enqueue_solve(d_b + (int64_t)c * ldb, d_x + (int64_t)c * ldx, st, use_top, 1, 0, 0, allow_chain);
+            for (int c = 0; c < nr; ++c)
+                enqueue_solve(d_b + (int64_t)c * ldb, d_x + (int64_t)c * ldx, st, use_top, 1, 0, 0, allow_chain, d_add ? d_add + (int64_t)c * ldx : nullptr);
             return;
         }
         const size_t nl = launches.size();
@@ -2141,6 +2147,10 @@
     DBuf<double> b, x, e, dx, rx, rz, sbuf, zbuf, ybuf;
     double *cur_x = nullptr, *cur_dx = nullptr;
     DBuf<double> partial, scal;
+    DBuf<int> mapDiagStatic;
+    DBuf<unsigned char> hs_is_diag;
+    DBuf<double> upd_partial, static_max;
+    bool reg_fold = false;
     std::unique_ptr<PinnedScalars> pin;
     DBuf<int> c_kind, c_off, c_numel, c_sidx, c_soff, c_elem, c_soclist;
     DBuf<int64_t> c_boff;
@@ -2543,6 +2553,7 @@
     });
 }
 
+static void kkt_refresh_static_max(hipkkt_kkt_t h);
 int hipkkt_kkt_create(hipkkt_kkt_t* out, int64_t n, int64_t m, const int64_t* Pcolptr, const int64_t* Prowval,
                       const double* Pnzval, const int64_t* Acolptr, const int64_t* Arowval, const double* Anzval,
                       int64_t ncones, const int32_t* kinds, const int64_t* dims, const hipkkt_settings* settings,
@@ -2617,6 +2628,21 @@
         h->mapA.upload(K.mapA);
         h->mapHs.upload(K.mapHs);
         h->mapDiag.upload(K.map_diag);
+        h->reg_fold = knobs().fold && K.ngenpow == 0;
+        if (h->reg_fold) {
+            std::vector<unsigned char> dyn((size_t)K.nnzK, 0), isd(K.mapHs.size(), 0);
+            std::vector<int> stat;
+            for (int e : K.mapHs) dyn[(size_t)e] = 1;
+            for (int e : K.mapD) dyn[(size_t)e] = 1;
+            for (int e : K.map_diag) if (!dyn[(size_t)e]) stat.push_back(e);
+            for (int e : K.map_diag) dyn[(size_t)e] |= 2;
+            for (size_t i = 0; i < K.mapHs.size(); ++i) isd[i] = (dyn[(size_t)K.mapHs[i]] & 2) ? 1 : 0;
+            h->mapDiagStatic.upload(stat);
+            h->hs_is_diag.upload(isd);
+            h->upd_partial.alloc(kUpdateValuesGrid);
+            h->static_max.alloc(1);
+            kkt_refresh_static_max(h.get());
+        }
         h->mapU.upload(K.mapU);
         h->mapV.upload(K.mapV);
         h->mapD.upload(K.mapD);
@@ -2822,22 +2848,34 @@
     });
 }
 
-static int kkt_update_device(hipkkt_kkt_t h, bool deferred = false)
+static void kkt_refresh_static_max(hipkkt_kkt_t h)
+{
+    if (!h->reg_fold) return;
+    launch_regularizer(h->Kval.p, h->mapDiagStatic.p, (int)h->mapDiagStatic.n, 0.0, 1.0, h->upd_partial.p, h->static_max.p, h->stream);
+}
+static int kkt_update_device(hipkkt_kkt_t h, bool deferred = false, bool scaled_here = false)
 {
     KKTAssembly& K = h->K;
     int pu = h->prof.begin(0, h->stream);
-    launch_update_values(h->Kval.p, h->mapHs.p, h->Hs.p, (int)K.nHs, h->mapU.p, h->mapV.p, h->mapD.p, h->soc_u.p, h->soc_v.p,
-                         h->soc_eta2.p, h->soc_of_entry.p, K.sparse_len, K.nsparse, h->fval_dirty ? nullptr : h->fval.p,
-                         h->kpos.p, h->stream);
+    const bool reg = h->st.static_regularization_enable != 0;
+    const bool fold = reg && scaled_here && h->reg_fold && !knobs().graph && !knobs().stamps;
+    const int nparts = launch_update_values(h->Kval.p, h->mapHs.p, h->Hs.p, (int)K.nHs, h->mapU.p, h->mapV.p, h->mapD.p, h->soc_u.p,
+                                            h->soc_v.p, h->soc_eta2.p, h->soc_of_entry.p, K.sparse_len, K.nsparse,
+                                            h->fval_dirty ? nullptr : h->fval.p, h->kpos.p, h->stream,
+                                            fold ? h->hs_is_diag.p : nullptr, fold ? h->upd_partial.p : nullptr);
     const double* eps_ptr = nullptr;
-    if (h->st.static_regularization_enable) {
-        launch_regularizer(h->Kval.p, h->mapDiag.p, K.N, h->st.static_regularization_constant,
-                           h->st.static_regularization_proportional, h->partial.p, h->scal.p, h->stream);
+    RegFinish rf{h->upd_partial.p, nparts, h->static_max.p, h->st.static_regularization_constant,
+                 h->st.static_regularization_proportional, h->scal.p};
+    if (reg) {
+        if (!fold) launch_regularizer(h->Kval.p, h->mapDiag.p, K.N, h->st.static_regularization_constant,
+                                      h->st.static_regularization_proportional, h->partial.p, h->scal.p, h->stream);
         eps_ptr = h->scal.p;
     }
     h->prof.end(pu, h->stream);
     int pf = h->prof.begin(1, h->stream);
+    h->eng->reg_finish = fold ? &rf : nullptr;
     h->eng->factor(h->Kval.p, eps_ptr);
+    h->eng->reg_finish = nullptr;
     h->prof.end(pf, h->stream);
     launch_collect_status(h->scal.p + 8, h->scal.p, h->fail.p, h->eng->flags_ptr(), h->stream, deferred ? h->ir_sticky : nullptr);
     if (deferred) return HIPKKT_OK;
@@ -2893,7 +2931,7 @@
         launch_cone_scaling(h->cone_dev(), h->cone_state(), d_s, d_z, h->K.m, h->stream);
         h->prof.end(pu, h->stream);
         h->scaling_valid = true;
-        return kkt_update_device(h, deferred);
+        return kkt_update_device(h, deferred, true);
     });
 }
 int hipkkt_kkt_update_from_sz_dev(hipkkt_kkt_t h, const double* d_s, const double* d_z)
@@ -2924,6 +2962,7 @@
         if (!k) return HIPKKT_OK;
         HIP_CHECK(hipMemcpyAsync(h->Pval.p, Pnzval, k * sizeof(double), hipMemcpyHostToDevice, h->stream));
         launch_scatter(h->Kval.p, h->mapP.p, h->Pval.p, (int64_t)k, 1.0, h->stream);
+        kkt_refresh_static_max(h);
         h->fval_dirty = true;
         HIP_CHECK(hipStreamSynchronize(h->stream));
         return HIPKKT_OK;
@@ -2939,6 +2978,7 @@
         if (!k) return HIPKKT_OK;
         HIP_CHECK(hipMemcpyAsync(h->Aval.p, Anzval, k * sizeof(double), hipMemcpyHostToDevice, h->stream));
         launch_scatter(h->Kval.p, h->mapA.p, h->Aval.p, (int64_t)k, 1.0, h->stream);
+        kkt_refresh_static_max(h);
         h->fval_dirty = true;
         HIP_CHECK(hipStreamSynchronize(h->stream));
         return HIPKKT_OK;
@@ -2994,11 +3034,12 @@
                     nr > 1 ? (int64_t)h->K.N : 0, h->eng->top_abort_word(), h->scal.p + 3, normb_out);
     h->prof.end(pr, h->stream);
 }
-static void kkt_trisolve(hipkkt_kkt_t h, const double* rhs, double* out, bool allow_top = true, int nr = 1)
+static bool kkt_trisolve(hipkkt_kkt_t h, const double* rhs, double* out, bool allow_top = true, int nr = 1, const double* add = nullptr)
 {
     int ps = h->prof.begin(2, h->stream);
-    h->eng->solve(rhs, out, allow_top, nr, h->K.N, h->K.N);
+    const bool summed = h->eng->solve(rhs, out, allow_top, nr, h->K.N, h->K.N, add);
     h->prof.end(ps, h->stream);
+    return summed;
 }
 
 struct IrNorms { double *norme0, *normb, *cand; };
@@ -3029,8 +3070,8 @@
 }
 static void kkt_enqueue_round(hipkkt_kkt_t h, int r, bool first, bool readback, bool fold, int nr)
 {
-    kkt_trisolve(h, h->e.p, h->dx.p, true, nr);
-    launch_axpby_sum(h->dx.p, h->dx.p, h->x.p, (int64_t)h->K.N * nr, h->stream);
+    if (!kkt_trisolve(h, h->e.p, h->dx.p, true, nr, knobs().fold ? h->x.p : nullptr) || !knobs().fold)
+        launch_axpby_sum(h->dx.p, h->dx.p, h->x.p, (int64_t)h->K.N * nr, h->stream);
     kkt_enqueue_refine_error(h, h->dx.p, kkt_ir_norms(h, nr).cand, nullptr, nr, true);
     kkt_launch_ir(h, r, first, readback, fold, nr);
 }
@@ -3622,9 +3663,15 @@
     P.a[1] = h->sb.p; P.b[1] = z1; P.len[1] = m;
     P.a[2] = d_var_x; P.b[2] = h->spa.p; P.len[2] = n;
     P.a[3] = h->sworkx.p; P.b[3] = h->spb.p; P.len[3] = n;
-    launch_dots_sys_step(P, h->sys_partial.p, h->sys_cached.p, rhs_tau, rhs_kappa, var_tau, var_kappa, h->sys_out_dev, d_lhs_x, d_lhs_z,
-                         x1, z1, x2, z2, n, m, st, with_const ? h->sx2.p : nullptr, with_const ? h->sz2.p : nullptr);
-    launch_mul_Hs(h->cone_dev(), h->cone_state(), d_lhs_s, d_lhs_z, m, st, addend ? addend : h->sconic.p, pub);
+    if (knobs().fold && step_mul_Hs_folds(h->cone_dev(), m)) {
+        StepArgs T{d_lhs_x, d_lhs_z, x1, z1, x2, z2, h->sys_partial.p, h->sys_cached.p, rhs_tau, rhs_kappa, var_tau, var_kappa,
+                   h->sys_out_dev, P.npairs, n, m, with_const ? h->sx2.p : nullptr, with_const ? h->sz2.p : nullptr};
+        launch_dots_sys_step_mul_Hs(P, T, h->cone_dev(), h->cone_state(), d_lhs_s, m, addend ? addend : h->sconic.p, pub, st);
+    } else {
+        launch_dots_sys_step(P, h->sys_partial.p, h->sys_cached.p, rhs_tau, rhs_kappa, var_tau, var_kappa, h->sys_out_dev, d_lhs_x, d_lhs_z,
+                             x1, z1, x2, z2, n, m, st, with_const ? h->sx2.p : nullptr, with_const ? h->sz2.p : nullptr);
+        launch_mul_Hs(h->cone_dev(), h->cone_state(), d_lhs_s, d_lhs_z, m, st, addend ? addend : h->sconic.p, pub);
+    }
     if (!lhs_tau_kappa) return;
     HIP_CHECK(hipMemcpyAsync(h->pin->h + 48, h->sys_out_dev, 2 * sizeof(double), hipMemcpyDeviceToHost, st));
     HIP_CHECK(hipStreamSynchronize(st));
@@ -3684,8 +3731,11 @@
     h->sys_const_pending = false;
     const size_t N = (size_t)h->K.N;
     auto run = [&](bool defer) -> int {
+        const bool packed = !affine && !pair && knobs().fold && sys_offset_packs(h->cone_dev(), m, false);
+        PackRhs pk;
+        if (packed) { pk.b = h->b.p; pk.rhs_x = d_rhs_x; pk.n = n; pk.p = h->K.p; }
         if (!affine && !launch_sys_offset(h->cone_dev(), h->cone_state(), h->sconic.p, h->sworkz.p, d_rhs_s, d_var_z, d_rhs_z,
-                                          m, false, st))
+                                          m, false, st, pk))
             throw ArgError("hipkkt_kkt_system_solve: unsupported cone kind");
         if (pair) {
             launch_pack_rhs_affine(h->b.p, h->snegq.p, h->sb.p, d_rhs_x, d_var_s, d_rhs_z, n, m, h->K.p, 2, st);
@@ -3693,7 +3743,7 @@
             if (rc != HIPKKT_OK) return rc;
         } else {
             if (affine) launch_pack_rhs_affine(h->b.p, nullptr, nullptr, d_rhs_x, d_var_s, d_rhs_z, n, m, h->K.p, 1, st);
-            else launch_pack_rhs(h->b.p, d_rhs_x, h->sworkz.p, n, m, h->K.p, st);
+            else if (!packed) launch_pack_rhs(h->b.p, d_rhs_x, h->sworkz.p, n, m, h->K.p, st);
             int rc = kkt_solve_core(h, false, 1, nullptr, defer);
             if (rc != HIPKKT_OK) return rc;
         }
diff --git a/cuclarabel_amd/csrc/kernels.hip b/cuclarabel_amd/csrc/kernels.hip
--- a/cuclarabel_amd/csrc/kernels.hip
+++ b/cuclarabel_amd/csrc/kernels.hip
@@ -25,6 +25,19 @@
     if (n <= 0) return;
     hipLaunchKernelGGL(k_scatter, dim3(grid_for(n, 256)), dim3(256), 0, st, K, idx, v, n, scale);
 }
+__device__ inline double block_max_256(double v, double* sh)
+{
+#pragma unroll
+    for (int o = 32; o > 0; o >>= 1) v = fmax(v, __shfl_down(v, o, 64));
+    const int lane = threadIdx.x & 63, wave = threadIdx.x >> 6;
+    if (lane == 0) sh[wave] = v;
+    __syncthreads();
+    if (threadIdx.x == 0) {
+        for (int w = 1; w < (int)(blockDim.x >> 6); ++w) v = fmax(v, sh[w]);
+    }
+    return v;
+}
+
 __device__ __forceinline__ void put_k(double* __restrict__ K, double* __restrict__ fval, const int* __restrict__ kpos, int e, double v)
 {
     K[e] = v;
@@ -38,12 +51,17 @@
                                 const int* __restrict__ mapU, const int* __restrict__ mapV, const int* __restrict__ mapD,
                                 const double* __restrict__ u, const double* __restrict__ v, const double* __restrict__ eta2,
                                 const int* __restrict__ soc_of_entry, int sparse_len, int nsparse,
-                                double* __restrict__ fval, const int* __restrict__ kpos)
-{
+                                double* __restrict__ fval, const int* __restrict__ kpos,
+                                const unsigned char* __restrict__ hs_is_diag, double* __restrict__ dmax_partial)
+{
+    __shared__ double sh[4];
+    double dmax = 0.0;
     const int total = nHs + sparse_len + nsparse;
     for (int i = blockIdx.x * blockDim.x + threadIdx.x; i < total; i += gridDim.x * blockDim.x) {
         if (i < nHs) {
-            put_k(K, fval, kpos, mapHs[i], -Hs[i]);
+            const double hv = Hs[i];
+            put_k(K, fval, kpos, mapHs[i], -hv);
+            if (dmax_partial && hs_is_diag[i]) dmax = fmax(dmax, fabs(hv));
         } else if (i < nHs + sparse_len) {
             const int j = i - nHs;
             const double e2 = eta2[soc_of_entry[j]];
@@ -53,17 +71,25 @@
             const int j = i - nHs - sparse_len;
             put_k(K, fval, kpos, mapD[2 * j], -eta2[j]);
             put_k(K, fval, kpos, mapD[2 * j + 1], eta2[j]);
-        }
-    }
-}
-void launch_update_values(double* K, const int* mapHs, const double* Hs, int nHs, const int* mapU, const int* mapV,
-                          const int* mapD, const double* u, const double* v, const double* eta2, const int* soc_of_entry,
-                          int sparse_len, int nsparse, double* fval, const int* kpos, hipStream_t st)
+            if (dmax_partial) dmax = fmax(dmax, fabs(eta2[j]));
+        }
+    }
+    if (dmax_partial) {
+        dmax = block_max_256(dmax, sh);
+        if (threadIdx.x == 0) dmax_partial[blockIdx.x] = dmax;
+    }
+}
+int launch_update_values(double* K, const int* mapHs, const double* Hs, int nHs, const int* mapU, const int* mapV,
+                         const int* mapD, const double* u, const double* v, const double* eta2, const int* soc_of_entry,
+                         int sparse_len, int nsparse, double* fval, const int* kpos, hipStream_t st,
+                         const unsigned char* hs_is_diag, double* dmax_partial)
 {
     const int total = nHs + sparse_len + nsparse;
-    if (total <= 0) return;
-    hipLaunchKernelGGL(k_update_values, dim3(grid_for(total, 256)), dim3(256), 0, st, K, mapHs, Hs, nHs, mapU, mapV, mapD, u, v,
-                       eta2, soc_of_entry, sparse_len, nsparse, fval, kpos);
+    if (total <= 0) return 0;
+    const int g = grid_for(total, 256, kUpdateValuesGrid);
+    hipLaunchKernelGGL(k_update_values, dim3(g), dim3(256), 0, st, K, mapHs, Hs, nHs, mapU, mapV, mapD, u, v,
+                       eta2, soc_of_entry, sparse_len, nsparse, fval, kpos, hs_is_diag, dmax_partial);
+    return g;
 }
 __global__ void k_scale(double* __restrict__ K, const int* __restrict__ idx, double scale, int64_t n)
 {
@@ -100,19 +126,6 @@
     if (n <= 0) return;
     hipLaunchKernelGGL(k_soc_columns, dim3((n + 255) / 256), dim3(256), 0, st, K, mapU, mapV, mapD, u, v, eta2,
                        soc_of_entry, sparse_len, nsparse);
-}
-
-__device__ inline double block_max_256(double v, double* sh)
-{
-#pragma unroll
-    for (int o = 32; o > 0; o >>= 1) v = fmax(v, __shfl_down(v, o, 64));
-    const int lane = threadIdx.x & 63, wave = threadIdx.x >> 6;
-    if (lane == 0) sh[wave] = v;
-    __syncthreads();
-    if (threadIdx.x == 0) {
-        for (int w = 1; w < (int)(blockDim.x >> 6); ++w) v = fmax(v, sh[w]);
-    }
-    return v;
 }
 
 constexpr int kRedBlocks = 256;
@@ -415,6 +428,27 @@
     int* __restrict__ p = Z.p[blockIdx.y];
     const int n = Z.n[blockIdx.y];
     for (int i = blockIdx.x * blockDim.x + threadIdx.x; i < n; i += gridDim.x * blockDim.x) p[i] = 0;
+}
+__global__ void k_zero_ints_reg(ZeroList Z, RegFinish R)
+{
+    __shared__ double sh[4];
+    if (blockIdx.y < (unsigned)Z.count) {
+        int* __restrict__ p = Z.p[blockIdx.y];
+        const int n = Z.n[blockIdx.y];
+        for (int i = blockIdx.x * blockDim.x + threadIdx.x; i < n; i += gridDim.x * blockDim.x) p[i] = 0;
+    }
+    if (blockIdx.x == 0 && blockIdx.y == 0) {
+        double v = 0.0;
+        for (int i = threadIdx.x; i < R.nparts; i += blockDim.x) v = fmax(v, R.partial[i]);
+        v = block_max_256(v, sh);
+        if (threadIdx.x == 0) R.eps_out[0] = R.c0 + R.c1 * fmax(v, R.static_max[0]);
+    }
+}
+void launch_zero_ints_reg(const ZeroList& Z, const RegFinish& R, hipStream_t st)
+{
+    int nmax = 1;
+    for (int k = 0; k < Z.count; ++k) nmax = Z.n[k] > nmax ? Z.n[k] : nmax;
+    hipLaunchKernelGGL(k_zero_ints_reg, dim3(grid_for(nmax, 256, 256), std::max(Z.count, 1)), dim3(256), 0, st, Z, R);
 }
 void launch_zero_ints_multi(const ZeroList& Z, hipStream_t st)
 {
@@ -1284,36 +1318,48 @@
     }
 }
 
+struct VecX {
+    const double* __restrict__ x;
+    __device__ __forceinline__ double operator()(int i) const { return x[i]; }
+};
+struct StepX {
+    const double* __restrict__ a;
+    const double* __restrict__ b;
+    double t;
+    __device__ __forceinline__ double operator()(int i) const { return a[i] + t * b[i]; }
+};
+template <class X>
 __device__ inline void mul_Hs_elementwise_body(const ConeDev& C, const ConeState& S, double* __restrict__ y,
-                                               const double* __restrict__ x, int m, const double* __restrict__ addend, int bx, int nb)
+                                               const X x, int m, const double* __restrict__ addend, int bx, int nb)
 {
     for (int i = bx * 256 + threadIdx.x; i < m; i += nb * 256) {
         const int kind = C.kind[C.elem_cone[i]];
         double v;
         if (kind == 0) v = 0.0;
-        else if (kind == 1) v = S.w[i] * (S.w[i] * x[i]);
+        else if (kind == 1) v = S.w[i] * (S.w[i] * x(i));
         else if (kind == 4 || kind == 5) {
             const int c = C.elem_cone[i], off = C.off[c], r = i - off;
             const double* Hs = S.Hs + C.boff[c];
             auto at = [&](int a, int b) { return a <= b ? Hs[b * (b + 1) / 2 + a] : Hs[a * (a + 1) / 2 + b]; };
-            v = at(r, 0) * x[off] + at(r, 1) * x[off + 1] + at(r, 2) * x[off + 2];
+            v = at(r, 0) * x(off) + at(r, 1) * x(off + 1) + at(r, 2) * x(off + 2);
         }
         else continue;
         y[i] = addend ? -(v + addend[i]) : v;
     }
 }
+template <class X>
 __device__ inline void mul_Hs_soc_body(const ConeDev& C, const ConeState& S, double* __restrict__ y,
-                                       const double* __restrict__ x, const double* __restrict__ addend, int ci, int lane)
+                                       const X x, const double* __restrict__ addend, int ci, int lane)
 {
     const int c = C.soc_list[ci];
     const int off = C.off[c], n = C.numel[c];
     const double* w = S.w + off;
     double dot = 0.0;
-    for (int i = lane; i < n; i += 64) dot += w[i] * x[off + i];
+    for (int i = lane; i < n; i += 64) dot += w[i] * x(off + i);
     dot = 2.0 * wave_sum(dot);
     const double e2 = S.eta[c] * S.eta[c];
     for (int i = lane; i < n; i += 64) {
-        const double xi = x[off + i];
+        const double xi = x(off + i);
         const double v = ((i == 0 ? -xi : xi) + dot * w[i]) * e2;
         y[off + i] = addend ? -(v + addend[off + i]) : v;
     }
@@ -1333,9 +1379,9 @@
                                                 int m, const double* __restrict__ addend, int ge, Publish P)
 {
     if (P.dst && blockIdx.x == gridDim.x - 1 && threadIdx.x == 255) publish_record(P);
-    if ((int)blockIdx.x < ge) { mul_Hs_elementwise_body(C, S, y, x, m, addend, blockIdx.x, ge); return; }
+    if ((int)blockIdx.x < ge) { mul_Hs_elementwise_body(C, S, y, VecX{x}, m, addend, blockIdx.x, ge); return; }
     const int ci = ((int)blockIdx.x - ge) * 4 + (int)(threadIdx.x >> 6);
-    if (ci < C.nsoc) mul_Hs_soc_body(C, S, y, x, addend, ci, threadIdx.x & 63);
+    if (ci < C.nsoc) mul_Hs_soc_body(C, S, y, VecX{x}, addend, ci, threadIdx.x & 63);
 }
 __global__ __launch_bounds__(256) void k_mul_Hs_gp(ConeDev C, ConeState S, double* __restrict__ y, const double* __restrict__ x,
                                                    int m, const double* __restrict__ addend, int ge, int gs, Publish P)
@@ -1343,10 +1389,10 @@
     __shared__ double sh[12];
     if (P.dst && blockIdx.x == gridDim.x - 1 && threadIdx.x == 255) publish_record(P);
     const int bx = (int)blockIdx.x;
-    if (bx < ge) { mul_Hs_elementwise_body(C, S, y, x, m, addend, bx, ge); return; }
+    if (bx < ge) { mul_Hs_elementwise_body(C, S, y, VecX{x}, m, addend, bx, ge); return; }
     if (bx < ge + gs) {
         const int ci = (bx - ge) * 4 + (int)(threadIdx.x >> 6);
-        if (ci < C.nsoc) mul_Hs_soc_body(C, S, y, x, addend, ci, threadIdx.x & 63);
+        if (ci < C.nsoc) mul_Hs_soc_body(C, S, y, VecX{x}, addend, ci, threadIdx.x & 63);
         return;
     }
     const int gq = (C.ngp_small + 3) / 4, b0 = bx - ge - gs;
@@ -1487,7 +1533,7 @@
 __device__ inline void sys_offset_elementwise_body(const ConeDev& C, const ConeState& S, double* __restrict__ konst,
                                                    double* __restrict__ workz, const double* __restrict__ ds,
                                                    const double* __restrict__ z, const double* __restrict__ rhs_z, int m,
-                                                   int affine, int bx, int nb)
+                                                   int affine, int bx, int nb, double* __restrict__ bz = nullptr)
 {
     for (int i = bx * 256 + threadIdx.x; i < m; i += nb * 256) {
         double o;
@@ -1501,13 +1547,16 @@
             else continue;
         }
         konst[i] = o;
-        workz[i] = o - rhs_z[i];
+        const double wz = o - rhs_z[i];
+        workz[i] = wz;
+        if (bz) bz[i] = wz;
     }
 }
 
 __device__ inline void sys_offset_soc_body(const ConeDev& C, const ConeState& S, double* __restrict__ konst,
                                            double* __restrict__ workz, const double* __restrict__ ds,
-                                           const double* __restrict__ z, const double* __restrict__ rhs_z, int ci, int lane)
+                                           const double* __restrict__ z, const double* __restrict__ rhs_z, int ci, int lane,
+                                           double* __restrict__ bz = nullptr)
 {
     const int c = C.soc_list[ci];
     const int off = C.off[c], n = C.numel[c];
@@ -1536,7 +1585,9 @@
         else o = -zc[i] * cc + eta * (dsc[i] + wfac * w[i]);
         o *= linv;
         konst[off + i] = o;
-        workz[off + i] = o - rhs_z[off + i];
+        const double wz = o - rhs_z[off + i];
+        workz[off + i] = wz;
+        if (bz) bz[off + i] = wz;
     }
 }
 
@@ -1583,14 +1634,24 @@
 
 __global__ __launch_bounds__(256) void k_sys_offset(ConeDev C, ConeState S, double* __restrict__ konst, double* __restrict__ workz,
                                                     const double* __restrict__ ds, const double* __restrict__ z,
-                                                    const double* __restrict__ rhs_z, int m, int affine, int ge)
-{
-    if ((int)blockIdx.x < ge) { sys_offset_elementwise_body(C, S, konst, workz, ds, z, rhs_z, m, affine, blockIdx.x, ge); return; }
-    const int ci = ((int)blockIdx.x - ge) * 4 + (int)(threadIdx.x >> 6);
-    if (ci < C.nsoc) sys_offset_soc_body(C, S, konst, workz, ds, z, rhs_z, ci, threadIdx.x & 63);
-}
+                                                    const double* __restrict__ rhs_z, int m, int affine, int ge, int gs, PackRhs B)
+{
+    double* bz = B.b ? B.b + B.n : nullptr;
+    if ((int)blockIdx.x < ge) { sys_offset_elementwise_body(C, S, konst, workz, ds, z, rhs_z, m, affine, blockIdx.x, ge, bz); return; }
+    if ((int)blockIdx.x < ge + gs) {
+        const int ci = ((int)blockIdx.x - ge) * 4 + (int)(threadIdx.x >> 6);
+        if (ci < C.nsoc) sys_offset_soc_body(C, S, konst, workz, ds, z, rhs_z, ci, threadIdx.x & 63, bz);
+        return;
+    }
+    const int gx = (int)gridDim.x - ge - gs;
+    for (int i = ((int)blockIdx.x - ge - gs) * 256 + (int)threadIdx.x; i < B.n + B.p; i += gx * 256) {
+        if (i < B.n) B.b[i] = B.rhs_x[i];
+        else B.b[m + i] = 0.0;
+    }
+}
+bool sys_offset_packs(const ConeDev& C, int m, bool affine) { return m > 0 && (affine || C.npsd == 0); }
 bool launch_sys_offset(const ConeDev& C, const ConeState& S, double* konst, double* workz, const double* ds,
-                       const double* z, const double* rhs_z, int m, bool affine, hipStream_t st)
+                       const double* z, const double* rhs_z, int m, bool affine, hipStream_t st, const PackRhs& B)
 {
     if (m <= 0) return true;
     if (!affine && C.npsd > 0) {
@@ -1600,7 +1661,8 @@
         hipLaunchKernelGGL(k_sys_offset_psd, dim3(C.npsd), dim3(256), lds, st, C, S, konst, workz, ds, rhs_z);
     }
     const int ge = grid_for(m, 256), gs = affine ? 0 : (C.nsoc + 3) / 4;
-    hipLaunchKernelGGL(k_sys_offset, dim3(ge + gs), dim3(256), 0, st, C, S, konst, workz, ds, z, rhs_z, m, affine ? 1 : 0, ge);
+    const int gx = (B.b && B.n + B.p > 0) ? grid_for(B.n + B.p, 256) : 0;
+    hipLaunchKernelGGL(k_sys_offset, dim3(ge + gs + gx), dim3(256), 0, st, C, S, konst, workz, ds, z, rhs_z, m, affine ? 1 : 0, ge, gs, B);
     return true;
 }
 
@@ -1807,6 +1869,68 @@
                        (const double*)partial, cached, rhs_tau, rhs_kappa, tau, kappa, out, P.npairs, n, m, keep_x2, keep_z2);
 }
 
+__global__ __launch_bounds__(256) void k_sys_step_mul_Hs(StepArgs T, ConeDev C, ConeState S, double* __restrict__ y, int m,
+                                                         const double* __restrict__ addend, int gstep, int ge, Publish P)
+{
+    __shared__ double d[8];
+    __shared__ double sh_dtau;
+    const int p = threadIdx.x;
+    if (p < T.npairs) {
+        double acc = 0.0;
+        for (int i = 0; i < kDotBlocks; ++i) acc += T.partial[p * kDotBlocks + i];
+        d[p] = acc;
+    }
+    __syncthreads();
+    if (p == 0) {
+        const double c0 = T.npairs == 7 ? d[4] : T.cached[0], c1 = T.npairs == 7 ? d[5] : T.cached[1], c2 = T.npairs == 7 ? d[6] : T.cached[2];
+        const double tau_num = T.rhs_tau - T.rhs_kappa / T.tau + d[0] + d[1] + 2.0 * (d[2] / T.tau);
+        double tau_den = T.kappa / T.tau - c0 - c1;
+        tau_den += d[3] - c2;
+        const double dtau = tau_num / tau_den;
+        sh_dtau = dtau;
+        if (blockIdx.x == 0) {
+            if (T.npairs == 7) { T.cached[0] = c0; T.cached[1] = c1; T.cached[2] = c2; }
+            T.out[0] = dtau;
+            T.out[1] = -(T.rhs_kappa + T.kappa * dtau) / T.tau;
+            T.out[2] = tau_num;
+            T.out[3] = tau_den;
+        }
+    }
+    __syncthreads();
+    const double dtau = sh_dtau;
+    const int bx = (int)blockIdx.x;
+    if (P.dst && bx == (int)gridDim.x - 1 && threadIdx.x == 255) {
+        publish_record(P);
+        if (P.n >= 10) { P.dst[8] = dtau; P.dst[9] = -(T.rhs_kappa + T.kappa * dtau) / T.tau; }
+    }
+    if (bx < gstep) {
+        for (int i = bx * 256 + (int)threadIdx.x; i < T.n + T.m; i += gstep * 256) {
+            if (i < T.n) {
+                const double v = T.x2[i];
+                T.dx[i] = T.x1[i] + dtau * v;
+                if (T.keep_x2) T.keep_x2[i] = v;
+            } else {
+                const double v = T.z2[i - T.n];
+                T.dz[i - T.n] = T.z1[i - T.n] + dtau * v;
+                if (T.keep_z2) T.keep_z2[i - T.n] = v;
+            }
+        }
+        return;
+    }
+    const StepX x{T.z1, T.z2, dtau};
+    if (bx - gstep < ge) { mul_Hs_elementwise_body(C, S, y, x, m, addend, bx - gstep, ge); return; }
+    const int ci = (bx - gstep - ge) * 4 + (int)(threadIdx.x >> 6);
+    if (ci < C.nsoc) mul_Hs_soc_body(C, S, y, x, addend, ci, threadIdx.x & 63);
+}
+bool step_mul_Hs_folds(const ConeDev& C, int m) { return m > 0 && C.npsd == 0 && C.ngp_small == 0 && C.ngp_big == 0; }
+void launch_dots_sys_step_mul_Hs(const DotPairs& P, const StepArgs& T, const ConeDev& C, const ConeState& S, double* y, int m,
+                                 const double* addend, const Publish& pub, hipStream_t st)
+{
+    hipLaunchKernelGGL(k_dots, dim3(kDotBlocks, P.npairs), dim3(256), 0, st, P, const_cast<double*>(T.partial));
+    const int gstep = grid_for(std::max(T.n + T.m, 1), 256), ge = grid_for(m, 256), gs = (C.nsoc + 3) / 4;
+    hipLaunchKernelGGL(k_sys_step_mul_Hs, dim3(gstep + ge + gs), dim3(256), 0, st, T, C, S, y, m, addend, gstep, ge, pub);
+}
+
 __global__ void k_neg_sum(double* __restrict__ y, const double* __restrict__ a, const double* __restrict__ b, int n)
 {
     for (int i = blockIdx.x * blockDim.x + threadIdx.x; i < n; i += gridDim.x * blockDim.x) y[i] = -(a[i] + b[i]);
diff --git a/cuclarabel_amd/csrc/kernels.hpp b/cuclarabel_amd/csrc/kernels.hpp
--- a/cuclarabel_amd/csrc/kernels.hpp
+++ b/cuclarabel_amd/csrc/kernels.hpp
@@ -262,9 +262,11 @@
 constexpr int kLongChunk = 2048;
 constexpr int kNormParts = 2048;
 constexpr int kMaxNormbCols = 4;
-void launch_update_values(double* K, const int* mapHs, const double* Hs, int nHs, const int* mapU, const int* mapV,
-                          const int* mapD, const double* u, const double* v, const double* eta2, const int* soc_of_entry,
-                          int sparse_len, int nsparse, double* fval, const int* kpos, hipStream_t st);
+constexpr int kUpdateValuesGrid = 4096;
+int launch_update_values(double* K, const int* mapHs, const double* Hs, int nHs, const int* mapU, const int* mapV,
+                         const int* mapD, const double* u, const double* v, const double* eta2, const int* soc_of_entry,
+                         int sparse_len, int nsparse, double* fval, const int* kpos, hipStream_t st,
+                         const unsigned char* hs_is_diag = nullptr, double* dmax_partial = nullptr);
 void launch_residual(const SpmvDev& A, const double* Kval, const double* b, const double* x, double* e,
                      double* partial, double* norm_out, hipStream_t st, int nrhs = 1, int64_t ld = 0,
                      const int* flag_in = nullptr, double* flag_out = nullptr, double* normb_out = nullptr);
@@ -302,6 +304,14 @@
     void add(int* ptr, int len) { if (ptr && len > 0 && count < 8) { p[count] = ptr; n[count] = len; ++count; } }
 };
 void launch_zero_ints_multi(const ZeroList& Z, hipStream_t st);
+struct RegFinish {
+    const double* partial;
+    int nparts;
+    const double* static_max;
+    double c0, c1;
+    double* eps_out;
+};
+void launch_zero_ints_reg(const ZeroList& Z, const RegFinish& R, hipStream_t st);
 void launch_collect_status(double* dst, const double* eps, const int* conefail, const int* flags, hipStream_t st, double* sticky = nullptr);
 
 struct ConeDev {
@@ -370,10 +380,30 @@
 void launch_mul_Hs(const ConeDev& C, const ConeState& S, double* y, const double* x, int m, hipStream_t st, const double* addend = nullptr,
                    const Publish& pub = Publish{});
 void launch_psd_A_from_R(const ConeDev& C, const ConeState& S, hipStream_t st);
+struct DotPairs;
+struct StepArgs {
+    double *dx, *dz;
+    const double *x1, *z1, *x2, *z2;
+    const double* partial;
+    double* cached;
+    double rhs_tau, rhs_kappa, tau, kappa;
+    double* out;
+    int npairs, n, m;
+    double *keep_x2, *keep_z2;
+};
+bool step_mul_Hs_folds(const ConeDev& C, int m);
+void launch_dots_sys_step_mul_Hs(const DotPairs& P, const StepArgs& T, const ConeDev& C, const ConeState& S, double* y, int m,
+                                 const double* addend, const Publish& pub, hipStream_t st);
 void launch_cone_from_scaling(const ConeDev& C, const ConeState& S, int m, hipStream_t st);
 
+struct PackRhs {
+    double* b = nullptr;
+    const double* rhs_x = nullptr;
+    int n = 0, p = 0;
+};
+bool sys_offset_packs(const ConeDev& C, int m, bool affine);
 bool launch_sys_offset(const ConeDev& C, const ConeState& S, double* konst, double* workz, const double* ds,
-                       const double* z, const double* rhs_z, int m, bool affine, hipStream_t st);
+                       const double* z, const double* rhs_z, int m, bool affine, hipStream_t st, const PackRhs& B = PackRhs{});
 void launch_P_spmv(const SpmvDev& A, const double* Kval, const double* x, double* y, int n, hipStream_t st);
 void launch_sys_axpby(double* out, const double* a, const double* alpha_div, const double* b, const double* beta,
                       double beta_host, int n, hipStream_t st);
diff --git a/cuclarabel_amd/csrc/knobs.hpp b/cuclarabel_amd/csrc/knobs.hpp
--- a/cuclarabel_amd/csrc/knobs.hpp
+++ b/cuclarabel_amd/csrc/knobs.hpp
@@ -35,6 +35,8 @@
     FLAG_ON(pull_leaves, "HIPKKT_PULL_LEAVES")                   \
     FLAG_ON(packed, "HIPKKT_PACKED")                            \
     KNOB(long long, packed_max_mb, "HIPKKT_PACKED_MAX_MB", 4096)                       \
+                                                                                       \
+    FLAG_ON(fold, "HIPKKT_FOLD")                             \
                                                                                                                \
     FLAG_SET(graph, "HIPKKT_GRAPH")                               \
     FLAG_SET(no_overlap, "HIPKKT_NO_OVERLAP")                                                         \
diff --git a/cuclarabel_amd/csrc/solve_common.hpp b/cuclarabel_amd/csrc/solve_common.hpp
--- a/cuclarabel_amd/csrc/solve_common.hpp
+++ b/cuclarabel_amd/csrc/solve_common.hpp
@@ -33,6 +33,11 @@
     v = dpp_add_step<0x142, 0xa>(v);
     v = dpp_add_step<0x143, 0xc>(v);
     return readlane_f64(v, 63);
+}
+
+__device__ __forceinline__ void st_out(const SolveArgs& A, int64_t o, double v)
+{
+    A.out[o] = A.add ? v + A.add[o] : v;
 }
 
 template <int NR>
diff --git a/cuclarabel_amd/csrc/solve_kernels.hip b/cuclarabel_amd/csrc/solve_kernels.hip
--- a/cuclarabel_amd/csrc/solve_kernels.hip
+++ b/cuclarabel_amd/csrc/solve_kernels.hip
@@ -121,7 +121,7 @@
     if (lane < nc) {
         stv<NR>(A.xp, c0 + lane, y);
 #pragma unroll
-        for (int c = 0; c < NR; ++c) A.out[c * A.ld_out + idx] = y[c];
+        for (int c = 0; c < NR; ++c) st_out(A, c * A.ld_out + idx, y[c]);
     }
 }
 
@@ -218,7 +218,7 @@
     if (live && sub < nc) {
         stv<NR>(A.xp, c0 + sub, y);
 #pragma unroll
-        for (int c = 0; c < NR; ++c) A.out[c * A.ld_out + idx] = y[c];
+        for (int c = 0; c < NR; ++c) st_out(A, c * A.ld_out + idx, y[c]);
     }
 }
 template <int NR>
@@ -434,7 +434,7 @@
         for (int c = 0; c < NR; ++c) {
             const double v = lds_sum_col<NR>(vp, part, cst, c, j, nrs, ncpad);
             w[c] = v;
-            A.out[c * A.ld_out + pi] = v;
+            st_out(A, c * A.ld_out + pi, v);
         }
         stv<NR>(A.xp, c0 + j, w);
     }
@@ -734,7 +734,7 @@
             for (int c = 0; c < NR; ++c) {
                 const double v = lds_sum_col<NR>(vp, part, cst, c, j, nrs, ncpad);
                 ST_AGENT_F64(A.xp + (int64_t)(c0 + j) * NR + c, v);
-                A.out[c * A.ld_out + pi] = v;
+                st_out(A, c * A.ld_out + pi, v);
             }
         }
         asm volatile("s_waitcnt vmcnt(0)" ::: "memory");
@@ -1243,7 +1243,7 @@
                 for (int c = 0; c < NR; ++c) {
                     const double v = lds_sum_col<NR>(vp, part, cst, c, j, nrs, ncpad);
                     ST_AGENT_F64(A.xp + (int64_t)(c0 + j) * NR + c, v);
-                    A.out[c * A.ld_out + pi] = v;
+                    st_out(A, c * A.ld_out + pi, v);
                 }
             }
             asm volatile("s_waitcnt vmcnt(0)" ::: "memory");
@@ -1354,7 +1354,7 @@
                 for (int w = 0; w < NW; ++w) v += part[b * cst + w * 16 + jj];
                 const int j = j0 + cc + jj;
                 ST_AGENT_F64(A.xp + (int64_t)(c0 + j) * NR + b, v);
-                A.out[b * A.ld_out + T.perm[c0 + j]] = v;
+                st_out(A, b * A.ld_out + T.perm[c0 + j], v);
             }
             __syncthreads();
         }
@@ -1650,7 +1650,7 @@
         double v = 0.0;
         for (int bx = j / BR; bx < nb_used; ++bx) v += LD_AGENT_F64(front_part + (int64_t)bx * kBdColsSolveMax + j);
         A.xp[c0 + j] = v;
-        A.out[T.perm[c0 + j]] = v;
+        st_out(A, T.perm[c0 + j], v);
     }
 }
 static int tall_block_rows()
```

Result: no change. 314.8, median of 2 (-0.1%).
